# AleoNet/snarkVM

Hardware: NVIDIA H100
Metric: bls12_377_g1_msm_points_per_sec (higher is better)
Workload: dtype u32 limbs (Montgomery integer arithmetic, IMAD pipe)

## Files before the change

snarkvm_b200/csrc/api.cu:

```cuda
#include "../../include/snarkvm_b200.h"

#include <algorithm>
#include <atomic>
#include <condition_variable>
#include <cstdlib>
#include <cstring>
#include <deque>
#include <functional>
#include <map>
#include <memory>
#include <mutex>
#include <thread>
#include <vector>

#include <cuda_runtime.h>
#include <pthread.h>
#include <sched.h>
#include <cstdio>

#include "host_ec.hpp"
#include "msm.cuh"
#include "ntt.cuh"
#include "poly.cuh"

namespace b200 { void host_stream_copy(void* dst, const void* src, size_t n); }
using namespace b200;

namespace {

snarkvm_error_t make_error(int code) {
    snarkvm_error_t e;
    e.code = code;
    e.message = nullptr;
    if (code != 0) {
        const char* s = cudaGetErrorString((cudaError_t)code);
        if (s) { size_t n = strlen(s) + 1; e.message = (char*)malloc(n); if (e.message) memcpy(e.message, s, n); }
    }
    return e;
}

struct ThreadCtx {
    cudaStream_t stream[64] = {};
    bool have[64] = {};
    cudaStream_t copy_stream[64] = {};
    bool have_copy[64] = {};
    ~ThreadCtx() {}
};
thread_local ThreadCtx t_ctx;

int thread_stream(cudaStream_t* out) {
    int dev = 0;
    cudaError_t e = cudaGetDevice(&dev);
    if (e != cudaSuccess) return (int)e;
    dev &= 63;
    if (!t_ctx.have[dev]) {
        e = cudaStreamCreateWithFlags(&t_ctx.stream[dev], cudaStreamNonBlocking);
        if (e != cudaSuccess) return (int)e;
        t_ctx.have[dev] = true;
    }
    *out = t_ctx.stream[dev];
    return 0;
}

int thread_copy_stream(cudaStream_t* out) {
    int dev = 0;
    cudaError_t e = cudaGetDevice(&dev);
    if (e != cudaSuccess) return (int)e;
    dev &= 63;
    if (!t_ctx.have_copy[dev]) {
        e = cudaStreamCreateWithFlags(&t_ctx.copy_stream[dev], cudaStreamNonBlocking);
        if (e != cudaSuccess) return (int)e;
        t_ctx.have_copy[dev] = true;
    }
    *out = t_ctx.copy_stream[dev];
    return 0;
}

struct PrecomputedBases { uint32_t* table; size_t n; MsmPlan plan; int device; };
struct ResidentBases {
    void* d_ptr = nullptr;
    size_t npoints = 0, stride = 0;
    int device = 0;
    std::atomic<PrecomputedBases*> tables{nullptr};
    uint8_t head[104] = {}, tail[104] = {};
    ~ResidentBases() {
        int cur = 0;
        cudaGetDevice(&cur);
        if (cur != device) cudaSetDevice(device);
        if (d_ptr) cudaFree(d_ptr);
        if (PrecomputedBases* t = tables.load()) { cudaFree(t->table); delete t; }
        if (cur != device) cudaSetDevice(cur);
    }
};
std::mutex g_bases_mu;
std::map<const void*, std::shared_ptr<ResidentBases>> g_bases;

std::shared_ptr<ResidentBases> find_resident(const void* host, size_t npoints, size_t stride) {
    int dev = 0;
    if (cudaGetDevice(&dev) != cudaSuccess) return nullptr;
    std::shared_ptr<ResidentBases> r;
    {
        std::lock_guard<std::mutex> lock(g_bases_mu);
        auto it = g_bases.find(host);
        if (it == g_bases.end()) return nullptr;
        r = it->second;
    }
    if (r->device != dev || r->stride != stride || r->npoints < npoints) return nullptr;
    if (memcmp(r->head, host, 104) != 0) return nullptr;
    if (memcmp(r->tail, (const uint8_t*)host + (r->npoints - 1) * stride, 104) != 0) return nullptr;
    return r;
}

void write_infinity(void* out144) {
    host::Xyzz inf = host::xyzz_inf();
    host::xyzz_to_normalised_projective(inf, (uint64_t*)out144);
}

int msm_jobs_impl(void* out144s, const MsmPlan& plan, const MsmBases* bases, int nbases, const uint32_t* table, size_t table_n,
                  const MsmSegment* segs, int nsegs, int njobs, cudaStream_t stream) {
    const size_t sets = table ? 1 : (size_t)plan.nwin;
    const size_t npts = (size_t)njobs * sets;
    uint32_t* d_buf = nullptr;
    cudaError_t e = pool_alloc(&d_buf, npts * 192 + 256, stream);
    if (e != cudaSuccess) return (int)e;
    uint32_t* d_flags = d_buf + npts * 48;
    int rc = (int)cudaMemsetAsync(d_flags, 0, 256, stream);
    if (rc == 0) rc = msm_core(d_buf, d_flags, plan, bases, nbases, table, table_n, segs, nsegs, njobs, stream);
    static thread_local void* t_result_pinned = nullptr;
    constexpr size_t RESULT_PINNED_BYTES = (size_t)64 << 10;
    const size_t result_bytes = npts * 192 + 256;
    if (!t_result_pinned && result_bytes <= RESULT_PINNED_BYTES && cudaHostAlloc(&t_result_pinned, RESULT_PINNED_BYTES, cudaHostAllocDefault) != cudaSuccess) {
        cudaGetLastError(); t_result_pinned = nullptr;
    }
    std::vector<host::Xyzz> sums(npts + 2);
    void* land = (t_result_pinned && result_bytes <= RESULT_PINNED_BYTES) ? t_result_pinned : (void*)sums.data();
    if (rc == 0) rc = (int)cudaMemcpyAsync(land, d_buf, result_bytes, cudaMemcpyDeviceToHost, stream);
    cudaFreeAsync(d_buf, stream);
    if (rc == 0) rc = (int)cudaStreamSynchronize(stream);
    if (rc != 0) return rc;
    if (land != (void*)sums.data()) memcpy(sums.data(), land, result_bytes);
    uint32_t flags = 0;
    memcpy(&flags, sums.data() + npts, 4);
    if (flags & 1u) return (int)cudaErrorInvalidValue;
    auto finish = [&](int j) {
        host::Xyzz total = table ? sums[(size_t)j] : host::horner_windows(sums.data() + (size_t)j * sets, plan.nwin, plan.c);
        host::xyzz_to_normalised_projective(total, (uint64_t*)((uint8_t*)out144s + (size_t)j * 144));
    };
    if (njobs <= 2) { for (int j = 0; j < njobs; j++) finish(j); }
    else {
        const int nt = njobs < 8 ? njobs : 8;
        std::vector<std::thread> th;
        std::atomic<int> next{0};
        for (int t = 0; t < nt; t++) th.emplace_back([&] { for (int j; (j = next.fetch_add(1)) < njobs;) finish(j); });
        for (auto& t : th) t.join();
    }
    return 0;
}

int msm_device_impl(void* out144, const void* d_points, size_t npoints, const void* d_scalars, size_t stride, int mont,
                    cudaStream_t stream) {
    if (npoints == 0) { write_infinity(out144); return 0; }
    if (stride < 104 || (stride & 7)) return (int)cudaErrorInvalidValue;
    MsmPlan plan = msm_make_plan(npoints);
    MsmBases b{d_points, stride, npoints};
    MsmSegment sg{d_scalars, npoints, 0u, 0u, mont};
    return msm_jobs_impl(out144, plan, &b, 1, nullptr, 0, &sg, 1, 1, stream);
}

static bool device_local_cpus(cpu_set_t* out) {
    if (const char* e = getenv("SNARKVM_B200_COPY_NUMA")) { if (atoi(e) == 0) return false; }
    else { const char* lws = getenv("LOCAL_WORLD_SIZE"); if (!lws || atoi(lws) <= 1) return false; }
    int dev = 0;
    if (cudaGetDevice(&dev) != cudaSuccess) { cudaGetLastError(); return false; }
    char bus[64] = {};
    if (cudaDeviceGetPCIBusId(bus, (int)sizeof bus - 1, dev) != cudaSuccess) { cudaGetLastError(); return false; }
    for (char* c = bus; *c; c++) if (*c >= 'A' && *c <= 'Z') *c = (char)(*c - 'A' + 'a');
    char path[160];
    snprintf(path, sizeof path, "/sys/bus/pci/devices/%s/local_cpulist", bus);
    FILE* f = fopen(path, "r");
    if (!f) return false;
    char line[4096] = {};
    const bool got = fgets(line, sizeof line, f) != nullptr;
    fclose(f);
    if (!got) return false;
    cpu_set_t allowed, local;
    CPU_ZERO(&local);
    if (sched_getaffinity(0, sizeof allowed, &allowed) != 0) return false;
    for (const char* p = line; *p;) {
        while (*p == ',' || *p == ' ') p++;
        if (*p < '0' || *p > '9') break;
        char* end = nullptr;
        long a = strtol(p, &end, 10), b = a;
        if (*end == '-') b = strtol(end + 1, &end, 10);
        for (long c = a; c <= b && c < CPU_SETSIZE; c++) if (CPU_ISSET((int)c, &allowed)) CPU_SET((int)c, &local);
        p = end;
    }
    if (CPU_COUNT(&local) < 2 || CPU_COUNT(&local) == CPU_COUNT(&allowed)) return false;
    *out = local;
    return true;
}

class CopyPool {
public:
    bool numa_cpus(cpu_set_t* out) const { if (have_numa_) *out = numa_; return have_numa_; }
    static CopyPool& get() { static CopyPool* p = new CopyPool(); return *p; }
    void parallel_memcpy(void* dst, const void* src, size_t bytes) {
        const size_t piece = (size_t)2 << 20;
        if (bytes <= piece || nthreads_ == 0) { host_stream_copy(dst, src, bytes); return; }
        Batch batch;
        batch.dst = (uint8_t*)dst; batch.src = (const uint8_t*)src; batch.bytes = bytes; batch.piece = piece;
        batch.npieces = (bytes + piece - 1) / piece;
        run(batch);
    }
    void parallel_rows(void* dst, size_t dpitch, const void* src, size_t spitch, size_t width, size_t rows) {
        if (rows == 0 || width == 0) return;
        Batch batch;
        batch.dst = (uint8_t*)dst; batch.src = (const uint8_t*)src; batch.bytes = rows * width; batch.piece = width;
        batch.npieces = rows; batch.dpitch = dpitch; batch.spitch = spitch; batch.rows = true;
        if (nthreads_ == 0) { work(batch); return; }
        run(batch);
    }
private:
    struct Batch;
    void run(Batch& batch) {
        {
            std::lock_guard<std::mutex> lock(mu_);
            queue_.push_back(&batch);
        }
        cv_.notify_all();
        work(batch);
        std::unique_lock<std::mutex> lock(mu_);
        for (auto it = queue_.begin(); it != queue_.end(); ++it) if (*it == &batch) { queue_.erase(it); break; }
        done_cv_.wait(lock, [&] { return batch.active == 0; });
    }
    struct Batch {
        uint8_t* dst; const uint8_t* src; size_t bytes, piece, npieces;
        size_t dpitch = 0, spitch = 0;
        bool rows = false;
        std::atomic<size_t> next{0};
        int active = 0;
    };
    CopyPool() {
        int n = 12;
        if (const char* lws = getenv("LOCAL_WORLD_SIZE")) {
            const int procs = atoi(lws), cores = (int)std::thread::hardware_concurrency();
            if (procs > 1 && cores > 0) { int per = cores / procs - 1; if (per < 2) per = 2; if (per < n) n = per; }
        }
        if (const char* e = getenv("SNARKVM_B200_COPY_THREADS")) { int v = atoi(e); if (v >= 0 && v <= 64) n = v; }
        nthreads_ = n;
        have_numa_ = device_local_cpus(&numa_);
        for (int i = 0; i < n; i++) std::thread([this] { loop(); }).detach();
    }
    static void work(Batch& b) {
        for (;;) {
            size_t k = b.next.fetch_add(1);
            if (k >= b.npieces) return;
            if (b.rows) { host_stream_copy(b.dst + k * b.dpitch, b.src + k * b.spitch, b.piece); continue; }
            size_t off = k * b.piece, len = b.bytes - off < b.piece ? b.bytes - off : b.piece;
            host_stream_copy(b.dst + off, b.src + off, len);
        }
    }
    void loop() {
        if (have_numa_) pthread_setaffinity_np(pthread_self(), sizeof numa_, &numa_);
        std::unique_lock<std::mutex> lock(mu_);
        for (;;) {
            cv_.wait(lock, [&] { return !queue_.empty(); });
            Batch* b = queue_.front();
            if (b->next.load() >= b->npieces) { queue_.pop_front(); continue; }
            b->active++;
            lock.unlock();
            work(*b);
            lock.lock();
            if (--b->active == 0) done_cv_.notify_all();
        }
    }
    std::mutex mu_;
    std::condition_variable cv_, done_cv_;
    std::deque<Batch*> queue_;
    int nthreads_ = 0;
    cpu_set_t numa_;
    bool have_numa_ = false;
};

static bool host_is_pinned(const void* p) {
    cudaPointerAttributes attr;
    if (cudaPointerGetAttributes(&attr, p) != cudaSuccess) { cudaGetLastError(); return false; }
    return attr.type == cudaMemoryTypeHost || attr.type == cudaMemoryTypeManaged;
}

struct StageRing {
    static constexpr int SLOTS = 4;
    static constexpr size_t SLOT_BYTES = (size_t)32 << 20;
    void* buf[SLOTS] = {};
    cudaEvent_t ev[SLOTS] = {};
    bool used[SLOTS] = {};
    int next = 0;
    int init() {
        if (buf[0]) return 0;
// ... 164 lines not shown
    bool have = false;
    for (size_t i = 0; i < pcount && rc == 0; i++) {
        void* dst = have ? tmp : d_out;
        rc = (int)cudaMemsetAsync(dst, 0, bytes, stream);
        if (rc == 0 && plens[i]) rc = (int)cudaMemcpyAsync(dst, d_polys[i], plens[i] * 32, cudaMemcpyDeviceToDevice, stream);
        if (rc == 0) rc = ntt_device(dst, lg, NTT_FORWARD, NTT_STANDARD, scratch, stream);
        if (rc == 0 && have) rc = fr_pointwise_mul_device(d_out, tmp, n, stream);
        have = true;
    }
    for (size_t i = 0; i < ecount && rc == 0; i++) {
        if (have) rc = fr_pointwise_mul_device(d_out, d_evals[i], n, stream);
        else rc = (int)cudaMemcpyAsync(d_out, d_evals[i], bytes, cudaMemcpyDeviceToDevice, stream);
        have = true;
    }
    if (rc == 0) rc = ntt_device(d_out, lg, NTT_INVERSE, NTT_STANDARD, scratch, stream);
    cudaFreeAsync(tmp, stream);
    cudaFreeAsync(scratch, stream);
    return rc;
}

}

extern "C" {

const char* snarkvm_b200_version(void) { return "snarkvm_b200 0.1 (sm_90a)"; }
uint64_t snarkvm_b200_launch_count(void) { return launch_count(); }

snarkvm_error_t snarkvm_ntt(void* inout, uint32_t lg, snarkvm_ntt_order_t order, snarkvm_ntt_direction_t dir,
                            snarkvm_ntt_type_t type) {
    if (lg > NTT_MAX_LG || !inout || (int)order < 0 || (int)order > 3) return make_error((int)cudaErrorInvalidValue);
    cudaStream_t stream;
    int rc = thread_stream(&stream);
    if (rc) return make_error(rc);
    const size_t bytes = ((size_t)1 << lg) * 32;
    const bool pinned = host_is_pinned(inout);
    static const bool no_pipe = getenv("SNARKVM_B200_NTT_NO_PIPELINE") != nullptr;
    if (lg >= 20 && order == SNARKVM_NTT_NN && !no_pipe) {
        rc = ntt_host_pipelined(inout, lg, (int)dir, (int)type, stream, pinned);
        if (rc != -1) {
            int rs = (int)cudaStreamSynchronize(stream);
            return make_error(rc ? rc : rs);
        }
        rc = 0;
    }
    void *d = nullptr, *scratch = nullptr;
    rc = (int)pool_alloc(&d, bytes, stream);
    if (rc == 0) rc = (int)pool_alloc(&scratch, bytes, stream);
    if (rc == 0) rc = upload(d, inout, bytes, stream, pinned);
    if (rc == 0) rc = ntt_ordered(d, lg, (int)order, (int)dir, (int)type, scratch, stream);
    if (rc == 0) rc = (int)cudaStreamSynchronize(stream);
    if (rc == 0) rc = download(inout, d, bytes, stream, pinned);
    if (d) cudaFreeAsync(d, stream);
    if (scratch) cudaFreeAsync(scratch, stream);
    int rs = (int)cudaStreamSynchronize(stream);
    return make_error(rc ? rc : rs);
}

snarkvm_error_t snarkvm_polymul(void* out, size_t pcount, const void* polynomials, const void* plens_v, size_t ecount,
                                const void* evaluations, const void* elens_v, uint32_t lg) {
    if (pcount + ecount == 0) return make_error(0);
    if (lg > NTT_MAX_LG || !out) return make_error((int)cudaErrorInvalidValue);
    const void* const* polys = (const void* const*)polynomials;
    const void* const* evals = (const void* const*)evaluations;
    const size_t* plens = (const size_t*)plens_v;
    const size_t* elens = (const size_t*)elens_v;
    const size_t n = (size_t)1 << lg, bytes = n * 32;
    for (size_t i = 0; i < pcount; i++) if (plens[i] > n) return make_error((int)cudaErrorInvalidValue);
    for (size_t i = 0; i < ecount; i++) if (elens[i] != n) return make_error((int)cudaErrorInvalidValue);
    cudaStream_t stream;
    int rc = thread_stream(&stream);
    if (rc) return make_error(rc);
    std::vector<void*> dbuf(pcount + ecount, nullptr);
    std::vector<const void*> dp(pcount), de(ecount);
    void* d_out = nullptr;
    rc = (int)pool_alloc(&d_out, bytes, stream);
    for (size_t i = 0; i < pcount && rc == 0; i++) {
        size_t b = plens[i] ? plens[i] * 32 : 32;
        rc = (int)pool_alloc(&dbuf[i], b, stream);
        if (rc == 0 && plens[i]) rc = upload(dbuf[i], polys[i], plens[i] * 32, stream, host_is_pinned(polys[i]));
        dp[i] = dbuf[i];
    }
    for (size_t i = 0; i < ecount && rc == 0; i++) {
        rc = (int)pool_alloc(&dbuf[pcount + i], bytes, stream);
        if (rc == 0) rc = upload(dbuf[pcount + i], evals[i], bytes, stream, host_is_pinned(evals[i]));
        de[i] = dbuf[pcount + i];
    }
    if (rc == 0) rc = polymul_device_impl(d_out, pcount, dp.data(), plens, ecount, de.data(), elens, lg, stream);
    if (rc == 0) rc = (int)cudaStreamSynchronize(stream);
    if (rc == 0) rc = download(out, d_out, bytes, stream, host_is_pinned(out));
    for (void* p : dbuf) if (p) cudaFreeAsync(p, stream);
    if (d_out) cudaFreeAsync(d_out, stream);
    int rs = (int)cudaStreamSynchronize(stream);
    return make_error(rc ? rc : rs);
}

static std::vector<size_t> msm_ranges(size_t npoints) {
    std::vector<size_t> w;
    if (npoints >= ((size_t)1 << 23)) w = {1, 2, 4, 9};
    if (const char* e = getenv("SNARKVM_B200_MSM_CHUNKS")) {
        std::vector<size_t> v;
        for (const char* p = e; *p;) {
            char* end = nullptr;
            long x = strtol(p, &end, 10);
            if (end == p || x < 1 || x > 1024) { v.clear(); break; }
            v.push_back((size_t)x);
            p = *end == ':' ? end + 1 : end;
            if (*end && *end != ':') { v.clear(); break; }
        }
        if (v.size() == 1) v.assign(v[0] <= 64 ? v[0] : 64, 1);
        if (!v.empty()) w = v;
    }
    size_t total = 0;
    for (size_t x : w) total += x;
    std::vector<size_t> bounds{0};
    size_t acc = 0;
    for (size_t x : w) {
        acc += x;
        size_t b = (size_t)((unsigned __int128)npoints * acc / total);
        if (b > bounds.back()) bounds.push_back(b);
    }
    if (bounds.back() != npoints) bounds.push_back(npoints);
    return bounds;
}

snarkvm_error_t snarkvm_msm(void* out, const void* points, size_t npoints, const void* scalars, size_t ffi_affine_sz) {
    if (!out) return make_error((int)cudaErrorInvalidValue);
    if (npoints == 0) { write_infinity(out); return make_error(0); }
    if (!points || !scalars || ffi_affine_sz < 104 || (ffi_affine_sz & 7)) return make_error((int)cudaErrorInvalidValue);
    cudaStream_t stream;
    int rc = thread_stream(&stream);
    if (rc) return make_error(rc);
    void *d_points = nullptr, *d_scalars = nullptr;
    std::shared_ptr<ResidentBases> rb = find_resident(points, npoints, ffi_affine_sz);
    const bool resident = rb != nullptr;
    std::vector<size_t> bounds{0, npoints};
    if (!resident) bounds = msm_ranges(npoints);
    const int chunks = (int)bounds.size() - 1;
    const bool pin_s = host_is_pinned(scalars), pin_p = resident || host_is_pinned(points);
    if (!resident) rc = (int)pool_alloc(&d_points, npoints * ffi_affine_sz, stream);
    if (rc == 0) rc = (int)pool_alloc(&d_scalars, npoints * 32, stream);
    uint64_t result[18];
    if (chunks == 1) {
        if (rc == 0) rc = upload(d_scalars, scalars, npoints * 32, stream, pin_s);
        if (rc == 0 && !resident) rc = upload(d_points, points, npoints * ffi_affine_sz, stream, pin_p);
        if (rc == 0 && resident && rb->tables.load()) rc = snarkvm_b200_msm_precomputed_device(result, rb->tables.load(), d_scalars, npoints, stream);
        else if (rc == 0) rc = msm_device_impl(result, resident ? rb->d_ptr : d_points, npoints, d_scalars, ffi_affine_sz, 0, stream);
    } else {
        cudaStream_t copy = nullptr;
        if (rc == 0) rc = thread_copy_stream(&copy);
        std::vector<MsmPlan> plans;
        std::vector<size_t> sum_off{0};
        for (int k = 0; k < chunks; k++) {
            plans.push_back(msm_make_plan(bounds[k + 1] - bounds[k]));
            sum_off.push_back(sum_off.back() + (size_t)plans.back().nwin);
        }
        std::vector<cudaEvent_t> ev((size_t)chunks + 1, nullptr);
        for (auto& e : ev) if (rc == 0) rc = (int)cudaEventCreateWithFlags(&e, cudaEventDisableTiming);
        uint32_t* d_sums = nullptr;
        const size_t nsums = sum_off.back();
        if (rc == 0) rc = (int)pool_alloc(&d_sums, nsums * 192 + 256, stream);
        uint32_t* d_flags = d_sums ? d_sums + nsums * 48 : nullptr;
        if (rc == 0) rc = (int)cudaMemsetAsync(d_flags, 0, 256, stream);
        if (rc == 0) rc = (int)cudaEventRecord(ev[chunks], stream);
        if (rc == 0) rc = (int)cudaStreamWaitEvent(copy, ev[chunks], 0);
        for (int k = 0; k < chunks && rc == 0; k++) {
            const size_t i0 = bounds[k], cn = bounds[k + 1] - i0;
            rc = upload((uint8_t*)d_scalars + i0 * 32, (const uint8_t*)scalars + i0 * 32, cn * 32, copy, pin_s);
            if (rc == 0) rc = upload((uint8_t*)d_points + i0 * ffi_affine_sz, (const uint8_t*)points + i0 * ffi_affine_sz, cn * ffi_affine_sz, copy, pin_p);
            if (rc == 0) rc = (int)cudaEventRecord(ev[k], copy);
            if (rc == 0) rc = (int)cudaStreamWaitEvent(stream, ev[k], 0);
            if (rc == 0) rc = msm_window_sums_device(d_sums + sum_off[k] * 48, d_flags, plans[k], (const uint8_t*)d_points + i0 * ffi_affine_sz,
                                                     ffi_affine_sz, (const uint8_t*)d_scalars + i0 * 32, cn, stream);
        }
        std::vector<host::Xyzz> sums(nsums + 2);
        if (rc == 0) rc = (int)cudaMemcpyAsync(sums.data(), d_sums, nsums * 192 + 256, cudaMemcpyDeviceToHost, stream);
        if (d_sums) cudaFreeAsync(d_sums, stream);
        if (copy) { int rs = (int)cudaStreamSynchronize(copy); if (rc == 0) rc = rs; }
        if (rc == 0) rc = (int)cudaStreamSynchronize(stream);
        for (auto& e : ev) if (e) cudaEventDestroy(e);
        if (rc == 0) {
            uint32_t flags = 0;
            memcpy(&flags, sums.data() + nsums, 4);
            if (flags & 1u) rc = (int)cudaErrorInvalidValue;
        }
        if (rc == 0) {
            host::Xyzz total = host::xyzz_inf();
            for (int k = 0; k < chunks; k++) host::xyzz_add(total, host::horner_windows(sums.data() + sum_off[k], plans[k].nwin, plans[k].c));
            host::xyzz_to_normalised_projective(total, result);
        }
    }
    if (d_points) cudaFreeAsync(d_points, stream);
    if (d_scalars) cudaFreeAsync(d_scalars, stream);
    int rs = (int)cudaStreamSynchronize(stream);
    if (rc == 0 && rs == 0) memcpy(out, result, 144);
    return make_error(rc ? rc : rs);
}

int snarkvm_b200_ntt_device(void* d_inout, uint32_t lg, int order, int dir, int type, void* d_scratch, void* stream) {
    if (lg > NTT_MAX_LG) return (int)cudaErrorInvalidValue;
    return ntt_ordered(d_inout, lg, order, dir, type, d_scratch, (cudaStream_t)stream);
}

int snarkvm_b200_polymul_device(void* d_out, size_t pcount, const void* const* d_polys, const size_t* plens, size_t ecount,
                                const void* const* d_evals, const size_t* elens, uint32_t lg, void* stream) {
    if (lg > NTT_MAX_LG) return (int)cudaErrorInvalidValue;
    return polymul_device_impl(d_out, pcount, d_polys, plens, ecount, d_evals, elens, lg, (cudaStream_t)stream);
}

int snarkvm_b200_msm_plan(size_t npoints, int* c, int* nwin, uint32_t* cap) {
    MsmPlan p = msm_make_plan(npoints);
    if (c) *c = p.c;
    if (nwin) *nwin = p.nwin;
    if (cap) *cap = p.cap;
    return 0;
}

int snarkvm_b200_msm_plan_levels(size_t npoints) { return msm_make_plan(npoints).levels; }

int snarkvm_b200_msm_device(void* out144, const void* d_points, size_t npoints, const void* d_scalars, size_t stride,
                            void* stream) {
    if (!out144) return (int)cudaErrorInvalidValue;
    return msm_device_impl(out144, d_points, npoints, d_scalars, stride, 0, (cudaStream_t)stream);
}

static int msm_batch_impl(void* out144s, const void* d_points, size_t stride, const void* const* d_scalars, const size_t* nscalars,
                          size_t count, int mont, const void* d_points2, const void* const* d_scalars2, const size_t* nscalars2,
                          cudaStream_t stream) {
    if (count == 0) return 0;
    if (!out144s || !d_scalars || !nscalars || stride < 104 || (stride & 7)) return (int)cudaErrorInvalidValue;
    std::vector<MsmSegment> segs;
    std::vector<size_t> job_of(count, (size_t)-1);
    size_t max_n = 0, total_n = 0, max_n2 = 0;
    uint32_t njobs = 0;
    for (size_t i = 0; i < count; i++) {
        const size_t n2 = (d_scalars2 && nscalars2) ? nscalars2[i] : 0;
        if (nscalars[i] == 0 && n2 == 0) { write_infinity((uint8_t*)out144s + i * 144); continue; }
        job_of[i] = njobs;
        if (nscalars[i]) segs.push_back(MsmSegment{d_scalars[i], nscalars[i], 0u, njobs, mont});
        if (nscalars[i] > max_n) max_n = nscalars[i];
        if (n2 > max_n2) max_n2 = n2;
        total_n += nscalars[i] + n2;
        njobs++;
    }
    if (njobs == 0) return 0;
    if (max_n >= (1ull << 31)) return (int)cudaErrorInvalidValue;
    for (size_t i = 0; i < count; i++) {
        const size_t n2 = (d_scalars2 && nscalars2) ? nscalars2[i] : 0;
        if (n2) segs.push_back(MsmSegment{d_scalars2[i], n2, (uint32_t)max_n, (uint32_t)job_of[i], mont});
    }
    MsmBases bases[2] = {{d_points, stride, max_n}, {d_points2, stride, max_n2}};
    const int nbases = max_n2 ? 2 : 1;
    if (max_n2 && !d_points2) return (int)cudaErrorInvalidValue;
    size_t job_max = max_n + max_n2;
    MsmPlan plan = msm_make_plan_batch(job_max ? job_max : 1, total_n);
    std::vector<uint8_t> outs((size_t)njobs * 144);
    int rc = msm_jobs_impl(outs.data(), plan, bases, nbases, nullptr, 0, segs.data(), (int)segs.size(), (int)njobs, stream);
    if (rc != 0) return rc;
    for (size_t i = 0; i < count; i++) if (job_of[i] != (size_t)-1) memcpy((uint8_t*)out144s + i * 144, outs.data() + job_of[i] * 144, 144);
    return 0;
}

int snarkvm_b200_msm_batch_device(void* out144s, const void* d_points, size_t stride, const void* const* d_scalars, const size_t* nscalars,
                                  size_t count, void* stream) {
    return msm_batch_impl(out144s, d_points, stride, d_scalars, nscalars, count, 0, nullptr, nullptr, nullptr, (cudaStream_t)stream);
}

int snarkvm_b200_msm_window_sums_device(void* d_window_sums, const void* d_points, size_t npoints, const void* d_scalars,
                                        size_t stride, void* stream) {
    return snarkvm_b200_msm_window_sums_plan_device(d_window_sums, nullptr, npoints, d_points, npoints, d_scalars, stride, stream);
}

int snarkvm_b200_msm_window_sums_plan_device(void* d_window_sums, uint32_t* d_flags, size_t plan_npoints, const void* d_points,
                                             size_t npoints, const void* d_scalars, size_t stride, void* stream_v) {
    if (!d_window_sums || stride < 104 || (stride & 7) || plan_npoints == 0 || npoints > plan_npoints) return (int)cudaErrorInvalidValue;
    cudaStream_t stream = (cudaStream_t)stream_v;
    MsmPlan plan = msm_make_plan(plan_npoints);
    uint32_t* own_flags = nullptr;
    int rc = 0;
    if (!d_flags) { rc = (int)pool_alloc(&own_flags, 256, stream); if (rc) return rc; d_flags = own_flags; }
    rc = (int)cudaMemsetAsync(d_flags, 0, 4, stream);
    if (rc == 0 && npoints == 0) rc = (int)cudaMemsetAsync(d_window_sums, 0, (size_t)plan.nwin * 192, stream);
    else if (rc == 0) rc = msm_window_sums_device((uint32_t*)d_window_sums, d_flags, plan, d_points, stride, d_scalars, npoints, stream);
    if (own_flags) cudaFreeAsync(own_flags, stream);
    return rc;
}

int snarkvm_b200_msm_window_sums_host(void* d_window_sums, uint32_t* d_flags, size_t plan_npoints, const void* h_points, size_t npoints,
                                      const void* h_scalars, size_t stride, void* stream_v) {
    if (!d_window_sums || stride < 104 || (stride & 7) || plan_npoints == 0 || npoints > plan_npoints) return (int)cudaErrorInvalidValue;
    cudaStream_t stream = (cudaStream_t)stream_v;
    MsmPlan plan = msm_make_plan(plan_npoints);
    uint32_t* own_flags = nullptr;
    int rc = 0;
    if (!d_flags) { rc = (int)pool_alloc(&own_flags, 256, stream); if (rc) return rc; d_flags = own_flags; }
    rc = (int)cudaMemsetAsync(d_flags, 0, 4, stream);
    if (npoints == 0) {
        if (rc == 0) rc = (int)cudaMemsetAsync(d_window_sums, 0, (size_t)plan.nwin * 192, stream);
        if (own_flags) cudaFreeAsync(own_flags, stream);
        return rc;
    }
    if (!h_points || !h_scalars) { if (own_flags) cudaFreeAsync(own_flags, stream); return (int)cudaErrorInvalidValue; }
    std::vector<size_t> bounds = msm_ranges(npoints);
    const int chunks = (int)bounds.size() - 1;
    const bool pin_s = host_is_pinned(h_scalars), pin_p = host_is_pinned(h_points);
    cudaStream_t copy = nullptr;
    void *d_points = nullptr, *d_scalars = nullptr;
    uint32_t* d_parts = nullptr;
    std::vector<cudaEvent_t> ev((size_t)chunks + 1, nullptr);
    if (rc == 0) rc = thread_copy_stream(&copy);
    if (rc == 0) rc = (int)pool_alloc(&d_points, npoints * stride, stream);
    if (rc == 0) rc = (int)pool_alloc(&d_scalars, npoints * 32, stream);
    if (rc == 0 && chunks > 1) rc = (int)pool_alloc(&d_parts, (size_t)chunks * plan.nwin * 192, stream);
    for (auto& e : ev) if (rc == 0) rc = (int)cudaEventCreateWithFlags(&e, cudaEventDisableTiming);
    if (rc == 0) rc = (int)cudaEventRecord(ev[chunks], stream);
    if (rc == 0) rc = (int)cudaStreamWaitEvent(copy, ev[chunks], 0);
    for (int k = 0; k < chunks && rc == 0; k++) {
        const size_t i0 = bounds[k], cn = bounds[k + 1] - i0;
        rc = upload((uint8_t*)d_scalars + i0 * 32, (const uint8_t*)h_scalars + i0 * 32, cn * 32, copy, pin_s);
        if (rc == 0) rc = upload((uint8_t*)d_points + i0 * stride, (const uint8_t*)h_points + i0 * stride, cn * stride, copy, pin_p);
        if (rc == 0) rc = (int)cudaEventRecord(ev[k], copy);
        if (rc == 0) rc = (int)cudaStreamWaitEvent(stream, ev[k], 0);
        uint32_t* dst = chunks > 1 ? d_parts + (size_t)k * plan.nwin * 48 : (uint32_t*)d_window_sums;
        if (rc == 0) rc = msm_window_sums_device(dst, d_flags, plan, (const uint8_t*)d_points + i0 * stride, stride,
                                                 (const uint8_t*)d_scalars + i0 * 32, cn, stream);
    }
    if (rc == 0 && chunks > 1) rc = xyzz_sum_ranks_device((uint32_t*)d_window_sums, d_parts, chunks, plan.nwin, stream);
    if (rc != 0 && copy) cudaStreamSynchronize(copy);
    if (d_parts) cudaFreeAsync(d_parts, stream);
    if (d_points) cudaFreeAsync(d_points, stream);
    if (d_scalars) cudaFreeAsync(d_scalars, stream);
    if (own_flags) cudaFreeAsync(own_flags, stream);
    for (auto& e : ev) if (e) cudaEventDestroy(e);
    return rc;
}

int snarkvm_b200_xyzz_sum_ranks_device(void* d_out, const void* d_in, int nranks, int count, void* stream) {
    if (nranks < 1 || count < 1) return (int)cudaErrorInvalidValue;
    return xyzz_sum_ranks_device((uint32_t*)d_out, (const uint32_t*)d_in, nranks, count, (cudaStream_t)stream);
}

int snarkvm_b200_msm_finish(void* out144, const void* h_window_sums, int nwin, int c) {
    if (!out144 || !h_window_sums || nwin < 1 || c < 0) return (int)cudaErrorInvalidValue;
    std::vector<host::Xyzz> sums((size_t)nwin);
    memcpy(sums.data(), h_window_sums, (size_t)nwin * 192);
    host::Xyzz total = host::horner_windows(sums.data(), nwin, c);
    host::xyzz_to_normalised_projective(total, (uint64_t*)out144);
    return 0;
}

int snarkvm_b200_msm_scratch_stats(size_t* limit_bytes, size_t* in_use_bytes, size_t* peak_bytes) {
    return msm_scratch_stats(limit_bytes, in_use_bytes, peak_bytes);
}
int snarkvm_b200_msm_set_scratch_limit(size_t limit_bytes) { return msm_set_scratch_limit(limit_bytes); }

int snarkvm_b200_kzg_commit_device(void* out144, const void* d_powers, size_t stride, const void* d_coeffs_mont,
                                   size_t ncoeffs, void* stream_v) {
    if (!out144) return (int)cudaErrorInvalidValue;
    return msm_device_impl(out144, d_powers, ncoeffs, d_coeffs_mont, stride, 1, (cudaStream_t)stream_v);
}

int snarkvm_b200_msm_precompute_device(void** handle_out, const void* d_points, size_t npoints, size_t stride, void* stream_v) {
    if (!handle_out || !d_points || npoints == 0 || stride < 104 || (stride & 7)) return (int)cudaErrorInvalidValue;
    cudaStream_t stream = (cudaStream_t)stream_v;
    MsmPlan plan = msm_make_plan_precomputed(npoints);
    if (npoints * (size_t)plan.nwin >= (1ull << 31)) return (int)cudaErrorInvalidValue;
    int dev = 0;
    cudaError_t e = cudaGetDevice(&dev);
    if (e != cudaSuccess) return (int)e;
    uint32_t* table = nullptr;
    if ((e = cudaMalloc(&table, npoints * (size_t)plan.nwin * 128)) != cudaSuccess) return (int)e;
    int rc = msm_precompute_tables_device(table, plan, d_points, stride, npoints, stream);
    if (rc == 0) rc = (int)cudaStreamSynchronize(stream);
    if (rc != 0) { cudaFree(table); return rc; }
    *handle_out = new PrecomputedBases{table, npoints, plan, dev};
    return 0;
}

int snarkvm_b200_msm_precomputed_free(void* handle) {
    if (!handle) return (int)cudaErrorInvalidValue;
    PrecomputedBases* h = (PrecomputedBases*)handle;
    cudaError_t e = cudaFree(h->table);
    delete h;
    return (int)e;
}

int snarkvm_b200_msm_precomputed_info(const void* handle, size_t* npoints, int* c, int* nwin, size_t* table_bytes) {
    if (!handle) return (int)cudaErrorInvalidValue;
    const PrecomputedBases* h = (const PrecomputedBases*)handle;
    if (npoints) *npoints = h->n;
    if (c) *c = h->plan.c;
    if (nwin) *nwin = h->plan.nwin;
    if (table_bytes) *table_bytes = h->n * (size_t)h->plan.nwin * 128;
    return 0;
}

static int msm_precomputed_impl(void* out144, const void* handle, const void* d_scalars, size_t nscalars, int mont, cudaStream_t stream) {
    if (!out144 || !handle) return (int)cudaErrorInvalidValue;
    const PrecomputedBases* h = (const PrecomputedBases*)handle;
    if (nscalars > h->n) return (int)cudaErrorInvalidValue;
    if (nscalars == 0) { write_infinity(out144); return 0; }
    if (!d_scalars) return (int)cudaErrorInvalidValue;
    MsmSegment sg{d_scalars, nscalars, 0u, 0u, mont};
    return msm_jobs_impl(out144, h->plan, nullptr, 0, h->table, h->n, &sg, 1, 1, stream);
}
int snarkvm_b200_msm_precomputed_device(void* out144, const void* handle, const void* d_scalars, size_t nscalars, void* stream_v) {
    return msm_precomputed_impl(out144, handle, d_scalars, nscalars, 0, (cudaStream_t)stream_v);
}
int snarkvm_b200_kzg_commit_precomputed_device(void* out144, const void* handle, const void* d_coeffs_mont, size_t ncoeffs, void* stream_v) {
    return msm_precomputed_impl(out144, handle, d_coeffs_mont, ncoeffs, 1, (cudaStream_t)stream_v);
}
int snarkvm_b200_kzg_commit_batch_precomputed_device(void* out144s, const void* handle, const void* const* d_coeffs_mont, const size_t* ncoeffs,
                                                     size_t count, void* stream_v) {
    if (count == 0) return 0;
    if (!out144s || !handle || !d_coeffs_mont || !ncoeffs) return (int)cudaErrorInvalidValue;
    const PrecomputedBases* h = (const PrecomputedBases*)handle;
    std::vector<MsmSegment> segs;
    std::vector<size_t> job_of(count, (size_t)-1);
    uint32_t njobs = 0;
    for (size_t i = 0; i < count; i++) {
        if (ncoeffs[i] > h->n) return (int)cudaErrorInvalidValue;
        if (ncoeffs[i] == 0) { write_infinity((uint8_t*)out144s + i * 144); continue; }
        job_of[i] = njobs;
        segs.push_back(MsmSegment{d_coeffs_mont[i], ncoeffs[i], 0u, njobs++, 1});
    }
    if (njobs == 0) return 0;
    std::vector<uint8_t> outs((size_t)njobs * 144);
    int rc = msm_jobs_impl(outs.data(), h->plan, nullptr, 0, h->table, h->n, segs.data(), (int)segs.size(), (int)njobs, (cudaStream_t)stream_v);
    if (rc != 0) return rc;
    for (size_t i = 0; i < count; i++) if (job_of[i] != (size_t)-1) memcpy((uint8_t*)out144s + i * 144, outs.data() + job_of[i] * 144, 144);
    return 0;
}

int snarkvm_b200_kzg_commit_hiding_device(void* out144, const void* d_powers, size_t stride, const void* d_coeffs_mont, size_t ncoeffs,
                                          const void* d_gamma_powers, const void* d_blinding_mont, size_t nblinding, void* stream) {
    if (!out144) return (int)cudaErrorInvalidValue;
    const void* c1[1] = {d_coeffs_mont};
    const void* c2[1] = {d_blinding_mont};
    return msm_batch_impl(out144, d_powers, stride, c1, &ncoeffs, 1, 1, d_gamma_powers, c2, &nblinding, (cudaStream_t)stream);
}

int snarkvm_b200_kzg_commit_batch_device(void* out144s, const void* d_powers, size_t stride, const void* const* d_coeffs_mont,
                                         const size_t* ncoeffs, size_t count, void* stream) {
    return msm_batch_impl(out144s, d_powers, stride, d_coeffs_mont, ncoeffs, count, 1, nullptr, nullptr, nullptr, (cudaStream_t)stream);
}
int snarkvm_b200_kzg_commit_batch_hiding_device(void* out144s, const void* d_powers, size_t stride, const void* const* d_coeffs_mont,
                                                const size_t* ncoeffs, const void* d_gamma_powers, const void* const* d_blinding_mont,
                                                const size_t* nblinding, size_t count, void* stream) {
    return msm_batch_impl(out144s, d_powers, stride, d_coeffs_mont, ncoeffs, count, 1, d_gamma_powers, d_blinding_mont, nblinding, (cudaStream_t)stream);
}

int snarkvm_b200_sonic_commit_batch_device(void* out144s, size_t stride, const void* const* d_bases, const void* const* d_coeffs_mont,
                                           const size_t* ncoeffs, const void* const* d_gamma_bases, const void* const* d_blinding_mont,
                                           const size_t* nblinding, size_t count, void* stream_v) {
    cudaStream_t stream = (cudaStream_t)stream_v;
    if (count == 0) return 0;
    if (!out144s || !d_bases || !d_coeffs_mont || !ncoeffs || stride < 104 || (stride & 7)) return (int)cudaErrorInvalidValue;
    struct Use { const uint8_t* p; size_t n; const void* scal; uint32_t job; };
    std::vector<Use> uses;
    std::vector<size_t> job_of(count, (size_t)-1), job_n;
    uint32_t njobs = 0;
    size_t total_n = 0;
    for (size_t i = 0; i < count; i++) {
        const size_t n1 = ncoeffs[i], n2 = (d_blinding_mont && nblinding) ? nblinding[i] : 0;
        if (n1 == 0 && n2 == 0) { write_infinity((uint8_t*)out144s + i * 144); continue; }
        if ((n1 && (!d_bases[i] || !d_coeffs_mont[i])) || (n2 && (!d_gamma_bases || !d_gamma_bases[i] || !d_blinding_mont[i]))) return (int)cudaErrorInvalidValue;
        job_of[i] = njobs;
        if (n1) uses.push_back(Use{(const uint8_t*)d_bases[i], n1, d_coeffs_mont[i], njobs});
        if (n2) uses.push_back(Use{(const uint8_t*)d_gamma_bases[i], n2, d_blinding_mont[i], njobs});
        job_n.push_back(n1 + n2);
        total_n += n1 + n2;
        njobs++;
    }
    if (njobs == 0) return 0;
    std::vector<size_t> order(uses.size());
    for (size_t k = 0; k < order.size(); k++) order[k] = k;
    std::sort(order.begin(), order.end(), [&](size_t a, size_t b) { return uses[a].p < uses[b].p; });
    std::vector<MsmBases> arrays;
    std::vector<size_t> array_first;
    std::vector<uint32_t> base0(uses.size(), 0);
    size_t concat = 0;
    for (size_t k : order) {
        const Use& u = uses[k];
        bool joined = false;
        if (!arrays.empty()) {
            MsmBases& a = arrays.back();
            const uint8_t* a0 = (const uint8_t*)a.d_points;
            const size_t off = (size_t)(u.p - a0);
            if (off <= a.n * stride && off % stride == 0) {
                const size_t first = off / stride;
                if (first + u.n > a.n) { concat += first + u.n - a.n; a.n = first + u.n; }
                base0[k] = (uint32_t)(array_first.back() + first);
                joined = true;
            } else if (off < a.n * stride) return (int)cudaErrorInvalidValue;
        }
        if (!joined) {
            array_first.push_back(concat);
            arrays.push_back(MsmBases{u.p, stride, u.n});
            base0[k] = (uint32_t)concat;
            concat += u.n;
        }
        if (concat >= (1ull << 31)) return (int)cudaErrorInvalidValue;
    }
    std::vector<MsmSegment> segs;
    for (size_t k = 0; k < uses.size(); k++) segs.push_back(MsmSegment{uses[k].scal, uses[k].n, base0[k], uses[k].job, 1});
    size_t job_max = 1;
    for (size_t v : job_n) if (v > job_max) job_max = v;
    MsmPlan plan = msm_make_plan_batch(job_max, total_n);
    std::vector<uint8_t> outs((size_t)njobs * 144);
    int rc = msm_jobs_impl(outs.data(), plan, arrays.data(), (int)arrays.size(), nullptr, 0, segs.data(), (int)segs.size(), (int)njobs, stream);
    if (rc != 0) return rc;
    for (size_t i = 0; i < count; i++) if (job_of[i] != (size_t)-1) memcpy((uint8_t*)out144s + i * 144, outs.data() + job_of[i] * 144, 144);
    return 0;
}

static int msm_g2_impl(void* out288, const void* d_points, size_t npoints, const void* d_scalars, size_t stride, cudaStream_t stream) {
    if (!out288) return (int)cudaErrorInvalidValue;
    if (npoints == 0) { host::Xyzz2 inf = host::xyzz_inf_t<host::Fq2>(); host::xyzz_to_normalised_projective(inf, (uint64_t*)out288); return 0; }
    if (!d_points || !d_scalars || stride < 200 || (stride & 7)) return (int)cudaErrorInvalidValue;
    MsmPlan plan = msm_make_plan(npoints);
    const size_t nw = (size_t)plan.nwin;
    uint32_t* d_buf = nullptr;
    cudaError_t e = pool_alloc(&d_buf, nw * 384 + 256, stream);
    if (e != cudaSuccess) return (int)e;
    uint32_t* d_flags = d_buf + nw * 96;
    int rc = (int)cudaMemsetAsync(d_flags, 0, 256, stream);
    if (rc == 0) rc = msm_g2_window_sums_device(d_buf, d_flags, plan, d_points, stride, d_scalars, npoints, 0, stream);
    std::vector<host::Xyzz2> sums(nw + 1);
    if (rc == 0) rc = (int)cudaMemcpyAsync(sums.data(), d_buf, nw * 384 + 256, cudaMemcpyDeviceToHost, stream);
    cudaFreeAsync(d_buf, stream);
    if (rc == 0) rc = (int)cudaStreamSynchronize(stream);
    if (rc != 0) return rc;
    uint32_t flags = 0;
    memcpy(&flags, sums.data() + nw, 4);
    if (flags & 1u) return (int)cudaErrorInvalidValue;
    host::Xyzz2 total = host::horner_windows(sums.data(), plan.nwin, plan.c);
    host::xyzz_to_normalised_projective(total, (uint64_t*)out288);
    return 0;
}
int snarkvm_b200_msm_g2_device(void* out288, const void* d_points, size_t npoints, const void* d_scalars, size_t stride, void* stream) {
    return msm_g2_impl(out288, d_points, npoints, d_scalars, stride, (cudaStream_t)stream);
}
snarkvm_error_t snarkvm_b200_msm_g2(void* out, const void* points, size_t npoints, const void* scalars, size_t ffi_affine_sz) {
    if (!out) return make_error((int)cudaErrorInvalidValue);
    uint64_t result[36];
    if (npoints == 0) { int rc0 = msm_g2_impl(result, nullptr, 0, nullptr, 200, nullptr); if (rc0 == 0) memcpy(out, result, 288); return make_error(rc0); }
    if (!points || !scalars || ffi_affine_sz < 200 || (ffi_affine_sz & 7)) return make_error((int)cudaErrorInvalidValue);
    cudaStream_t stream;
    int rc = thread_stream(&stream);
    if (rc) return make_error(rc);
    void *d_points = nullptr, *d_scalars = nullptr;
    rc = (int)pool_alloc(&d_points, npoints * ffi_affine_sz, stream);
    if (rc == 0) rc = (int)pool_alloc(&d_scalars, npoints * 32, stream);
    if (rc == 0) rc = upload(d_scalars, scalars, npoints * 32, stream, host_is_pinned(scalars));
    if (rc == 0) rc = upload(d_points, points, npoints * ffi_affine_sz, stream, host_is_pinned(points));
    if (rc == 0) rc = msm_g2_impl(result, d_points, npoints, d_scalars, ffi_affine_sz, stream);
    if (d_points) cudaFreeAsync(d_points, stream);
    if (d_scalars) cudaFreeAsync(d_scalars, stream);
    int rs = (int)cudaStreamSynchronize(stream);
    if (rc == 0 && rs == 0) memcpy(out, result, 288);
    return make_error(rc ? rc : rs);
}
int snarkvm_b200_generate_bases_g2_device(void* d_points, size_t npoints, size_t stride, uint64_t seed, void* stream) {
    return msm_generate_bases_g2_device(d_points, npoints, stride, seed, (cudaStream_t)stream);
}

int snarkvm_b200_g1_ntt_device(void* d_out, size_t out_stride, const void* d_in, size_t in_stride, uint32_t lg, int direction, void* stream) {
    return g1_ntt_device(d_out, out_stride, d_in, in_stride, lg, direction, (cudaStream_t)stream);
}
int snarkvm_b200_fr_batch_inversion_and_mul_device(void* d_v, size_t n, const void* coeff_mont_host, void* stream) {
    return fr_batch_inversion_and_mul_device(d_v, n, coeff_mont_host, (cudaStream_t)stream);
}
int snarkvm_b200_poly_divide_by_vanishing_device(void* d_q, void* d_r, const void* d_p, size_t m, size_t n, void* stream) {
    return poly_divide_by_vanishing_device(d_q, d_r, d_p, m, n, (cudaStream_t)stream);
}
int snarkvm_b200_poly_divide_by_linear_device(void* d_q, const void* d_p, size_t m, const void* point_mont_host, void* stream) {
    return poly_divide_by_linear_device(d_q, d_p, m, point_mont_host, (cudaStream_t)stream);
}
int snarkvm_b200_sparse_matvec_device(void* d_out, const void* d_row_ptr, const void* d_cols, const void* d_vals, size_t nrows, const void* d_x,
                                      size_t nvars, void* stream) {
    return sparse_matvec_device(d_out, d_row_ptr, d_cols, d_vals, nrows, d_x, nvars, (cudaStream_t)stream);
}
int snarkvm_b200_fr_vec_op_device(void* d_out, const void* d_a, const void* d_b, size_t n, int op, void* stream) {
    return fr_vec_op_device(d_out, d_a, d_b, n, op, (cudaStream_t)stream);
}
int snarkvm_b200_fr_vec_scalar_op_device(void* d_out, const void* d_a, const void* scalar_mont_host, size_t n, int op, void* stream) {
    return fr_vec_scalar_op_device(d_out, d_a, scalar_mont_host, n, op, (cudaStream_t)stream);
}
int snarkvm_b200_domain_elements_device(void* d_out, uint32_t lg, void* stream) {
    return domain_elements_device(d_out, lg, (cudaStream_t)stream);
}
int snarkvm_b200_varuna_matrix_evals_device(void* d_row, void* d_col, void* d_row_col_val, const void* d_row_ptr, size_t nrows,
                                            const void* d_cols, const void* d_vals, size_t nnz, size_t nvars, size_t input_size,
                                            uint32_t lg_constraint, uint32_t lg_variable, uint32_t lg_non_zero, void* stream) {
    return varuna_matrix_evals_device(d_row, d_col, d_row_col_val, d_row_ptr, nrows, d_cols, d_vals, nnz, nvars, input_size, lg_constraint,
                                      lg_variable, lg_non_zero, (cudaStream_t)stream);
}
int snarkvm_b200_csr_transpose_device(void* d_t_row_ptr, void* d_t_cols, void* d_t_vals, const void* d_row_ptr, size_t nrows,
                                      const void* d_cols, const void* d_vals, size_t nnz, size_t nvars, size_t input_size,
                                      uint32_t lg_variable, void* stream) {
    return csr_transpose_device(d_t_row_ptr, d_t_cols, d_t_vals, d_row_ptr, nrows, d_cols, d_vals, nnz, nvars, input_size, lg_variable,
                                (cudaStream_t)stream);
}
int snarkvm_b200_poly_evaluate_device(void* out_mont_host, const void* d_coeffs, size_t m, const void* point_mont_host, void* stream) {
    return poly_evaluate_device(out_mont_host, d_coeffs, m, point_mont_host, (cudaStream_t)stream);
}

int snarkvm_b200_fr_from_mont_device(void* d_out, const void* d_in, size_t n, void* stream) {
    return fr_from_mont_device(d_out, d_in, n, (cudaStream_t)stream);
}
int snarkvm_b200_fr_to_mont_device(void* d_out, const void* d_in, size_t n, void* stream) {
    return fr_to_mont_device(d_out, d_in, n, (cudaStream_t)stream);
}

int snarkvm_b200_srs_decode_device(void* d_out, size_t stride, const void* d_in96, size_t npoints, uint32_t* d_invalid, void* stream) {
    if (!d_out || !d_in96 || !d_invalid) return (int)cudaErrorInvalidValue;
    return srs_decode_device(d_out, stride, d_in96, npoints, d_invalid, (cudaStream_t)stream);
}

int snarkvm_b200_register_bases(const void* host_points, size_t npoints, size_t stride) {
    if (!host_points || npoints == 0 || stride < 104 || (stride & 7)) return (int)cudaErrorInvalidValue;
    auto rb = std::make_shared<ResidentBases>();
    cudaError_t e = cudaGetDevice(&rb->device);
    if (e != cudaSuccess) return (int)e;
    if ((e = cudaMalloc(&rb->d_ptr, npoints * stride)) != cudaSuccess) return (int)e;
    if ((e = cudaMemcpy(rb->d_ptr, host_points, npoints * stride, cudaMemcpyHostToDevice)) != cudaSuccess) return (int)e;
    rb->npoints = npoints; rb->stride = stride;
    memcpy(rb->head, host_points, 104);
    memcpy(rb->tail, (const uint8_t*)host_points + (npoints - 1) * stride, 104);
    std::lock_guard<std::mutex> lock(g_bases_mu);
    g_bases[host_points] = rb;
    return 0;
}
int snarkvm_b200_unregister_bases(const void* host_points) {
    std::shared_ptr<ResidentBases> old;
    {
        std::lock_guard<std::mutex> lock(g_bases_mu);
        auto it = g_bases.find(host_points);
        if (it == g_bases.end()) return (int)cudaErrorInvalidValue;
        old = it->second;
        g_bases.erase(it);
    }
    return 0;
}
int snarkvm_b200_register_bases_precomputed(const void* host_points, size_t npoints, size_t stride) {
    int rc = snarkvm_b200_register_bases(host_points, npoints, stride);
    if (rc != 0) return rc;
    std::shared_ptr<ResidentBases> rb;
    {
        std::lock_guard<std::mutex> lock(g_bases_mu);
        auto it = g_bases.find(host_points);
        if (it == g_bases.end()) return (int)cudaErrorInvalidValue;
        rb = it->second;
    }
    cudaStream_t stream;
    if ((rc = thread_stream(&stream)) != 0) return rc;
    void* tables = nullptr;
    rc = snarkvm_b200_msm_precompute_device(&tables, rb->d_ptr, npoints, stride, stream);
    if (rc != 0) { snarkvm_b200_unregister_bases(host_points); return rc; }
    PrecomputedBases* expected = nullptr;
    if (!rb->tables.compare_exchange_strong(expected, (PrecomputedBases*)tables)) { snarkvm_b200_msm_precomputed_free(tables); }
    return 0;
}

int snarkvm_b200_selftest_host_copy(size_t max_bytes, uint64_t seed, uint32_t* mismatches) {
    if (!mismatches || max_bytes < 4096) return (int)cudaErrorInvalidValue;
    std::vector<uint8_t> src(max_bytes + 256), dst(max_bytes + 256), ref(max_bytes + 256);
    uint64_t x = seed | 1;
    auto rnd = [&x]() { x ^= x << 13; x ^= x >> 7; x ^= x << 17; return x; };
    for (size_t i = 0; i < src.size(); i++) src[i] = (uint8_t)rnd();
    uint32_t bad = 0;
    const size_t sizes[] = {0, 1, 31, 32, 33, 4095, 4096, 4097, 65537, ((size_t)2 << 20) - 1, ((size_t)2 << 20) + 5, max_bytes};
    for (size_t n : sizes) {
// ... 104 lines not shown
```

snarkvm_b200/csrc/host_ec.hpp:

```cpp
#pragma once
#include <cstdint>
#include <cstring>
#if defined(__x86_64__)
#include <x86intrin.h>
#endif

namespace b200 { namespace host {

typedef unsigned __int128 u128;

struct Fq {
    uint64_t l[6];
};
static const uint64_t Q_MOD[6] = {0x8508c00000000001ull, 0x170b5d4430000000ull, 0x1ef3622fba094800ull,
                                  0x1a22d9f300f5138full, 0xc63b05c06ca1493bull, 0x01ae3a4617c510eaull};
static const uint64_t Q_R1[6] = {0x02cdffffffffff68ull, 0x51409f837fffffb1ull, 0x9f7db3a98a7d3ff2ull,
                                 0x7b4e97b76e7c6305ull, 0x4cf495bf803c84e8ull, 0x008d6661e2fdf49aull};
static const uint64_t Q_INV = 9586122913090633727ull;

inline Fq fq_zero() { Fq r; memset(r.l, 0, 48); return r; }
inline Fq fq_one() { Fq r; memcpy(r.l, Q_R1, 48); return r; }
inline bool fq_is_zero(const Fq& a) { uint64_t t = 0; for (int i = 0; i < 6; i++) t |= a.l[i]; return t == 0; }
inline bool fq_eq(const Fq& a, const Fq& b) { return memcmp(a.l, b.l, 48) == 0; }
inline bool ge_mod(const uint64_t* t) {
    for (int i = 5; i >= 0; i--) { if (t[i] != Q_MOD[i]) return t[i] > Q_MOD[i]; }
    return true;
}
inline void sub_mod(uint64_t* t) {
    uint64_t br = 0;
    for (int i = 0; i < 6; i++) { u128 d = (u128)t[i] - Q_MOD[i] - br; t[i] = (uint64_t)d; br = (uint64_t)(d >> 64) & 1; }
}
inline Fq fq_add(const Fq& a, const Fq& b) {
#if defined(__x86_64__)
    unsigned long long s[6], d[6];
    unsigned char c = 0, br = 0;
    for (int i = 0; i < 6; i++) c = _addcarry_u64(c, a.l[i], b.l[i], &s[i]);
    for (int i = 0; i < 6; i++) br = _subborrow_u64(br, s[i], Q_MOD[i], &d[i]);
    Fq r;
    for (int i = 0; i < 6; i++) r.l[i] = br ? s[i] : d[i];
    return r;
#else
    Fq r; u128 c = 0;
    for (int i = 0; i < 6; i++) { c += (u128)a.l[i] + b.l[i]; r.l[i] = (uint64_t)c; c >>= 64; }
    if (ge_mod(r.l)) sub_mod(r.l);
    return r;
#endif
}
inline Fq fq_sub(const Fq& a, const Fq& b) {
#if defined(__x86_64__)
    unsigned long long d[6], e[6];
    unsigned char br = 0, c = 0;
    for (int i = 0; i < 6; i++) br = _subborrow_u64(br, a.l[i], b.l[i], &d[i]);
    for (int i = 0; i < 6; i++) c = _addcarry_u64(c, d[i], Q_MOD[i], &e[i]);
    Fq r;
    for (int i = 0; i < 6; i++) r.l[i] = br ? e[i] : d[i];
    return r;
#else
    Fq r; uint64_t br = 0;
    for (int i = 0; i < 6; i++) { u128 d = (u128)a.l[i] - b.l[i] - br; r.l[i] = (uint64_t)d; br = (uint64_t)(d >> 64) & 1; }
    if (br) { u128 c = 0; for (int i = 0; i < 6; i++) { c += (u128)r.l[i] + Q_MOD[i]; r.l[i] = (uint64_t)c; c >>= 64; } }
    return r;
#endif
}
inline Fq fq_dbl(const Fq& a) { return fq_add(a, a); }
inline void fq_mul_row(uint64_t (&t)[6], const uint64_t* a, uint64_t bi) {
    u128 p = (u128)a[0] * bi + t[0];
    uint64_t c1 = (uint64_t)(p >> 64);
    const uint64_t lo = (uint64_t)p, k = lo * Q_INV;
    p = (u128)k * Q_MOD[0] + lo;
    uint64_t c2 = (uint64_t)(p >> 64);
#pragma GCC unroll 8
    for (int j = 1; j < 6; j++) {
        p = (u128)a[j] * bi + t[j] + c1;
        c1 = (uint64_t)(p >> 64);
        p = (u128)k * Q_MOD[j] + (uint64_t)p + c2;
        t[j - 1] = (uint64_t)p;
        c2 = (uint64_t)(p >> 64);
    }
    t[5] = c1 + c2;
}
inline Fq fq_mul(const Fq& a, const Fq& b) {
    uint64_t t[6] = {0, 0, 0, 0, 0, 0};
#pragma GCC unroll 8
    for (int i = 0; i < 6; i++) fq_mul_row(t, a.l, b.l[i]);
    if (ge_mod(t)) sub_mod(t);
    Fq r; memcpy(r.l, t, 48); return r;
}
inline Fq fq_sqr(const Fq& a) { return fq_mul(a, a); }
inline Fq fq_inverse(const Fq& a) {
    uint64_t e[6]; memcpy(e, Q_MOD, 48); e[0] -= 2;
    Fq acc = fq_one(); bool started = false;
    for (int i = 5; i >= 0; i--)
        for (int b = 63; b >= 0; b--) {
            if (started) acc = fq_sqr(acc);
            if ((e[i] >> b) & 1) { acc = started ? fq_mul(acc, a) : a; started = true; }
        }
    return acc;
}

struct Fq2 {
    Fq c0, c1;
};
inline Fq fq_times5(const Fq& x) { Fq t = fq_dbl(fq_dbl(x)); return fq_add(t, x); }
inline Fq f_zero(const Fq*) { return fq_zero(); }
inline Fq f_one(const Fq*) { return fq_one(); }
inline bool f_is_zero(const Fq& a) { return fq_is_zero(a); }
inline Fq f_add(const Fq& a, const Fq& b) { return fq_add(a, b); }
inline Fq f_sub(const Fq& a, const Fq& b) { return fq_sub(a, b); }
inline Fq f_dbl(const Fq& a) { return fq_dbl(a); }
inline Fq f_mul(const Fq& a, const Fq& b) { return fq_mul(a, b); }
inline Fq f_sqr(const Fq& a) { return fq_sqr(a); }
inline Fq f_inverse(const Fq& a) { return fq_inverse(a); }
inline Fq2 f_zero(const Fq2*) { Fq2 r; r.c0 = fq_zero(); r.c1 = fq_zero(); return r; }
inline Fq2 f_one(const Fq2*) { Fq2 r; r.c0 = fq_one(); r.c1 = fq_zero(); return r; }
inline bool f_is_zero(const Fq2& a) { return fq_is_zero(a.c0) && fq_is_zero(a.c1); }
inline Fq2 f_add(const Fq2& a, const Fq2& b) { Fq2 r; r.c0 = fq_add(a.c0, b.c0); r.c1 = fq_add(a.c1, b.c1); return r; }
inline Fq2 f_sub(const Fq2& a, const Fq2& b) { Fq2 r; r.c0 = fq_sub(a.c0, b.c0); r.c1 = fq_sub(a.c1, b.c1); return r; }
inline Fq2 f_dbl(const Fq2& a) { return f_add(a, a); }
inline Fq2 f_mul(const Fq2& a, const Fq2& b) {
    Fq v0 = fq_mul(a.c0, b.c0), v1 = fq_mul(a.c1, b.c1);
    Fq2 r;
    r.c1 = fq_sub(fq_sub(fq_mul(fq_add(a.c0, a.c1), fq_add(b.c0, b.c1)), v0), v1);
    r.c0 = fq_sub(v0, fq_times5(v1));
    return r;
}
inline Fq2 f_sqr(const Fq2& a) { return f_mul(a, a); }
inline Fq2 f_inverse(const Fq2& a) {
    Fq n = fq_inverse(fq_add(fq_sqr(a.c0), fq_times5(fq_sqr(a.c1))));
    Fq2 r; r.c0 = fq_mul(a.c0, n); r.c1 = fq_sub(fq_zero(), fq_mul(a.c1, n));
    return r;
}

template <class F>
struct XyzzT {
    F X, Y, ZZ, ZZZ;
};
typedef XyzzT<Fq> Xyzz;
typedef XyzzT<Fq2> Xyzz2;
template <class F> inline XyzzT<F> xyzz_inf_t() { XyzzT<F> r; r.X = r.Y = r.ZZ = r.ZZZ = f_zero((const F*)nullptr); return r; }
inline Xyzz xyzz_inf() { return xyzz_inf_t<Fq>(); }
template <class F> inline bool xyzz_is_inf(const XyzzT<F>& p) { return f_is_zero(p.ZZ); }
template <class F> inline void xyzz_dbl(XyzzT<F>& p) {
    if (xyzz_is_inf(p)) return;
    F U = f_dbl(p.Y), V = f_sqr(U), W = f_mul(U, V), S = f_mul(p.X, V);
    F XX = f_sqr(p.X), M = f_add(f_dbl(XX), XX);
    F X3 = f_sub(f_sqr(M), f_dbl(S));
    F Y3 = f_sub(f_mul(M, f_sub(S, X3)), f_mul(W, p.Y));
    p.X = X3; p.Y = Y3; p.ZZ = f_mul(V, p.ZZ); p.ZZZ = f_mul(W, p.ZZZ);
}
template <class F> inline void xyzz_add(XyzzT<F>& p, const XyzzT<F>& o) {
    if (xyzz_is_inf(o)) return;
    if (xyzz_is_inf(p)) { p = o; return; }
    F U1 = f_mul(p.X, o.ZZ), U2 = f_mul(o.X, p.ZZ), S1 = f_mul(p.Y, o.ZZZ), S2 = f_mul(o.Y, p.ZZZ);
    F P = f_sub(U2, U1), R = f_sub(S2, S1);
    if (f_is_zero(P)) { if (f_is_zero(R)) xyzz_dbl(p); else p = xyzz_inf_t<F>(); return; }
    F PP = f_sqr(P), PPP = f_mul(P, PP), Q = f_mul(U1, PP);
    F X3 = f_sub(f_sub(f_sqr(R), PPP), f_dbl(Q));
    p.Y = f_sub(f_mul(R, f_sub(Q, X3)), f_mul(S1, PPP));
    p.X = X3;
    p.ZZ = f_mul(f_mul(p.ZZ, o.ZZ), PP);
    p.ZZZ = f_mul(f_mul(p.ZZZ, o.ZZZ), PPP);
}
template <class F> inline void xyzz_to_normalised_projective(const XyzzT<F>& p, uint64_t* out) {
    const size_t fb = sizeof(F);
    F one = f_one((const F*)nullptr);
    if (xyzz_is_inf(p)) { memset(out, 0, 3 * fb); memcpy((uint8_t*)out + fb, &one, fb); return; }
    F i = f_inverse(f_mul(p.ZZ, p.ZZZ));
    F x = f_mul(p.X, f_mul(i, p.ZZZ)), y = f_mul(p.Y, f_mul(i, p.ZZ));
    memcpy(out, &x, fb); memcpy((uint8_t*)out + fb, &y, fb); memcpy((uint8_t*)out + 2 * fb, &one, fb);
}
inline Xyzz xyzz_from_projective(const uint64_t in[18]) {
    Xyzz p; memcpy(p.X.l, in, 48); memcpy(p.Y.l, in + 6, 48);
    Fq Z; memcpy(Z.l, in + 12, 48);
    p.ZZ = fq_sqr(Z); p.ZZZ = fq_mul(p.ZZ, Z);
    if (fq_is_zero(Z)) p = xyzz_inf();
    return p;
}
template <class F> inline XyzzT<F> horner_windows(const XyzzT<F>* sums, int nwin, int c) {
    XyzzT<F> total = xyzz_inf_t<F>();
    for (int w = nwin - 1; w >= 0; w--) {
        for (int k = 0; k < c; k++) xyzz_dbl(total);
        xyzz_add(total, sums[w]);
    }
    return total;
}

}}
```

snarkvm_b200/csrc/msm.cu:

```cuda
#include "msm.cuh"

#include <atomic>
#include <condition_variable>
#include <memory>
#include <mutex>
#include <utility>
#include <vector>
#include <cstdio>
#include <cstdlib>
#include <cub/device/device_scan.cuh>

#define FF_CALL_MUL 1
#include "ec.cuh"
#include "cta_inverse.cuh"
#include "quad.cuh"
#define FIELD_TEST_ENTRY test_field_op_msm
#include "testops.cuh"

namespace b200 {

static std::atomic<uint64_t> g_launches{0};
uint64_t launch_count() { return g_launches.load(); }
void count_launch(int n) { g_launches.fetch_add((uint64_t)n); }

static std::atomic<bool> g_prof{false};
static std::mutex g_prof_mu;
static std::vector<std::pair<cudaEvent_t, cudaEvent_t>> g_prof_recs[PROF_KINDS];
void prof_enable(bool on) { g_prof.store(on); }
bool prof_enabled() { return g_prof.load(); }
ProfScope::ProfScope(int kind_, cudaStream_t stream_) : stream(stream_), kind(kind_) {
    if (!g_prof.load()) return;
    if (cudaEventCreate(&a) != cudaSuccess || cudaEventCreate(&b) != cudaSuccess) { a = b = nullptr; return; }
    cudaEventRecord(a, stream);
}
ProfScope::~ProfScope() {
    if (!a) return;
    cudaEventRecord(b, stream);
    std::lock_guard<std::mutex> lock(g_prof_mu);
    g_prof_recs[kind].emplace_back(a, b);
}
int prof_collect(int kind, double* total_ms, uint64_t* count) {
    if (kind < 0 || kind >= PROF_KINDS) return (int)cudaErrorInvalidValue;
    std::vector<std::pair<cudaEvent_t, cudaEvent_t>> recs;
    { std::lock_guard<std::mutex> lock(g_prof_mu); recs.swap(g_prof_recs[kind]); }
    double tot = 0; int rc = 0;
    for (auto& r : recs) {
        float ms = 0;
        cudaError_t e = cudaEventSynchronize(r.second);
        if (e == cudaSuccess) e = cudaEventElapsedTime(&ms, r.first, r.second);
        if (e != cudaSuccess) rc = (int)e; else tot += ms;
        cudaEventDestroy(r.first); cudaEventDestroy(r.second);
    }
    if (total_ms) *total_ms = tot;
    if (count) *count = recs.size();
    return rc;
}

#define CUDA_TRY(x)                                   \
    do {                                              \
        cudaError_t e_ = (x);                         \
        if (e_ != cudaSuccess) { rc = (int)e_; goto done; } \
    } while (0)

static int ceil_log2(size_t x) { int l = 0; size_t v = x > 1 ? x - 1 : 0; while (v) { l++; v >>= 1; } return l; }
static int plan_log2(size_t x) {
    int l = ceil_log2(x < 2 ? 2 : x);
    if (l > 1 && (double)x < 0.70710678118 * (double)((size_t)1 << l)) l--;
    return l;
}

MsmPlan msm_make_plan(size_t npoints) {
    MsmPlan p;
    int lg = plan_log2(npoints);
    int c = lg <= 8 ? 4 : lg <= 12 ? lg - 4 : lg <= 18 ? 11 : lg == 19 ? 13 : lg == 20 ? 15 : lg <= 22 ? 16 : 17;
    if (const char* e = getenv("SNARKVM_B200_MSM_C")) { int v = atoi(e); if (v >= 2 && v <= 24) c = v; }
    p.c = c;
    p.nwin = 253 / c + 1;
    p.nbuckets = 1u << (c - 1);
    size_t total = npoints * (size_t)p.nwin;
    size_t cap = total / 300000 + 1;
    if (cap < 16) cap = 16;
    if (const char* e = getenv("SNARKVM_B200_MSM_CAP")) { long v = atol(e); if (v >= 1) cap = (size_t)v; }
    p.cap = (uint32_t)cap;
    int levels = lg >= 23 ? 5 : lg >= 21 ? 4 : lg == 20 ? 3 : lg == 19 ? 2 : 0;
    while (levels > 0 && ((npoints >> (c - 1)) >> levels) < 2) levels--;
    if (const char* e = getenv("SNARKVM_B200_MSM_LEVELS")) { int v = atoi(e); if (v >= 0 && v <= 16) levels = v; }
    p.levels = levels;
    return p;
}

MsmPlan msm_make_plan_batch(size_t max_n, size_t total_n) {
    MsmPlan p = msm_make_plan(max_n);
    if (total_n > max_n) {
        int lgt = plan_log2(total_n);
        int levels = lgt >= 23 ? 5 : lgt >= 21 ? 4 : lgt == 20 ? 3 : lgt == 19 ? 2 : 0;
        while (levels > p.levels && ((max_n >> (p.c - 1)) >> levels) < 4) levels--;
        while (levels > 0 && ((max_n >> (p.c - 1)) >> levels) < 2) levels--;
        if (const char* e = getenv("SNARKVM_B200_MSM_LEVELS")) { int v = atoi(e); if (v >= 0 && v <= 16) levels = v; }
        if (levels > p.levels) p.levels = levels;
        size_t cap = total_n * (size_t)p.nwin / 300000 + 1;
        if (cap < 16) cap = 16;
        if (const char* e = getenv("SNARKVM_B200_MSM_CAP")) { long v = atol(e); if (v >= 1) cap = (size_t)v; }
        p.cap = (uint32_t)cap;
    }
    return p;
}

template <bool SCATTER, bool MONT>
__global__ void __launch_bounds__(256) k_digits(const uint32_t* __restrict__ scalars, size_t n, int c, int nwin,
                                                uint32_t nbuckets, uint32_t* __restrict__ counters ,
                                                uint32_t* __restrict__ sorted, size_t flat ,
                                                uint32_t slot_base, uint32_t index_base, uint32_t* __restrict__ flags) {
    size_t i = (size_t)blockIdx.x * blockDim.x + threadIdx.x;
    if (i >= n) return;
    uint32_t s[8];
    {
        const uint4* q = reinterpret_cast<const uint4*>(scalars + 8 * i);
        uint4 a = __ldg(q), b = __ldg(q + 1);
        s[0] = a.x; s[1] = a.y; s[2] = a.z; s[3] = a.w; s[4] = b.x; s[5] = b.y; s[6] = b.z; s[7] = b.w;
    }
    if (MONT) {
        Fr x;
#pragma unroll
        for (int k = 0; k < 8; k++) x.v[k] = s[k];
        x = x.from_mont();
#pragma unroll
        for (int k = 0; k < 8; k++) s[k] = x.v[k];
    }
    if (!SCATTER && (s[7] >> 29)) atomicOr(flags, 1u);
    const uint32_t half = 1u << (c - 1);
    uint32_t carry = 0;
    for (int w = 0; w < nwin; w++) {
        int bit = w * c;
        int wi = bit >> 5, sh = bit & 31;
        uint32_t lo = 0, hi = 0;
#pragma unroll
        for (int k = 0; k < 8; k++) { if (k == wi) lo = s[k]; if (k == wi + 1) hi = s[k]; }
        uint32_t raw = (__funnelshift_r(lo, hi, sh) & ((1u << c) - 1u)) + carry;
        uint32_t neg = raw > half ? 1u : 0u;
        uint32_t mag = neg ? (1u << c) - raw : raw;
        carry = neg;
        if (mag != 0u) {
            uint32_t slot = slot_base + (flat ? 0u : (uint32_t)w * nbuckets) + (mag - 1u);
            if (SCATTER) {
                uint32_t pos = atomicAdd(&counters[slot], 1u);
                sorted[pos] = (uint32_t)(flat ? (size_t)w * flat + i : (size_t)index_base + i) | (neg << 31);
            } else {
                atomicAdd(&counters[slot], 1u);
            }
        }
    }
}

__global__ void k_items_per_bucket(const uint32_t* __restrict__ hist, uint32_t* __restrict__ items, uint32_t total_buckets, uint32_t cap,
                                   uint32_t* __restrict__ hot , uint32_t hot_max,
                                   uint32_t keep) {
    uint32_t i = blockIdx.x * blockDim.x + threadIdx.x;
    if (i < total_buckets) {
        const uint32_t it = (hist[i] + cap - 1u) / cap;
        items[i] = it;
        if (hot != nullptr && it > keep) { const uint32_t pos = atomicAdd(hot, 1u); if (pos < hot_max) hot[1u + pos] = i; }
    } else if (i == total_buckets) items[i] = 0;
}

static constexpr int DENSE_WORDS = 24;
static constexpr int BASE_WORDS = 32;

struct DensePoint { Fq x, y; bool inf; };
FF_DEV DensePoint load_dense(const uint32_t* p) {
    DensePoint d; d.x = Fq::load_ldg(p); d.y = Fq::load_ldg(p + 12);
    d.inf = d.x.is_zero() && d.y.is_zero();
    return d;
}
FF_DEV void store_dense(uint32_t* p, const DensePoint& d) {
    if (d.inf) { Fq z = Fq::zero(); z.store(p); z.store(p + 12); }
    else { d.x.store(p); d.y.store(p + 12); }
}
static constexpr uint32_t REC_NONE = 0xffffffffu;
template <bool MONT, bool FLAT>
__global__ void __launch_bounds__(256) k_scatter_records(const uint32_t* __restrict__ scalars, size_t n, const uint8_t* __restrict__ points,
                                                         size_t stride, const uint32_t* __restrict__ table, size_t table_n, int c, uint32_t nbuckets,
                                                         uint32_t* __restrict__ cursors, uint32_t slot_base, int w_lo, int w_hi,
                                                         const uint32_t* __restrict__ pos_base_ptr, uint4* __restrict__ dense0) {
    __shared__ uint4 sh_rec[256 * 9];
    __shared__ uint32_t sh_pos[2][256];
    const uint32_t tid = threadIdx.x;
    const size_t i = (size_t)blockIdx.x * 256 + tid;
    const bool live = i < n;
    const uint32_t pos_base = __ldg(pos_base_ptr);
    uint32_t s[8];
#pragma unroll
    for (int k = 0; k < 8; k++) s[k] = 0u;
    auto stage = [&](Fq x, Fq y, bool inf) {
        Fq yn = y.neg();
        if (inf) { x = Fq::zero(); y = Fq::zero(); yn = Fq::zero(); }
        uint4* r = sh_rec + tid * 9;
#pragma unroll
        for (int k = 0; k < 3; k++) {
            r[k] = make_uint4(x.v[4 * k], x.v[4 * k + 1], x.v[4 * k + 2], x.v[4 * k + 3]);
            r[3 + k] = make_uint4(y.v[4 * k], y.v[4 * k + 1], y.v[4 * k + 2], y.v[4 * k + 3]);
            r[6 + k] = make_uint4(yn.v[4 * k], yn.v[4 * k + 1], yn.v[4 * k + 2], yn.v[4 * k + 3]);
        }
    };
    if (live) {
        const uint4* q = reinterpret_cast<const uint4*>(scalars + 8 * i);
        uint4 a = __ldg(q), b = __ldg(q + 1);
        s[0] = a.x; s[1] = a.y; s[2] = a.z; s[3] = a.w; s[4] = b.x; s[5] = b.y; s[6] = b.z; s[7] = b.w;
        if (MONT) {
            Fr x;
#pragma unroll
            for (int k = 0; k < 8; k++) x.v[k] = s[k];
            x = x.from_mont();
#pragma unroll
            for (int k = 0; k < 8; k++) s[k] = x.v[k];
        }
        if (!FLAT) {
            AffinePoint pt = load_affine(points, stride, i);
            stage(pt.x, pt.y, pt.inf);
        }
    }
    const uint32_t half = 1u << (c - 1);
    uint32_t carry = 0;
    for (int w = 0; w < w_hi; w++) {
        const int bit = w * c, wi = bit >> 5, sh = bit & 31;
        uint32_t lo = 0, hi = 0;
#pragma unroll
        for (int k = 0; k < 8; k++) { if (k == wi) lo = s[k]; if (k == wi + 1) hi = s[k]; }
        const uint32_t raw = (__funnelshift_r(lo, hi, sh) & ((1u << c) - 1u)) + carry;
        const uint32_t neg = raw > half ? 1u : 0u;
        const uint32_t mag = neg ? (1u << c) - raw : raw;
        carry = neg;
        if (w < w_lo) continue;
        if (FLAT) {
            if (w > w_lo) __syncthreads();
            if (live && mag != 0u) {
                const DensePoint d = load_dense(table + ((size_t)w * table_n + i) * BASE_WORDS);
                stage(d.x, d.y, d.inf);
            }
        }
        uint32_t pos = REC_NONE;
        if (live && mag != 0u) pos = (atomicAdd(&cursors[slot_base + (FLAT ? 0u : (uint32_t)w * nbuckets) + (mag - 1u)], 1u) - pos_base) | (neg << 31);
        uint32_t* my_pos = sh_pos[w & 1];
        my_pos[tid] = pos;
        __syncthreads();
        for (uint32_t k = tid; k < 256u * 6u; k += 256u) {
            const uint32_t r = k / 6u, part = k - 6u * r;
            const uint32_t pp = my_pos[r];
            if (pp == REC_NONE) continue;
            const uint32_t src = part < 3u ? part : ((pp >> 31) ? 3u : 0u) + part;
            dense0[(size_t)(pp & 0x7fffffffu) * 6u + part] = sh_rec[r * 9u + src];
        }
    }
}

FF_DEV AffinePoint load_record(const uint32_t* __restrict__ records, uint32_t idx) {
    const uint32_t* p = records + (size_t)idx * 32;
    AffinePoint a;
    a.x = Fq::load_ldg(p); a.y = Fq::load_ldg(p + 12);
    a.inf = a.x.is_zero() && a.y.is_zero();
    return a;
}
#ifndef MSM_ACC_THREADS
#define MSM_ACC_THREADS 128
#define MSM_ACC_MINBLOCKS 4
#endif
__global__ void __launch_bounds__(MSM_ACC_THREADS, MSM_ACC_MINBLOCKS) k_bucket_accumulate(const uint32_t* __restrict__ records ,
                                                            const uint32_t* __restrict__ sorted,
                                                            const uint32_t* __restrict__ bucket_start ,
                                                            const uint32_t* __restrict__ item_start ,
                                                            uint32_t total_buckets, uint32_t cap, uint32_t* __restrict__ partial) {
    uint32_t t = blockIdx.x * blockDim.x + threadIdx.x;
    uint32_t total_items = item_start[total_buckets];
    if (t >= total_items) return;
    uint32_t lo = 0, hi = total_buckets;
    while (hi - lo > 1) {
        uint32_t mid = (lo + hi) >> 1;
        if (item_start[mid] <= t) lo = mid; else hi = mid;
    }
    uint32_t wb = lo;
    uint32_t seg = t - item_start[wb];
    uint32_t b0 = bucket_start[wb], b1 = bucket_start[wb + 1];
    uint32_t s0 = b0 + seg * cap;
    uint32_t s1 = s0 + cap < b1 ? s0 + cap : b1;

    XYZZ acc = XYZZ::infinity();
    uint32_t e = sorted[s0];
    AffinePoint p = load_record(records, e & 0x7fffffffu);
    for (uint32_t k = s0; k < s1; k++) {
        uint32_t e_cur = e;
        AffinePoint p_cur = p;
        if (k + 1 < s1) { e = sorted[k + 1]; p = load_record(records, e & 0x7fffffffu); }
        acc.add_affine(p_cur, (e_cur >> 31) != 0u);
    }
    acc.store(partial + (size_t)t * XYZZ_WORDS);
}

template <bool GATHER>
FF_DEV DensePoint load_level_input(const uint32_t* __restrict__ dense_bases, const uint32_t* __restrict__ sorted,
                                   const uint32_t* __restrict__ dense_in, uint32_t idx) {
    DensePoint d;
    if (GATHER) {
        uint32_t e = sorted[idx];
        d = load_dense(dense_bases + (size_t)(e & 0x7fffffffu) * BASE_WORDS);
        if ((e >> 31) && !d.inf) d.y = d.y.neg();
    } else {
        d = load_dense(dense_in + (size_t)idx * DENSE_WORDS);
    }
    return d;
}
template <bool GATHER>
FF_DEV const uint32_t* level_input_ptr(const uint32_t* __restrict__ dense_bases, const uint32_t* __restrict__ sorted,
                                       const uint32_t* __restrict__ dense_in, uint32_t idx) {
    if (GATHER) return dense_bases + (size_t)(sorted[idx] & 0x7fffffffu) * BASE_WORDS;
    return dense_in + (size_t)idx * DENSE_WORDS;
}
__global__ void k_densify_bases(const uint8_t* __restrict__ points, size_t stride, size_t n, uint32_t* __restrict__ out) {
    size_t i = (size_t)blockIdx.x * blockDim.x + threadIdx.x;
    if (i >= n) return;
    AffinePoint a = load_affine(points, stride, i);
    DensePoint d; d.x = a.x; d.y = a.y; d.inf = a.inf;
    store_dense(out + i * BASE_WORDS, d);
}
__global__ void __launch_bounds__(CTA_INV_THREADS) k_precompute_tables(const uint8_t* __restrict__ points, size_t stride, size_t n, int c, int nwin,
                                                            uint32_t* __restrict__ table) {
    __shared__ uint4 sh_inv[CTA_INV_SMEM_BYTES / 16];
    const size_t i = (size_t)blockIdx.x * blockDim.x + threadIdx.x;
    const bool live = i < n;
    AffinePoint a;
    a.x = Fq::zero(); a.y = Fq::zero(); a.inf = true;
    if (live) a = load_affine(points, stride, i);
    DensePoint d; d.x = a.x; d.y = a.y; d.inf = a.inf;
    if (live) store_dense(table + i * BASE_WORDS, d);
    XYZZ q = XYZZ::from_affine(a);
    for (int w = 1; w < nwin; w++) {
        for (int k = 0; k < c; k++) q.dbl();
        const bool inf = q.is_inf();
        Fq z = inf ? Fq::one() : q.ZZ * q.ZZZ;
        Fq iz = cta_shared_inverse_by(z, reinterpret_cast<uint32_t*>(sh_inv), w & 3);
        __syncthreads();
        if (inf) { d.x = Fq::zero(); d.y = Fq::zero(); d.inf = true; }
        else { d.x = q.X * (iz * q.ZZZ); d.y = q.Y * (iz * q.ZZ); d.inf = false; }
        if (live) store_dense(table + ((size_t)w * n + i) * BASE_WORDS, d);
    }
}

static constexpr int PAIR_THREADS = CTA_INV_THREADS;
enum PairKind { PAIR_COPY1 = 0, PAIR_COPY2 = 1, PAIR_INF = 2, PAIR_ADD = 3, PAIR_DBL = 4 };
FF_DEV int classify_pair(const DensePoint& P, const DensePoint& Q, bool has2, Fq& d) {
    if (!has2 || Q.inf) return PAIR_COPY1;
    if (P.inf) return PAIR_COPY2;
    if (P.x == Q.x) {
        if (P.y == Q.y && !P.y.is_zero()) { d = P.y.dbl(); return PAIR_DBL; }
        return PAIR_INF;
    }
    d = Q.x - P.x;
    return PAIR_ADD;
}

template <bool GATHER>
__global__ void __launch_bounds__(PAIR_THREADS, 4) k_pair_level(const uint32_t* __restrict__ dense_bases,
                                                        const uint32_t* __restrict__ sorted, const uint32_t* __restrict__ dense_in,
                                                        const uint32_t* __restrict__ off_in, const uint32_t* __restrict__ off_out,
                                                        uint32_t total_buckets, uint32_t T, uint32_t* __restrict__ prefix,
                                                        uint32_t* __restrict__ dense_out) {
    __shared__ uint4 sh_inv4[PAIR_THREADS * 3];
    uint32_t* sh_inv = reinterpret_cast<uint32_t*>(sh_inv4);
    const uint32_t total = off_out[total_buckets];
    const uint64_t o0_64 = (uint64_t)(blockIdx.x * blockDim.x + threadIdx.x) * T;
    const uint32_t o0 = o0_64 < total ? (uint32_t)o0_64 : total;
    const uint32_t o1 = (o0_64 + T < total) ? o0 + T : total;
    uint32_t lo = 0, hi = total_buckets;
    if (o0 < o1) while (hi - lo > 1) { uint32_t mid = (lo + hi) >> 1; if (off_out[mid] <= o0) lo = mid; else hi = mid; }
    uint32_t b = lo;

    Fq run = Fq::one();
    for (uint32_t o = o0; o < o1; o++) {
        while (o >= off_out[b + 1]) b++;
        const uint32_t i = o - off_out[b], base_in = off_in[b], cnt = off_in[b + 1] - base_in;
        const bool has2 = 2 * i + 1 < cnt;
        if (has2) {
            const uint32_t* pp = level_input_ptr<GATHER>(dense_bases, sorted, dense_in, base_in + 2 * i);
            const uint32_t* qp = level_input_ptr<GATHER>(dense_bases, sorted, dense_in, base_in + 2 * i + 1);
            Fq x1 = Fq::load_ldg(pp), x2 = Fq::load_ldg(qp);
            if (x1 == x2 || x1.is_zero() || x2.is_zero()) {
                DensePoint P = load_level_input<GATHER>(dense_bases, sorted, dense_in, base_in + 2 * i);
                DensePoint Q = load_level_input<GATHER>(dense_bases, sorted, dense_in, base_in + 2 * i + 1);
                Fq d;
                int kind = classify_pair(P, Q, true, d);
                if (kind >= PAIR_ADD) run = run * d;
            } else {
                run = run * (x2 - x1);
            }
        }
        run.store(prefix + (size_t)o * 12);
    }
    Fq inv = cta_shared_inverse(run, sh_inv);
    for (uint32_t o = o1; o-- > o0;) {
        while (o < off_out[b]) b--;
        const uint32_t i = o - off_out[b], base_in = off_in[b], cnt = off_in[b + 1] - base_in;
        const bool has2 = 2 * i + 1 < cnt;
        DensePoint P = load_level_input<GATHER>(dense_bases, sorted, dense_in, base_in + 2 * i);
        DensePoint Q = P;
        if (has2) Q = load_level_input<GATHER>(dense_bases, sorted, dense_in, base_in + 2 * i + 1);
        Fq d;
        int kind = classify_pair(P, Q, has2, d);
        DensePoint R;
        if (kind == PAIR_COPY1) R = P;
        else if (kind == PAIR_COPY2) R = Q;
        else if (kind == PAIR_INF) { R.inf = true; R.x = Fq::zero(); R.y = Fq::zero(); }
        else {
            Fq inv_d = (o == o0) ? inv : inv * Fq::load(prefix + (size_t)(o - 1) * 12);
            inv = inv * d;
            Fq lambda;
            if (kind == PAIR_ADD) lambda = (Q.y - P.y) * inv_d;
            else { Fq xx = P.x.sqr(); lambda = (xx.dbl() + xx) * inv_d; }
            Fq x3 = lambda.sqr() - P.x - Q.x;
            R.y = lambda * (P.x - x3) - P.y;
            R.x = x3;
            R.inf = false;
        }
        store_dense(dense_out + (size_t)o * DENSE_WORDS, R);
    }
}


FF_DEV uint32_t smem_addr_u32(const void* p) { return (uint32_t)__cvta_generic_to_shared(p); }
FF_DEV void cp_async16(uint32_t dst, const void* src) {
    asm volatile("cp.async.cg.shared.global [%0], [%1], 16;" ::"r"(dst), "l"(src) : "memory");
}
FF_DEV void cp_async_commit() { asm volatile("cp.async.commit_group;" ::: "memory"); }
FF_DEV void cp_async_wait_1() { asm volatile("cp.async.wait_group 1;" ::: "memory"); }
FF_DEV void cp_async_wait_0() { asm volatile("cp.async.wait_group 0;" ::: "memory"); }
FF_DEV void cp_async_wait_3() { asm volatile("cp.async.wait_group 3;" ::: "memory"); }

static constexpr int RING_CHUNKS = 12;
static constexpr int RING_STAGE_U4 = RING_CHUNKS * 32;
static constexpr int PAIR2_SMEM = PAIR_THREADS * 48 + 4 * 2 * RING_STAGE_U4 * 16;

FF_DEV Fq ring_fq(const uint4* slot) {
    Fq r;
#pragma unroll
    for (int i = 0; i < 3; i++) { uint4 t = slot[i * 32]; r.v[4 * i] = t.x; r.v[4 * i + 1] = t.y; r.v[4 * i + 2] = t.z; r.v[4 * i + 3] = t.w; }
    return r;
}

static constexpr uint32_t PAIR_NONE = 0xffffffffu;
template <bool GATHER>
__global__ void __launch_bounds__(256) k_pair_desc(const uint32_t* __restrict__ sorted, const uint32_t* __restrict__ off_in,
                                                   const uint32_t* __restrict__ off_out, uint32_t total_buckets, uint2* __restrict__ desc,
                                                   const uint32_t* __restrict__ in_base_ptr ) {
    const uint32_t o = blockIdx.x * blockDim.x + threadIdx.x;
    if (o >= __ldg(off_out + total_buckets)) return;
    uint32_t lo = 0, hi = total_buckets;
    while (hi - lo > 1) { uint32_t mid = (lo + hi) >> 1; if (__ldg(off_out + mid) <= o) lo = mid; else hi = mid; }
    const uint32_t i = o - __ldg(off_out + lo), base_in = __ldg(off_in + lo), cnt = __ldg(off_in + lo + 1) - base_in;
    const uint32_t idx = base_in + 2u * i;
    const bool has2 = 2u * i + 1u < cnt;
    uint2 d;
    if (GATHER) { d.x = __ldg(sorted + idx); d.y = has2 ? __ldg(sorted + idx + 1) : PAIR_NONE; }
    else { d.x = idx - (in_base_ptr ? __ldg(in_base_ptr) : 0u); d.y = has2 ? 0u : PAIR_NONE; }
    desc[o] = d;
}

struct PairDesc {
    uint32_t p, q;
    bool valid;
    FF_DEV bool has2() const { return valid && q != PAIR_NONE; }
};
FF_DEV PairDesc pair_load_desc(int64_t j, uint32_t nv, const uint2* __restrict__ dlane) {
    PairDesc d; d.p = 0; d.q = PAIR_NONE; d.valid = false;
    if (j < 0 || j >= (int64_t)nv) return d;
    const uint2 v = __ldg(dlane + 32 * j);
    d.p = v.x; d.q = v.y; d.valid = true;
    return d;
}
template <bool GATHER>
FF_DEV const uint32_t* pair_src(const PairDesc& d, int which, const uint32_t* __restrict__ records) {
    if (GATHER) return records + (size_t)((which ? d.q : d.p) & 0x7fffffffu) * BASE_WORDS;
    return records + (size_t)(d.p + (uint32_t)which) * DENSE_WORDS;
}
template <bool GATHER, bool FULL>
FF_DEV void pair_issue(const PairDesc& d, uint4* ring, int st, int lane, const uint32_t* __restrict__ records, int chunks) {
    if (d.valid) {
        const uint32_t dst = smem_addr_u32(ring + (size_t)st * (size_t)(chunks * 32) + lane);
        const uint32_t* p = pair_src<GATHER>(d, 0, records);
#pragma unroll
        for (int k = 0; k < (FULL ? 6 : 3); k++) cp_async16(dst + (uint32_t)k * 512u, p + 4 * k);
        if (d.q != PAIR_NONE) {
            const uint32_t* q = pair_src<GATHER>(d, 1, records);
#pragma unroll
            for (int k = 0; k < (FULL ? 6 : 3); k++) cp_async16(dst + (uint32_t)((FULL ? 6 : 3) + k) * 512u, q + 4 * k);
        }
    }
    cp_async_commit();
}
template <bool GATHER>
FF_DEV int pair_classify_global(const PairDesc& d, const uint32_t* __restrict__ records, Fq& den) {
    DensePoint P = load_dense(pair_src<GATHER>(d, 0, records));
    DensePoint Q = load_dense(pair_src<GATHER>(d, 1, records));
    if (GATHER) { if ((d.p >> 31) && !P.inf) P.y = P.y.neg(); if ((d.q >> 31) && !Q.inf) Q.y = Q.y.neg(); }
    return classify_pair(P, Q, true, den);
}

template <bool GATHER, int MINB>
__global__ void __launch_bounds__(PAIR_THREADS, MINB) k_pair_level2(const uint32_t* __restrict__ records ,
                                                         const uint2* __restrict__ desc, const uint32_t* __restrict__ total_ptr,
                                                         uint32_t T, uint32_t* __restrict__ prefix, uint32_t* __restrict__ dense_out,
                                                         uint32_t* __restrict__ sm_slots) {
    extern __shared__ uint4 pair2_smem[];
    __shared__ uint32_t sh_slot;
    uint32_t* sh_inv = reinterpret_cast<uint32_t*>(pair2_smem);
    const int lane = threadIdx.x & 31, warp = threadIdx.x >> 5;
    uint4* ring = pair2_smem + PAIR_THREADS * 3 + (size_t)warp * 2 * RING_STAGE_U4;
    if (threadIdx.x == 0) {
        uint32_t smid;
        asm volatile("mov.u32 %0, %%smid;" : "=r"(smid));
        sh_slot = atomicAdd(sm_slots + (smid & 255u), 1u);
    }
    __syncthreads();
    const int inv_warp = (int)(sh_slot & 3u);
    const uint32_t total = __ldg(total_ptr);
    const uint64_t w0_64 = ((uint64_t)blockIdx.x * (PAIR_THREADS / 32) + (uint32_t)warp) * 32ull * T + (uint32_t)lane;
    uint32_t nv = 0;
    if (w0_64 < total) { const uint64_t left = (total - w0_64 + 31) / 32; nv = left < T ? (uint32_t)left : T; }
    const uint2* dlane = desc + w0_64;
    uint32_t* plane = prefix + w0_64 * 12;
    uint32_t* olane = dense_out + w0_64 * DENSE_WORDS;

    Fq run = Fq::one();
    {
        constexpr int PF = 3;
        PairDesc q0 = pair_load_desc(0, nv, dlane), q1 = pair_load_desc(1, nv, dlane), q2 = pair_load_desc(2, nv, dlane);
        pair_issue<GATHER, false>(q0, ring, 0, lane, records, 6);
        pair_issue<GATHER, false>(q1, ring, 1, lane, records, 6);
        pair_issue<GATHER, false>(q2, ring, 2, lane, records, 6);
        PairDesc ahead = pair_load_desc(PF, nv, dlane);
        for (uint32_t j = 0; j < T; j++) {
            pair_issue<GATHER, false>(ahead, ring, (int)((j + PF) & 3u), lane, records, 6);
            const PairDesc cur = q0;
            q0 = q1; q1 = q2; q2 = ahead;
            ahead = pair_load_desc((int64_t)j + PF + 1, nv, dlane);
            cp_async_wait_3();
            Fq d = Fq::one();
            if (cur.has2()) {
                const uint4* slot_p = ring + (size_t)(j & 3u) * (6 * 32) + lane;
                Fq x1 = ring_fq(slot_p), x2 = ring_fq(slot_p + 3 * 32);
                if (x1 == x2 || x1.is_zero() || x2.is_zero()) {
                    Fq den;
                    if (pair_classify_global<GATHER>(cur, records, den) >= PAIR_ADD) d = den;
                } else {
                    d = x2 - x1;
                }
            }
            run = run * d;
            if (cur.valid) run.store(plane + (size_t)j * (32 * 12));
        }
        cp_async_wait_0();
    }
    Fq inv = cta_shared_inverse_by(run, sh_inv, inv_warp);
    {
        PairDesc cur = pair_load_desc((int64_t)T - 1, nv, dlane);
        pair_issue<GATHER, true>(cur, ring, 0, lane, records, 12);
        PairDesc nxt = pair_load_desc((int64_t)T - 2, nv, dlane);
        for (uint32_t k = 0; k < T; k++) {
            const uint32_t j = T - 1 - k;
            pair_issue<GATHER, true>(nxt, ring, (int)((k + 1) & 1u), lane, records, 12);
            PairDesc nn = pair_load_desc((int64_t)j - 2, nv, dlane);
            Fq pf = Fq::one();
            if (cur.valid && j != 0) pf = Fq::load(plane + (size_t)(j - 1) * (32 * 12));
            cp_async_wait_1();
            const uint4* slot_p = ring + (size_t)(k & 1u) * RING_STAGE_U4 + lane;
            int kind = PAIR_COPY1;
            Fq d = Fq::one(), num = Fq::zero();
            const bool has2 = cur.has2();
            const bool negP = GATHER && (cur.p >> 31), negQ = GATHER && has2 && (cur.q >> 31);
            if (has2) {
                Fq x1 = ring_fq(slot_p), x2 = ring_fq(slot_p + 6 * 32);
                if (x1 == x2 || x1.is_zero() || x2.is_zero()) {
                    DensePoint P, Q;
                    P.x = x1; P.y = ring_fq(slot_p + 3 * 32); P.inf = P.x.is_zero() && P.y.is_zero();
                    Q.x = x2; Q.y = ring_fq(slot_p + 9 * 32); Q.inf = Q.x.is_zero() && Q.y.is_zero();
                    if (negP && !P.inf) P.y = P.y.neg();
                    if (negQ && !Q.inf) Q.y = Q.y.neg();
                    Fq den;
                    kind = classify_pair(P, Q, true, den);
                    if (kind >= PAIR_ADD) d = den;
                    if (kind == PAIR_ADD) num = Q.y - P.y;
                    else if (kind == PAIR_DBL) { Fq xx = P.x.sqr(); num = xx.dbl() + xx; }
                } else {
                    kind = PAIR_ADD;
                    d = x2 - x1;
                    Fq y1 = ring_fq(slot_p + 3 * 32), y2 = ring_fq(slot_p + 9 * 32);
                    if (negP == negQ) { num = y2 - y1; if (negP) num = num.neg(); }
                    else { num = y2 + y1; if (negQ) num = num.neg(); }
                }
            }
            Fq inv_next = inv * d;
            Fq inv_d = (j != 0) ? inv * pf : inv;
            inv = inv_next;
            Fq lambda = num * inv_d;
            Fq x3 = lambda.sqr();
            {
                Fq x1 = ring_fq(slot_p), x2 = has2 ? ring_fq(slot_p + 6 * 32) : x1;
                x3 = x3 - x1 - x2;
                Fq t = x1 - x3;
                Fq y3 = lambda * t;
                if (cur.valid) {
                    DensePoint R;
                    if (kind >= PAIR_ADD) {
                        Fq y1 = ring_fq(slot_p + 3 * 32);
                        R.x = x3; R.y = negP ? y3 + y1 : y3 - y1; R.inf = false;
                    } else if (kind == PAIR_INF) {
                        R.inf = true; R.x = Fq::zero(); R.y = Fq::zero();
                    } else {
                        const int c0 = (kind == PAIR_COPY2) ? 6 : 0;
                        R.x = ring_fq(slot_p + c0 * 32); R.y = ring_fq(slot_p + (c0 + 3) * 32);
                        R.inf = R.x.is_zero() && R.y.is_zero();
                        if (((kind == PAIR_COPY2) ? negQ : negP) && !R.inf) R.y = R.y.neg();
                    }
                    store_dense(olane + (size_t)j * (32 * DENSE_WORDS), R);
                }
            }
            cur = nxt; nxt = nn;
        }
        cp_async_wait_0();
    }
}

__global__ void k_halve_counts(const uint32_t* __restrict__ off_in, uint32_t* __restrict__ cnt_out, uint32_t total_buckets) {
    uint32_t i = blockIdx.x * blockDim.x + threadIdx.x;
    if (i < total_buckets) cnt_out[i] = (off_in[i + 1] - off_in[i] + 1u) >> 1;
    else if (i == total_buckets) cnt_out[i] = 0;
}
__global__ void k_items_from_offsets(const uint32_t* __restrict__ off, uint32_t* __restrict__ items, uint32_t total_buckets, uint32_t cap,
                                     uint32_t* __restrict__ hot, uint32_t hot_max, uint32_t keep) {
    uint32_t i = blockIdx.x * blockDim.x + threadIdx.x;
    if (i < total_buckets) {
        const uint32_t it = (off[i + 1] - off[i] + cap - 1u) / cap;
        items[i] = it;
        if (hot != nullptr && it > keep) { const uint32_t pos = atomicAdd(hot, 1u); if (pos < hot_max) hot[1u + pos] = i; }
    } else if (i == total_buckets) items[i] = 0;
}

__global__ void __launch_bounds__(MSM_ACC_THREADS, MSM_ACC_MINBLOCKS) k_bucket_accumulate_dense(
    const uint32_t* __restrict__ dense, const uint32_t* __restrict__ bucket_start, const uint32_t* __restrict__ item_start,
    uint32_t total_buckets, uint32_t cap, uint32_t* __restrict__ partial) {
    uint32_t t = blockIdx.x * blockDim.x + threadIdx.x;
    uint32_t total_items = item_start[total_buckets];
    if (t >= total_items) return;
    uint32_t lo = 0, hi = total_buckets;
    while (hi - lo > 1) { uint32_t mid = (lo + hi) >> 1; if (item_start[mid] <= t) lo = mid; else hi = mid; }
    uint32_t wb = lo, seg = t - item_start[wb];
    uint32_t b0 = bucket_start[wb], b1 = bucket_start[wb + 1];
    uint32_t s0 = b0 + seg * cap, s1 = s0 + cap < b1 ? s0 + cap : b1;
    XYZZ acc = XYZZ::infinity();
    DensePoint p = load_dense(dense + (size_t)s0 * DENSE_WORDS);
    for (uint32_t k = s0; k < s1; k++) {
        AffinePoint cur; cur.x = p.x; cur.y = p.y; cur.inf = p.inf;
        if (k + 1 < s1) p = load_dense(dense + (size_t)(k + 1) * DENSE_WORDS);
        acc.add_affine(cur, false);
    }
    acc.store(partial + (size_t)t * XYZZ_WORDS);
}

__global__ void k_group_counts(const uint32_t* __restrict__ start_in, uint32_t* __restrict__ cnt_out, uint32_t total_buckets) {
    uint32_t i = blockIdx.x * blockDim.x + threadIdx.x;
    if (i < total_buckets) cnt_out[i] = (start_in[i + 1] - start_in[i] + 31u) >> 5;
    else if (i == total_buckets) cnt_out[i] = 0;
}
__global__ void __launch_bounds__(128) k_partial_group_sum(const uint32_t* __restrict__ partial_in, const uint32_t* __restrict__ start_in,
                                                            const uint32_t* __restrict__ start_out, uint32_t total_buckets,
                                                            uint32_t* __restrict__ partial_out) {
    uint32_t t = blockIdx.x * blockDim.x + threadIdx.x;
    if (t >= start_out[total_buckets]) return;
    uint32_t lo = 0, hi = total_buckets;
    while (hi - lo > 1) { uint32_t mid = (lo + hi) >> 1; if (start_out[mid] <= t) lo = mid; else hi = mid; }
    uint32_t g = t - start_out[lo];
    uint32_t i0 = start_in[lo] + g * 32u, i1 = start_in[lo + 1];
    if (i0 + 32u < i1) i1 = i0 + 32u;
    XYZZ s = XYZZ::load(partial_in + (size_t)i0 * XYZZ_WORDS);
    for (uint32_t i = i0 + 1; i < i1; i++) s.add(XYZZ::load(partial_in + (size_t)i * XYZZ_WORDS));
    s.store(partial_out + (size_t)t * XYZZ_WORDS);
}

FF_DEV uint32_t fold_rounds_of(uint32_t cnt, uint32_t& final_cnt, uint32_t keep = 32u) {
    uint32_t r = 0;
    while (cnt > keep) { cnt = (cnt + 31u) >> 5; r++; }
    final_cnt = cnt;
    return r;
}

FF_DEV XYZZ bucket_sum(const uint32_t* __restrict__ partial, const uint32_t* __restrict__ item_start, uint32_t wb) {
    uint32_t i0 = item_start[wb], i1 = item_start[wb + 1];
    XYZZ s = XYZZ::infinity();
    for (uint32_t i = i0; i < i1; i++) {
        if (i == i0) s = XYZZ::load(partial + (size_t)i * XYZZ_WORDS);
        else s.add(XYZZ::load(partial + (size_t)i * XYZZ_WORDS));
    }
    return s;
}

template <bool PAIRS>
__global__ void __launch_bounds__(128) k_bucket_reduce(const uint32_t* __restrict__ partial, const uint32_t* __restrict__ item_start,
                                                        uint32_t nbuckets, uint32_t chunk, uint32_t chunks_per_window,
                                                        uint32_t nwin, uint32_t* __restrict__ out,
                                                        const uint32_t* __restrict__ partial_b = nullptr, int folds = 0) {
    uint32_t t = blockIdx.x * blockDim.x + threadIdx.x;
    if (t >= chunks_per_window * nwin) return;
    uint32_t w = t / chunks_per_window, j = t % chunks_per_window;
    uint32_t lo = j * chunk, hi = lo + chunk;
    XYZZ running = XYZZ::infinity(), acc = XYZZ::infinity();
    for (uint32_t b = hi; b-- > lo;) {
        XYZZ s;
        if (PAIRS && folds > 0) {
            const uint32_t wb = w * nbuckets + b, i0 = item_start[wb];
            uint32_t cnt = item_start[wb + 1] - i0;
            const uint32_t r = fold_rounds_of(cnt, cnt, 1u);
            s = cnt ? XYZZ::load(((r & 1u) ? partial_b : partial) + (size_t)i0 * XYZZ_WORDS) : XYZZ::infinity();
        } else
            s = bucket_sum(partial, item_start, w * nbuckets + b);
        running.add(s);
        acc.add(running);
    }
    if (PAIRS) {
        acc.store(out + (size_t)t * 2 * XYZZ_WORDS);
        running.store(out + ((size_t)t * 2 + 1) * XYZZ_WORDS);
        return;
    }
    if (lo != 0u) acc.add(running.mul_u32(lo));
    acc.store(out + (size_t)t * XYZZ_WORDS);
}

__global__ void __launch_bounds__(128) k_group_sum(const uint32_t* __restrict__ in, uint32_t per_row, uint32_t group,
                                                    uint32_t out_per_row, uint32_t rows, uint32_t* __restrict__ out) {
    uint32_t t = blockIdx.x * blockDim.x + threadIdx.x;
    if (t >= out_per_row * rows) return;
    uint32_t r = t / out_per_row, j = t % out_per_row;
    uint32_t i0 = j * group, i1 = i0 + group < per_row ? i0 + group : per_row;
    XYZZ s = XYZZ::infinity();
    for (uint32_t i = i0; i < i1; i++) s.add(XYZZ::load(in + ((size_t)r * per_row + i) * XYZZ_WORDS));
    s.store(out + (size_t)t * XYZZ_WORDS);
}

FF_DEV XYZZ shfl_xor_xyzz(const XYZZ& a, int m) {
    XYZZ r;
#pragma unroll
    for (int j = 0; j < 12; j++) {
        r.X.v[j] = __shfl_xor_sync(0xffffffffu, a.X.v[j], m); r.Y.v[j] = __shfl_xor_sync(0xffffffffu, a.Y.v[j], m);
        r.ZZ.v[j] = __shfl_xor_sync(0xffffffffu, a.ZZ.v[j], m); r.ZZZ.v[j] = __shfl_xor_sync(0xffffffffu, a.ZZZ.v[j], m);
    }
    return r;
}
FF_DEV XYZZ shfl_down_xyzz(const XYZZ& a, int d) {
    XYZZ r;
#pragma unroll
    for (int j = 0; j < 12; j++) {
        r.X.v[j] = __shfl_down_sync(0xffffffffu, a.X.v[j], d); r.Y.v[j] = __shfl_down_sync(0xffffffffu, a.Y.v[j], d);
        r.ZZ.v[j] = __shfl_down_sync(0xffffffffu, a.ZZ.v[j], d); r.ZZZ.v[j] = __shfl_down_sync(0xffffffffu, a.ZZZ.v[j], d);
    }
    return r;
}
FF_DEV XYZZ warp_sum_xyzz(XYZZ a) {
#pragma unroll 1
    for (int m = 16; m >= 1; m >>= 1) { XYZZ o = shfl_xor_xyzz(a, m); a.add(o); }
    return a;
}
FF_DEV XYZZ warp_suffix_scan_xyzz(XYZZ a, int lane) {
#pragma unroll 1
    for (int d = 1; d < 32; d <<= 1) { XYZZ o = shfl_down_xyzz(a, d); if (lane + d < 32) a.add(o); }
    return a;
}

static constexpr int ACC_G = 8;
__global__ void __launch_bounds__(128, 4) k_bucket_accumulate_g8(const uint32_t* __restrict__ records, const uint32_t* __restrict__ sorted,
                                                                 const uint32_t* __restrict__ bucket_start, const uint32_t* __restrict__ item_start,
                                                                 uint32_t total_buckets, uint32_t cap, uint32_t* __restrict__ partial) {
    const uint32_t t = blockIdx.x * blockDim.x + threadIdx.x, item = t / ACC_G, sub = t % ACC_G;
    const bool valid = item < item_start[total_buckets];
    XYZZ acc = XYZZ::infinity();
    if (valid) {
        uint32_t lo = 0, hi = total_buckets;
        while (hi - lo > 1) { uint32_t mid = (lo + hi) >> 1; if (item_start[mid] <= item) lo = mid; else hi = mid; }
        const uint32_t seg = item - item_start[lo];
        const uint32_t b0 = bucket_start[lo], b1 = bucket_start[lo + 1];
        const uint32_t s0 = b0 + seg * cap, s1 = s0 + cap < b1 ? s0 + cap : b1;
        uint32_t k = s0 + sub;
        if (k < s1) {
            uint32_t e = sorted[k];
            AffinePoint p = load_record(records, e & 0x7fffffffu);
            for (; k < s1; k += ACC_G) {
                const uint32_t e_cur = e;
                const AffinePoint p_cur = p;
                if (k + ACC_G < s1) { e = sorted[k + ACC_G]; p = load_record(records, e & 0x7fffffffu); }
                acc.add_affine(p_cur, (e_cur >> 31) != 0u);
            }
        }
    }
#pragma unroll 1
    for (int m = ACC_G / 2; m >= 1; m >>= 1) { XYZZ o = shfl_xor_xyzz(acc, m); acc.add(o); }
    if (valid && sub == 0) acc.store(partial + (size_t)item * XYZZ_WORDS);
}

__global__ void __launch_bounds__(128) k_bucket_reduce_warp(const uint32_t* __restrict__ partial, const uint32_t* __restrict__ item_start,
                                                            uint32_t nbuckets, uint32_t chunks, uint32_t nsets, uint32_t* __restrict__ out) {
    const uint32_t warp = (blockIdx.x * blockDim.x + threadIdx.x) >> 5, lane = threadIdx.x & 31u;
    if (warp >= nsets * chunks) return;
    const uint32_t set = warp / chunks, ch = warp % chunks, b = ch * 32u + lane;
    XYZZ s = XYZZ::infinity();
    if (b < nbuckets) s = bucket_sum(partial, item_start, set * nbuckets + b);
    const XYZZ run = warp_suffix_scan_xyzz(s, (int)lane);
    const XYZZ acc = warp_sum_xyzz(run);
    if (lane == 0) {
        acc.store(out + (size_t)warp * 2 * XYZZ_WORDS);
        run.store(out + ((size_t)warp * 2 + 1) * XYZZ_WORDS);
    }
}
__global__ void __launch_bounds__(32) k_window_combine_warp(const uint32_t* __restrict__ in, uint32_t chunks, uint32_t* __restrict__ out) {
    const uint32_t set = blockIdx.x, lane = threadIdx.x;
    XYZZ a = XYZZ::infinity(), r = XYZZ::infinity();
    if (lane < chunks) {
        a = XYZZ::load(in + ((size_t)set * chunks + lane) * 2 * XYZZ_WORDS);
        r = XYZZ::load(in + (((size_t)set * chunks + lane) * 2 + 1) * XYZZ_WORDS);
    }
    XYZZ total = warp_sum_xyzz(a);
    if (chunks > 1) {
        XYZZ suf = warp_suffix_scan_xyzz(r, (int)lane);
        if (lane == 0) suf = XYZZ::infinity();
        XYZZ w = warp_sum_xyzz(suf);
        for (int k = 0; k < 5; k++) w.dbl();
        total.add(w);
    }
    if (lane == 0) total.store(out + (size_t)set * XYZZ_WORDS);
}

FF_DEV XYZZ load_xyzz_plain(const uint32_t* p) {
    XYZZ r; const uint4* q = reinterpret_cast<const uint4*>(p);
    uint32_t w[XYZZ_WORDS];
#pragma unroll
    for (int i = 0; i < XYZZ_WORDS / 4; i++) { const uint4 t = q[i]; w[4 * i] = t.x; w[4 * i + 1] = t.y; w[4 * i + 2] = t.z; w[4 * i + 3] = t.w; }
#pragma unroll
    for (int j = 0; j < 12; j++) { r.X.v[j] = w[j]; r.Y.v[j] = w[12 + j]; r.ZZ.v[j] = w[24 + j]; r.ZZZ.v[j] = w[36 + j]; }
    return r;
}
FF_DEV void store_xyzz_plain(uint32_t* p, const XYZZ& a) {
    uint4* q = reinterpret_cast<uint4*>(p);
    uint32_t w[XYZZ_WORDS];
#pragma unroll
    for (int j = 0; j < 12; j++) { w[j] = a.X.v[j]; w[12 + j] = a.Y.v[j]; w[24 + j] = a.ZZ.v[j]; w[36 + j] = a.ZZZ.v[j]; }
#pragma unroll
    for (int i = 0; i < XYZZ_WORDS / 4; i++) q[i] = make_uint4(w[4 * i], w[4 * i + 1], w[4 * i + 2], w[4 * i + 3]);
}

__global__ void __launch_bounds__(128, 2) k_bucket_accumulate_q8(const uint32_t* __restrict__ records, const uint32_t* __restrict__ sorted,
                                                                 const uint32_t* __restrict__ bucket_start, const uint32_t* __restrict__ item_start,
                                                                 uint32_t total_buckets, uint32_t cap, uint32_t* __restrict__ partial) {
    const uint32_t item = (blockIdx.x * blockDim.x + threadIdx.x) >> 5;
    if (item >= item_start[total_buckets]) return;
    const Quad Q = Quad::here();
    uint32_t lo = 0, hi = total_buckets;
    while (hi - lo > 1) { uint32_t mid = (lo + hi) >> 1; if (item_start[mid] <= item) lo = mid; else hi = mid; }
    const uint32_t seg = item - item_start[lo];
    const uint32_t b0 = bucket_start[lo], b1 = bucket_start[lo + 1];
    const uint32_t s0 = b0 + seg * cap, s1 = s0 + cap < b1 ? s0 + cap : b1;
    XYZZ acc = XYZZ::infinity();
    {
        AffinePoint p; p.x = Fq::zero(); p.y = Fq::zero(); p.inf = true;
        uint32_t e = 0;
        uint32_t k = s0 + (uint32_t)Q.slot;
        if (k < s1) { e = sorted[k]; p = load_record(records, e & 0x7fffffffu); }
#pragma unroll 1
        for (uint32_t base = s0; base < s1; base += 8, k += 8) {
            __syncwarp();
            const uint32_t e_cur = e;
            const AffinePoint p_cur = p;
            p.inf = true;
            if (k + 8 < s1) { e = sorted[k + 8]; p = load_record(records, e & 0x7fffffffu); }
            acc = quad_add_affine(acc, p_cur, (e_cur >> 31) != 0u, Q);
        }
    }
    acc = slot_sum(acc, Q);
    if ((threadIdx.x & 31u) == 0u) acc.store(partial + (size_t)item * XYZZ_WORDS);
}

__global__ void __launch_bounds__(128) k_fold_hot_quad(const uint32_t* __restrict__ in, const uint32_t* __restrict__ item_start,
                                                       const uint32_t* __restrict__ hot, uint32_t hot_max, uint32_t round, uint32_t keep,
                                                       uint32_t* __restrict__ out) {
    uint32_t nhot = hot[0];
    if (nhot > hot_max) nhot = hot_max;
    const Quad Q = Quad::here();
    const uint32_t nwarps = (gridDim.x * blockDim.x) >> 5, w0 = (blockIdx.x * blockDim.x + threadIdx.x) >> 5;
    for (uint32_t h = w0 >> 5; h < nhot; h += nwarps >> 5) {
        const uint32_t b = hot[1u + h];
        const uint32_t i0 = item_start[b];
        uint32_t cnt = item_start[b + 1] - i0;
        bool live = true;
        for (uint32_t r = 0; r < round; r++) { if (cnt <= keep) live = false; cnt = (cnt + 31u) >> 5; }
        if (!live || cnt <= keep) continue;
        const uint32_t groups = (cnt + 31u) >> 5;
        for (uint32_t g = w0 & 31u; g < groups; g += 32u) {
            const uint32_t k = g << 5, end = k + 32u < cnt ? k + 32u : cnt;
            XYZZ s = XYZZ::infinity();
#pragma unroll 1
            for (uint32_t i = k; i < end; i += 8u) {
                __syncwarp();
                XYZZ v = XYZZ::infinity();
                if (i + (uint32_t)Q.slot < end) v = XYZZ::load(in + (size_t)(i0 + i + (uint32_t)Q.slot) * XYZZ_WORDS);
                s = quad_add(s, v, Q);
            }
            s = slot_sum(s, Q);
            if ((threadIdx.x & 31u) == 0u) s.store(out + (size_t)(i0 + g) * XYZZ_WORDS);
        }
    }
}

__global__ void __launch_bounds__(128) k_bucket_reduce_quad(const uint32_t* __restrict__ partial_a, const uint32_t* __restrict__ partial_b,
                                                            const uint32_t* __restrict__ item_start, int folds,
                                                            uint32_t nbuckets, uint32_t chunks, uint32_t nsets, uint32_t* __restrict__ out) {
    const uint32_t warp = (blockIdx.x * blockDim.x + threadIdx.x) >> 5;
    if (warp >= nsets * chunks) return;
    const Quad Q = Quad::here();
    const uint32_t set = warp / chunks, ch = warp % chunks, b = ch * 8u + (uint32_t)Q.slot;
    XYZZ s = XYZZ::infinity();
    {
        uint32_t i0 = 0, cnt = 0;
        const uint32_t* partial = partial_a;
        if (b < nbuckets) {
            const uint32_t wb = set * nbuckets + b;
            i0 = item_start[wb];
            cnt = item_start[wb + 1] - i0;
            if (folds) { if (fold_rounds_of(cnt, cnt) & 1u) partial = partial_b; }
        }
        const uint32_t trips = __reduce_max_sync(0xffffffffu, cnt);
#pragma unroll 1
        for (uint32_t i = 0; i < trips; i++) {
            __syncwarp();
            XYZZ t = XYZZ::infinity();
            if (i < cnt) t = XYZZ::load(partial + (size_t)(i0 + i) * XYZZ_WORDS);
            s = quad_add(s, t, Q);
        }
    }
    const XYZZ run = slot_suffix_scan(s, Q);
    const XYZZ acc = slot_sum(run, Q);
    if ((threadIdx.x & 31u) == 0u) {
        acc.store(out + (size_t)warp * 2 * XYZZ_WORDS);
        run.store(out + ((size_t)warp * 2 + 1) * XYZZ_WORDS);
    }
}

FF_DEV XYZZ combine_fold_quad(const XYZZ& a, const XYZZ& r, int lgw, const Quad& Q, XYZZ& run_out) {
    XYZZ A = slot_sum(a, Q);
    const XYZZ suf = slot_suffix_scan(r, Q);
    XYZZ W = slot_sum(Q.slot == 0 ? XYZZ::infinity() : suf, Q);
#pragma unroll 1
    for (int k = 0; k < lgw; k++) W = quad_dbl(W, Q);
    run_out = suf;
    return quad_add(A, W, Q);
}
__global__ void __launch_bounds__(128) k_combine_level_quad(const uint32_t* __restrict__ in, uint32_t m, uint32_t nsets, int lgw, uint32_t* __restrict__ out) {
    const uint32_t warp = (blockIdx.x * blockDim.x + threadIdx.x) >> 5, groups = (m + 7u) / 8u;
    if (warp >= nsets * groups) return;
    const Quad Q = Quad::here();
    const uint32_t set = warp / groups, g = warp % groups, j = g * 8u + (uint32_t)Q.slot;
    XYZZ a = XYZZ::infinity(), r = XYZZ::infinity();
    if (j < m) { a = load_xyzz_plain(in + ((size_t)set * m + j) * 2 * XYZZ_WORDS); r = load_xyzz_plain(in + (((size_t)set * m + j) * 2 + 1) * XYZZ_WORDS); }
    XYZZ run;
    const XYZZ A = combine_fold_quad(a, r, lgw, Q, run);
    if ((threadIdx.x & 31u) == 0u) {
        store_xyzz_plain(out + (size_t)warp * 2 * XYZZ_WORDS, A);
        store_xyzz_plain(out + ((size_t)warp * 2 + 1) * XYZZ_WORDS, run);
    }
}
__global__ void __launch_bounds__(128) k_combine_level_quadseq(const uint32_t* __restrict__ in, uint32_t m, uint32_t nsets, int lgw, uint32_t* __restrict__ out) {
    const uint32_t quad = (blockIdx.x * blockDim.x + threadIdx.x) >> 2, groups = (m + 7u) / 8u;
    if (quad >= nsets * groups) return;
    const Quad Q = Quad::here();
    const uint32_t set = quad / groups, g = quad % groups, first = g * 8u;
    const uint32_t cnt = m - first < 8u ? m - first : 8u;
    XYZZ A = XYZZ::infinity(), running = XYZZ::infinity(), W = XYZZ::infinity();
#pragma unroll 1
    for (uint32_t s = cnt; s-- > 0u;) {
        const size_t e = ((size_t)set * m + first + s) * 2;
        A = quad_add(A, load_xyzz_plain(in + e * XYZZ_WORDS), Q);
        running = quad_add(running, load_xyzz_plain(in + (e + 1) * XYZZ_WORDS), Q);
        if (s >= 1u) W = quad_add(W, running, Q);
    }
#pragma unroll 1
    for (int k = 0; k < lgw; k++) W = quad_dbl(W, Q);
    A = quad_add(A, W, Q);
    if (Q.q == 0) {
        store_xyzz_plain(out + (size_t)quad * 2 * XYZZ_WORDS, A);
        store_xyzz_plain(out + ((size_t)quad * 2 + 1) * XYZZ_WORDS, running);
    }
}
static constexpr int COMBINE_QUAD_MAX_WARPS = 8;
__global__ void __launch_bounds__(32 * COMBINE_QUAD_MAX_WARPS) k_window_combine_quad(const uint32_t* __restrict__ in, uint32_t m0, int lgw0, uint32_t* __restrict__ out) {
    __shared__ __align__(16) uint32_t sm[COMBINE_QUAD_MAX_WARPS][2][XYZZ_WORDS];
    const uint32_t set = blockIdx.x, warp = threadIdx.x >> 5;
    const Quad Q = Quad::here();
    const uint32_t* src = in + (size_t)set * m0 * 2 * XYZZ_WORDS;
    uint32_t m = m0;
    int lgw = lgw0;
    for (;;) {
        const uint32_t groups = (m + 7u) / 8u;
        XYZZ A, run;
        if (warp < groups) {
            const uint32_t j = warp * 8u + (uint32_t)Q.slot;
            XYZZ a = XYZZ::infinity(), r = XYZZ::infinity();
            if (j < m) { a = load_xyzz_plain(src + (size_t)j * 2 * XYZZ_WORDS); r = load_xyzz_plain(src + ((size_t)j * 2 + 1) * XYZZ_WORDS); }
            A = combine_fold_quad(a, r, lgw, Q, run);
            if (groups == 1u && (threadIdx.x & 31u) == 0u) A.store(out + (size_t)set * XYZZ_WORDS);
        }
        if (groups == 1u) break;
        __syncthreads();
        if (warp < groups && (threadIdx.x & 31u) == 0u) { store_xyzz_plain(&sm[warp][0][0], A); store_xyzz_plain(&sm[warp][1][0], run); }
        __syncthreads();
        src = &sm[0][0][0];
        m = groups; lgw += 3;
    }
}

__global__ void k_xyzz_sum_ranks(const uint32_t* __restrict__ in, int nranks, int count, uint32_t* __restrict__ out) {
    int i = blockIdx.x * blockDim.x + threadIdx.x;
    if (i >= count) return;
    XYZZ s = XYZZ::load(in + (size_t)i * XYZZ_WORDS);
    for (int r = 1; r < nranks; r++) s.add(XYZZ::load(in + ((size_t)r * count + i) * XYZZ_WORDS));
    s.store(out + (size_t)i * XYZZ_WORDS);
}

int xyzz_sum_ranks_device(uint32_t* d_out, const uint32_t* d_in, int nranks, int count, cudaStream_t stream) {
    k_xyzz_sum_ranks<<<(count + 31) / 32, 32, 0, stream>>>(d_in, nranks, count, d_out);
    count_launch();
    return (int)cudaGetLastError();
}

struct DeviceScratch {
    std::mutex mu;
    std::condition_variable cv;
    cudaMemPool_t pool = nullptr;
    size_t limit = 0, in_use = 0, peak = 0, total = 0;
    bool ready = false;
};
static DeviceScratch g_scratch[64];

static size_t default_scratch_bytes(size_t total) { return total / 20 * 11; }

static int scratch_init(DeviceScratch& ds, int dev) {
    if (ds.ready) return 0;
    size_t free_b = 0, total_b = 0;
    cudaError_t e = cudaMemGetInfo(&free_b, &total_b);
    if (e != cudaSuccess) return (int)e;
    size_t limit = default_scratch_bytes(total_b);
    if (const char* v = getenv("SNARKVM_B200_SCRATCH_LIMIT_GB")) { long g = atol(v); if (g >= 1) limit = (size_t)g << 30; }
    cudaMemPoolProps props = {};
    props.allocType = cudaMemAllocationTypePinned;
    props.handleTypes = cudaMemHandleTypeNone;
    props.location.type = cudaMemLocationTypeDevice;
    props.location.id = dev;
    if ((e = cudaMemPoolCreate(&ds.pool, &props)) != cudaSuccess) return (int)e;
    uint64_t thr = limit;
    cudaMemPoolSetAttribute(ds.pool, cudaMemPoolAttrReleaseThreshold, &thr);
    ds.limit = limit;
    ds.total = total_b;
    ds.ready = true;
    return 0;
}
static int scratch_group_budget(size_t* out) {
    int dev = 0;
    cudaError_t e = cudaGetDevice(&dev);
    if (e != cudaSuccess) return (int)e;
    DeviceScratch& ds = g_scratch[dev & 63];
    std::lock_guard<std::mutex> lock(ds.mu);
    int rc = scratch_init(ds, dev);
    if (rc) return rc;
    *out = default_scratch_bytes(ds.total);
    return 0;
}
int pool_alloc_raw(void** p, size_t bytes, cudaStream_t stream) {
    int dev = 0;
    cudaError_t e = cudaGetDevice(&dev);
    if (e != cudaSuccess) return (int)e;
    DeviceScratch& ds = g_scratch[dev & 63];
    {
        std::lock_guard<std::mutex> lock(ds.mu);
        int rc = scratch_init(ds, dev);
        if (rc) return rc;
    }
    return (int)cudaMallocFromPoolAsync(p, bytes ? bytes : 16, ds.pool, stream);
}
struct ScratchLease { DeviceScratch* ds; size_t bytes; };
static void CUDART_CB scratch_release_cb(void* p) {
    ScratchLease* l = (ScratchLease*)p;
    { std::lock_guard<std::mutex> lock(l->ds->mu); l->ds->in_use -= l->bytes; }
    l->ds->cv.notify_all();
    delete l;
}
static int scratch_acquire(void** out, size_t bytes, cudaStream_t stream, DeviceScratch** ds_out) {
    int dev = 0;
    cudaError_t e = cudaGetDevice(&dev);
    if (e != cudaSuccess) return (int)e;
    DeviceScratch& ds = g_scratch[dev & 63];
    {
        std::unique_lock<std::mutex> lock(ds.mu);
        int rc = scratch_init(ds, dev);
        if (rc) return rc;
        ds.cv.wait(lock, [&] { return ds.in_use == 0 || ds.in_use + bytes <= ds.limit; });
        ds.in_use += bytes;
        if (ds.in_use > ds.peak) ds.peak = ds.in_use;
    }
    e = cudaMallocFromPoolAsync(out, bytes, ds.pool, stream);
    if (e != cudaSuccess) {
        { std::lock_guard<std::mutex> lock(ds.mu); ds.in_use -= bytes; }
        ds.cv.notify_all();
        return (int)e;
    }
    *ds_out = &ds;
    return 0;
}
static void scratch_release(void* p, size_t bytes, cudaStream_t stream, DeviceScratch* ds) {
    cudaFreeAsync(p, stream);
    ScratchLease* l = new ScratchLease{ds, bytes};
    if (cudaLaunchHostFunc(stream, scratch_release_cb, l) != cudaSuccess) scratch_release_cb(l);
}
int msm_scratch_stats(size_t* limit, size_t* in_use, size_t* peak) {
    int dev = 0;
    cudaError_t e = cudaGetDevice(&dev);
    if (e != cudaSuccess) return (int)e;
    DeviceScratch& ds = g_scratch[dev & 63];
    std::lock_guard<std::mutex> lock(ds.mu);
    if (limit) *limit = ds.limit;
    if (in_use) *in_use = ds.in_use;
    if (peak) *peak = ds.peak;
    return 0;
}

int msm_set_scratch_limit(size_t bytes) {
    int dev = 0;
    cudaError_t e = cudaGetDevice(&dev);
    if (e != cudaSuccess) return (int)e;
    if (bytes == 0) return (int)cudaErrorInvalidValue;
    DeviceScratch& ds = g_scratch[dev & 63];
    {
        std::lock_guard<std::mutex> lock(ds.mu);
        int rc = scratch_init(ds, dev);
        if (rc) return rc;
        ds.limit = bytes;
        ds.peak = ds.in_use;
        uint64_t thr = bytes;
        cudaMemPoolSetAttribute(ds.pool, cudaMemPoolAttrReleaseThreshold, &thr);
    }
    ds.cv.notify_all();
    return 0;
}

struct Arena {
    uint8_t* base = nullptr;
    size_t off = 0;
    template <class T> T* take(size_t count) {
        T* p = base ? (T*)(base + off) : nullptr;
        off += (count * sizeof(T) + 255) & ~(size_t)255;
        return p;
    }
};

int msm_core(uint32_t* d_window_sums, uint32_t* d_flags, const MsmPlan& plan, const MsmBases* bases, int nbases,
             const uint32_t* table, size_t table_n, const MsmSegment* segs, int nsegs, int njobs, cudaStream_t stream) {
    int rc = 0;
    const bool flat = table != nullptr;
    const uint32_t sets_per_job = flat ? 1u : (uint32_t)plan.nwin;
    if (njobs < 1 || nsegs < 1 || (!flat && nbases < 1)) return (int)cudaErrorInvalidValue;
    const uint64_t nsets64 = (uint64_t)njobs * sets_per_job;
    const uint64_t TB64 = nsets64 * plan.nbuckets;
    if (TB64 >= (1ull << 31)) return (int)cudaErrorInvalidValue;
    const uint32_t nsets = (uint32_t)nsets64, TB = (uint32_t)TB64;
    size_t total_scalars = 0, total_bases = 0;
    std::vector<size_t> job_n((size_t)njobs, 0);
    for (int i = 0; i < nbases; i++) {
        if (bases[i].stride < 104 || (bases[i].stride & 7)) return (int)cudaErrorInvalidValue;
        total_bases += bases[i].n;
    }
    for (int i = 0; i < nsegs; i++) {
        if (segs[i].job >= (uint32_t)njobs) return (int)cudaErrorInvalidValue;
        if (flat ? (segs[i].base0 != 0 || segs[i].n > table_n) : ((size_t)segs[i].base0 + segs[i].n > total_bases)) return (int)cudaErrorInvalidValue;
        total_scalars += segs[i].n;
        job_n[segs[i].job] += segs[i].n;
    }
    size_t max_job_n = 0;
    for (size_t v : job_n) if (v > max_job_n) max_job_n = v;
    const size_t max_entries = total_scalars * (size_t)plan.nwin;
    if (total_scalars == 0 || total_bases >= (1ull << 31) || max_entries >= (1ull << 32)) return (int)cudaErrorInvalidValue;
    if (flat && table_n * (size_t)plan.nwin >= (1ull << 31)) return (int)cudaErrorInvalidValue;
    const int levels = plan.levels;
    const size_t set_cap = flat ? max_job_n * (size_t)plan.nwin : max_job_n;
    bool records = levels > 0;
    if (const char* e = getenv("SNARKVM_B200_MSM_RECORDS")) records = records && atoi(e) != 0;
    if (const char* e = getenv("SNARKVM_B200_MSM_PAIR_V1")) { if (atoi(e) != 0) records = false; }
    std::vector<const uint8_t*> seg_points((size_t)nsegs, nullptr);
    std::vector<size_t> seg_stride((size_t)nsegs, 0);
    if (records && !flat) {
        for (int i = 0; i < nsegs; i++) {
            size_t off = 0; bool found = segs[i].n == 0;
            for (int k = 0; k < nbases && !found; k++) {
                if (segs[i].base0 >= off && (size_t)segs[i].base0 + segs[i].n <= off + bases[k].n) {
                    seg_points[i] = (const uint8_t*)bases[k].d_points + ((size_t)segs[i].base0 - off) * bases[k].stride;
                    seg_stride[i] = bases[k].stride;
                    found = true;
                }
                off += bases[k].n;
            }
            if (!found) return (int)cudaErrorInvalidValue;
        }
    }

    size_t budget = 0;
    if ((rc = scratch_group_budget(&budget)) != 0) return rc;
    if (const char* e = getenv("SNARKVM_B200_MSM_SCRATCH_GB")) { long v = atol(e); if (v >= 1) budget = (size_t)v << 30; }
    if (const char* e = getenv("SNARKVM_B200_MSM_SCRATCH_MB")) { long v = atol(e); if (v >= 1) budget = (size_t)v << 20; }
    uint32_t gw = nsets;
    if (levels > 0) {
        size_t per_set = set_cap * (size_t)(records ? 180 : 104) + 1;
        size_t fit = budget / per_set;
        if (fit < 1) fit = 1;
        if (fit < gw) {
            const uint32_t ngroups = (uint32_t)((nsets + fit - 1) / fit);
            gw = (nsets + ngroups - 1) / ngroups;
        }
    }
    const uint32_t TBg = gw * plan.nbuckets;
    size_t entries_g = set_cap * (size_t)gw;
    if (entries_g > max_entries) entries_g = max_entries;
    if (records && entries_g >= 0x7fffffffull) return (int)cudaErrorInvalidValue;
    bool warp_reduce = plan.nbuckets <= 1024u;
    bool acc_g8 = levels == 0 && max_entries <= 100000;
    int quad_path = 1;
    if (const char* e = getenv("SNARKVM_B200_MSM_QUAD")) quad_path = atoi(e);
    bool acc_q8 = quad_path != 0 && warp_reduce && levels == 0 && (size_t)TB + max_entries / 32 <= 1100;
    if (const char* e = getenv("SNARKVM_B200_MSM_WARP_PATH")) { if (atoi(e) == 0) { warp_reduce = false; acc_g8 = false; acc_q8 = false; } }
    bool quad_tail_large = true;
    if (plan.nbuckets < 16384u) quad_tail_large = false;
    if (const char* e = getenv("SNARKVM_B200_MSM_QUAD_TAIL")) quad_tail_large = atoi(e) != 0;
    const bool quad_fold = quad_path != 0 && warp_reduce && levels == 0;
    const bool large_hot = quad_path != 0 && quad_tail_large && !warp_reduce;
    const uint32_t hot_keep = large_hot ? 1u : 32u;
    if (acc_q8) acc_g8 = false;
    uint32_t item_cap = plan.cap;
    if (acc_g8) {
        size_t per_lane = max_entries / 300000 + 1;
        if (per_lane < 4) per_lane = 4;
        if (per_lane > 16) per_lane = 16;
        item_cap = (uint32_t)per_lane * 8u;
        if (const char* e = getenv("SNARKVM_B200_MSM_CAP")) { long v = atol(e); if (v >= 1) item_cap = (uint32_t)v; }
    }
    if (acc_q8) {
        size_t cap16 = ((set_cap + 15) / 16 + 7) & ~(size_t)7;
        item_cap = (uint32_t)(cap16 < 32 ? 32 : cap16);
    } else if (quad_fold && !acc_g8 && max_entries <= 900000) {
        item_cap = max_entries <= 150000 ? 4 : 8;
        if (const char* e = getenv("SNARKVM_B200_MSM_CAP")) { long v = atol(e); if (v >= 1) item_cap = (uint32_t)v; }
    }
    const bool small_cap = quad_fold && !acc_g8 && !acc_q8 && item_cap != plan.cap;
    const size_t max_items = (size_t)TBg + entries_g / (item_cap < plan.cap ? item_cap : plan.cap) + 1;
    const size_t hot_max = max_items / 2 + 1;
    const size_t dense_cap_a = entries_g / 2 + TBg + 1, dense_cap_b = entries_g / 4 + 2 * (size_t)TBg + 1;

    size_t pair_waves = 0;
    if (const char* e = getenv("SNARKVM_B200_MSM_PAIR_WAVES")) { long v = atol(e); if (v >= 1) pair_waves = (size_t)v; }
    bool pair_v1 = false;
    if (const char* e = getenv("SNARKVM_B200_MSM_PAIR_V1")) pair_v1 = atoi(e) != 0;
    int pair_minb = 4;
    if (const char* e = getenv("SNARKVM_B200_MSM_PAIR_MINB")) { int v = atoi(e); if (v == 3 || v == 4) pair_minb = v; }
    int sm_count = 0;
    {
        static std::once_flag smem_once[64];
        int dev = 0; cudaGetDevice(&dev);
        std::call_once(smem_once[dev & 63], [] {
            cudaFuncSetAttribute(k_pair_level2<true, 4>, cudaFuncAttributeMaxDynamicSharedMemorySize, PAIR2_SMEM);
            cudaFuncSetAttribute(k_pair_level2<false, 4>, cudaFuncAttributeMaxDynamicSharedMemorySize, PAIR2_SMEM);
            cudaFuncSetAttribute(k_pair_level2<true, 3>, cudaFuncAttributeMaxDynamicSharedMemorySize, PAIR2_SMEM);
            cudaFuncSetAttribute(k_pair_level2<false, 3>, cudaFuncAttributeMaxDynamicSharedMemorySize, PAIR2_SMEM);
        });
        const cudaError_t e = cudaDeviceGetAttribute(&sm_count, cudaDevAttrMultiProcessorCount, dev);
        if (e != cudaSuccess) return (int)e;
    }
    const uint32_t chunk = plan.nbuckets < 16u ? plan.nbuckets : 16u;
    const uint32_t tree = 8;
    const uint32_t chunks_per_set = plan.nbuckets / chunk;

    size_t cub_bytes = 0;
    if (cub::DeviceScan::ExclusiveSum(nullptr, cub_bytes, (uint32_t*)nullptr, (uint32_t*)nullptr, (int)(TB + 1), stream) != cudaSuccess) return (int)cudaErrorUnknown;
    if (cub_bytes < 16) cub_bytes = 16;

    uint32_t *hist, *bucket_start, *cursors, *items, *item_start, *items2, *sorted, *partial, *partial2, *red_a, *red_b;
    uint32_t *off_a = nullptr, *off_b = nullptr, *dense_a = nullptr, *dense_b = nullptr, *prefix = nullptr, *dense_bases = nullptr, *sm_slots = nullptr;
    uint32_t *dense0 = nullptr, *cnt_tmp = nullptr, *hot_dev = nullptr;
    uint2* desc = nullptr;
    uint8_t* cub_tmp;
    Arena ar;
    auto layout = [&](Arena& a) {
        hist = a.take<uint32_t>((size_t)TB + 1);
        bucket_start = a.take<uint32_t>((size_t)TB + 1);
        cursors = a.take<uint32_t>((size_t)TB + 1);
        items = a.take<uint32_t>((size_t)TBg + 1);
        item_start = a.take<uint32_t>((size_t)TBg + 1);
        items2 = a.take<uint32_t>((size_t)TBg + 1);
        sorted = records ? nullptr : a.take<uint32_t>(max_entries);
        cnt_tmp = a.take<uint32_t>((size_t)TBg + 1);
        partial = a.take<uint32_t>(max_items * XYZZ_WORDS);
        partial2 = a.take<uint32_t>(((quad_fold || large_hot) ? max_items : (size_t)TBg + max_items / 32 + 2) * XYZZ_WORDS);
        hot_dev = a.take<uint32_t>(hot_max + 2);
        red_a = a.take<uint32_t>((size_t)gw * (2 * chunks_per_set > 2 * ((plan.nbuckets + 7u) / 8u) ? 2 * chunks_per_set : 2 * ((plan.nbuckets + 7u) / 8u)) * XYZZ_WORDS);
        red_b = a.take<uint32_t>((size_t)gw * (chunks_per_set / tree + 1 > 2 * ((plan.nbuckets + 63u) / 64u) + 2 ? chunks_per_set / tree + 1 : 2 * ((plan.nbuckets + 63u) / 64u) + 2) * XYZZ_WORDS);
        cub_tmp = a.take<uint8_t>(cub_bytes);
        if (!flat && !records) dense_bases = a.take<uint32_t>(total_bases * (size_t)BASE_WORDS);
        if (records) dense0 = a.take<uint32_t>(entries_g * (size_t)DENSE_WORDS);
        if (levels > 0) {
            off_a = a.take<uint32_t>((size_t)TBg + 1);
            off_b = a.take<uint32_t>((size_t)TBg + 1);
            dense_a = a.take<uint32_t>(dense_cap_a * DENSE_WORDS);
            if (levels > 1) dense_b = records && dense_cap_b <= entries_g ? dense0 : a.take<uint32_t>(dense_cap_b * DENSE_WORDS);
            prefix = a.take<uint32_t>(dense_cap_a * 12);
            desc = a.take<uint2>(dense_cap_a);
            sm_slots = a.take<uint32_t>(256);
        }
    };
    layout(ar);
    const size_t scratch_bytes = ar.off;
    void* block = nullptr;
    DeviceScratch* ds = nullptr;
    if ((rc = scratch_acquire(&block, scratch_bytes, stream, &ds)) != 0) return rc;
    ar.base = (uint8_t*)block; ar.off = 0;
    layout(ar);

    CUDA_TRY(cudaMemsetAsync(hist, 0, (size_t)(TB + 1) * 4, stream));
    if (sm_slots) CUDA_TRY(cudaMemsetAsync(sm_slots, 0, 256 * 4, stream));
    if (quad_fold) CUDA_TRY(cudaMemsetAsync(hot_dev, 0, 4, stream));
    {
        {
            ProfScope sort_scope(PROF_MSM_SORT, stream);
            for (int pass = 0; pass < (records ? 1 : 2); pass++) {
                for (int i = 0; i < nsegs; i++) {
                    const MsmSegment& sg = segs[i];
                    if (sg.n == 0) continue;
                    const unsigned grid = (unsigned)((sg.n + 255) / 256);
                    const uint32_t slot_base = sg.job * sets_per_job * plan.nbuckets;
                    const uint32_t* sc = (const uint32_t*)sg.d_scalars;
                    const size_t fl = flat ? table_n : 0;
                    if (pass == 0) {
                        if (sg.mont) k_digits<false, true><<<grid, 256, 0, stream>>>(sc, sg.n, plan.c, plan.nwin, plan.nbuckets, hist, nullptr, fl, slot_base, sg.base0, d_flags);
                        else k_digits<false, false><<<grid, 256, 0, stream>>>(sc, sg.n, plan.c, plan.nwin, plan.nbuckets, hist, nullptr, fl, slot_base, sg.base0, d_flags);
                    } else {
                        if (sg.mont) k_digits<true, true><<<grid, 256, 0, stream>>>(sc, sg.n, plan.c, plan.nwin, plan.nbuckets, cursors, sorted, fl, slot_base, sg.base0, d_flags);
                        else k_digits<true, false><<<grid, 256, 0, stream>>>(sc, sg.n, plan.c, plan.nwin, plan.nbuckets, cursors, sorted, fl, slot_base, sg.base0, d_flags);
                    }
                    count_launch();
                }
                if (pass == 0) {
                    CUDA_TRY(cub::DeviceScan::ExclusiveSum(cub_tmp, cub_bytes, hist, bucket_start, (int)(TB + 1), stream));
                    CUDA_TRY(cudaMemcpyAsync(cursors, bucket_start, (size_t)(TB + 1) * 4, cudaMemcpyDeviceToDevice, stream));
                    count_launch(2);
                }
            }
        }
        const uint32_t* gather_src = flat ? table : dense_bases;
        if (!flat && !records) {
            ProfScope acc_scope(PROF_MSM_ACCUMULATE, stream);
            size_t at = 0;
            for (int i = 0; i < nbases; i++) {
                if (bases[i].n == 0) continue;
                k_densify_bases<<<(unsigned)((bases[i].n + 255) / 256), 256, 0, stream>>>((const uint8_t*)bases[i].d_points, bases[i].stride, bases[i].n,
                                                                                        dense_bases + at * BASE_WORDS);
                count_launch();
                at += bases[i].n;
            }
        }
        for (uint32_t w0 = 0; w0 < nsets; w0 += gw) {
            const uint32_t wn = nsets - w0 < gw ? nsets - w0 : gw;
            const uint32_t tb = wn * plan.nbuckets;
            const uint32_t* bs = bucket_start + (size_t)w0 * plan.nbuckets;
            size_t entries = set_cap * (size_t)wn;
            if (entries > max_entries) entries = max_entries;
            if (large_hot) CUDA_TRY(cudaMemsetAsync(hot_dev, 0, 4, stream));
            size_t items_bound = 1;
            size_t items_launched = 1;
            const uint32_t* final_partial = nullptr;
            const uint32_t* final_start = nullptr;
            if (levels == 0) {
                const uint32_t cap = (acc_g8 || acc_q8 || small_cap) ? item_cap : plan.cap;
                k_items_per_bucket<<<(tb + 256) / 256, 256, 0, stream>>>(hist + (size_t)w0 * plan.nbuckets, items, tb, cap, (quad_fold || large_hot) ? hot_dev : nullptr, (uint32_t)hot_max, hot_keep);
                CUDA_TRY(cub::DeviceScan::ExclusiveSum(cub_tmp, cub_bytes, items, item_start, (int)(tb + 1), stream));
                count_launch(2);
                const size_t group_items = (size_t)tb + entries / cap + 1;
                items_bound = set_cap / cap + 1;
                items_launched = group_items;
                ProfScope acc_scope(PROF_MSM_ACCUMULATE, stream);
                if (acc_q8) {
                    k_bucket_accumulate_q8<<<(unsigned)((group_items * 32 + 127) / 128), 128, 0, stream>>>(gather_src, sorted, bs, item_start, tb, cap, partial);
                    items_bound = 1;
                } else if (acc_g8)
                    k_bucket_accumulate_g8<<<(unsigned)((group_items * ACC_G + 127) / 128), 128, 0, stream>>>(gather_src, sorted, bs, item_start, tb, cap, partial);
                else
                    k_bucket_accumulate<<<(unsigned)((group_items + MSM_ACC_THREADS - 1) / MSM_ACC_THREADS), MSM_ACC_THREADS, 0, stream>>>(
                        gather_src, sorted, bs, item_start, tb, cap, partial);
                count_launch();
            } else {
                if (records) {
                    ProfScope sort_scope(PROF_MSM_SORT, stream);
                    for (int i = 0; i < nsegs; i++) {
                        const MsmSegment& sg = segs[i];
                        if (sg.n == 0) continue;
                        const int64_t first = (int64_t)sg.job * sets_per_job;
                        int w_lo, w_hi;
                        if (flat) {
                            if (first < (int64_t)w0 || first >= (int64_t)w0 + wn) continue;
                            w_lo = 0; w_hi = plan.nwin;
                        } else {
                            const int64_t lo_w = (int64_t)w0 - first, hi_w = (int64_t)w0 + wn - first;
                            w_lo = lo_w < 0 ? 0 : (int)lo_w; w_hi = hi_w > plan.nwin ? plan.nwin : (int)hi_w;
                            if (w_lo >= w_hi) continue;
                        }
                        const unsigned grid = (unsigned)((sg.n + 255) / 256);
                        const uint32_t slot_base = sg.job * sets_per_job * plan.nbuckets;
                        const uint32_t* sc = (const uint32_t*)sg.d_scalars;
                        if (flat) {
                            if (sg.mont) k_scatter_records<true, true><<<grid, 256, 0, stream>>>(sc, sg.n, nullptr, 0, table, table_n, plan.c, plan.nbuckets, cursors, slot_base, w_lo, w_hi, bs, (uint4*)dense0);
                            else k_scatter_records<false, true><<<grid, 256, 0, stream>>>(sc, sg.n, nullptr, 0, table, table_n, plan.c, plan.nbuckets, cursors, slot_base, w_lo, w_hi, bs, (uint4*)dense0);
                        } else {
                            if (sg.mont) k_scatter_records<true, false><<<grid, 256, 0, stream>>>(sc, sg.n, seg_points[i], seg_stride[i], nullptr, 0, plan.c, plan.nbuckets, cursors, slot_base, w_lo, w_hi, bs, (uint4*)dense0);
                            else k_scatter_records<false, false><<<grid, 256, 0, stream>>>(sc, sg.n, seg_points[i], seg_stride[i], nullptr, 0, plan.c, plan.nbuckets, cursors, slot_base, w_lo, w_hi, bs, (uint4*)dense0);
                        }
                        count_launch();
                    }
                }
                ProfScope acc_scope(PROF_MSM_ACCUMULATE, stream);
                const uint32_t* off_in = bs;
                uint32_t* off_bufs[2] = {off_a, off_b};
                uint32_t* dense_bufs[2] = {dense_a, dense_b};
                const uint32_t* dense_in = records ? dense0 : nullptr;
                size_t bound = entries;
                for (int l = 0; l < levels; l++) {
                    uint32_t* off_out = off_bufs[l & 1];
                    uint32_t* dense_out = dense_bufs[l & 1];
                    k_halve_counts<<<(tb + 256) / 256, 256, 0, stream>>>(off_in, cnt_tmp, tb);
                    CUDA_TRY(cub::DeviceScan::ExclusiveSum(cub_tmp, cub_bytes, cnt_tmp, off_out, (int)(tb + 1), stream));
                    bound = bound / 2 + tb;
                    const size_t wave = (size_t)sm_count * (pair_v1 ? 4 : pair_minb) * 128;
                    size_t waves = (bound + 1024 * wave - 1) / (1024 * wave);
                    if (pair_waves) waves = pair_waves;
                    size_t T = (bound + waves * wave - 1) / (waves * wave);
                    const size_t nthreads = (bound + T - 1) / T;
                    const unsigned lgrid = (unsigned)((nthreads + 127) / 128);
                    if (pair_v1) {
                        if (l == 0 && !records)
                            k_pair_level<true><<<lgrid, 128, 0, stream>>>(gather_src, sorted, nullptr, off_in, off_out, tb, (uint32_t)T, prefix, dense_out);
                        else
                            k_pair_level<false><<<lgrid, 128, 0, stream>>>(nullptr, nullptr, dense_in, off_in, off_out, tb, (uint32_t)T, prefix, dense_out);
                    } else {
                        const unsigned dgrid = (unsigned)((bound + 255) / 256);
                        if (l == 0 && !records) {
                            k_pair_desc<true><<<dgrid, 256, 0, stream>>>(sorted, off_in, off_out, tb, desc, nullptr);
                            if (pair_minb == 3) k_pair_level2<true, 3><<<lgrid, 128, PAIR2_SMEM, stream>>>(gather_src, desc, off_out + tb, (uint32_t)T, prefix, dense_out, sm_slots);
                            else k_pair_level2<true, 4><<<lgrid, 128, PAIR2_SMEM, stream>>>(gather_src, desc, off_out + tb, (uint32_t)T, prefix, dense_out, sm_slots);
                        } else {
                            k_pair_desc<false><<<dgrid, 256, 0, stream>>>(nullptr, off_in, off_out, tb, desc, l == 0 ? bs : nullptr);
                            if (pair_minb == 3) k_pair_level2<false, 3><<<lgrid, 128, PAIR2_SMEM, stream>>>(dense_in, desc, off_out + tb, (uint32_t)T, prefix, dense_out, sm_slots);
                            else k_pair_level2<false, 4><<<lgrid, 128, PAIR2_SMEM, stream>>>(dense_in, desc, off_out + tb, (uint32_t)T, prefix, dense_out, sm_slots);
                        }
                        count_launch(1);
                    }
                    count_launch(3);
                    off_in = off_out;
                    dense_in = dense_out;
                }
                k_items_from_offsets<<<(tb + 256) / 256, 256, 0, stream>>>(off_in, items, tb, plan.cap, large_hot ? hot_dev : nullptr, (uint32_t)hot_max, hot_keep);
                CUDA_TRY(cub::DeviceScan::ExclusiveSum(cub_tmp, cub_bytes, items, item_start, (int)(tb + 1), stream));
                const size_t group_items = (size_t)tb + bound / plan.cap + 1;
                items_bound = ((set_cap >> levels) + 1) / plan.cap + 1;
                items_launched = group_items;
                k_bucket_accumulate_dense<<<(unsigned)((group_items + MSM_ACC_THREADS - 1) / MSM_ACC_THREADS), MSM_ACC_THREADS, 0, stream>>>(
                    dense_in, off_in, item_start, tb, plan.cap, partial);
                count_launch(3);
            }
            ProfScope red_scope(PROF_MSM_REDUCE, stream);
            int quad_rounds = 0;
            if (quad_fold) {
                size_t worst = acc_q8 ? 1 : items_bound;
                const uint32_t* p_in = partial; uint32_t* p_out = partial2;
                while (worst > 32) {
                    k_fold_hot_quad<<<(unsigned)sm_count * 8, 128, 0, stream>>>(p_in, item_start, hot_dev, (uint32_t)hot_max, (uint32_t)quad_rounds, 32u, p_out);
                    count_launch();
                    worst = (worst + 31) / 32;
                    quad_rounds++;
                    const uint32_t* t1 = p_in; p_in = p_out; p_out = (uint32_t*)t1;
                }
                final_partial = partial; final_start = item_start;
            } else if (large_hot) {
                size_t worst = items_bound;
                const uint32_t* p_in = partial; uint32_t* p_out = partial2;
                while (worst > 1) {
                    k_fold_hot_quad<<<(unsigned)sm_count * 8, 128, 0, stream>>>(p_in, item_start, hot_dev, (uint32_t)hot_max, (uint32_t)quad_rounds, 1u, p_out);
                    count_launch();
                    worst = (worst + 31) / 32;
                    quad_rounds++;
                    const uint32_t* t1 = p_in; p_in = p_out; p_out = (uint32_t*)t1;
                }
                final_partial = partial; final_start = item_start;
            } else {
                size_t worst = items_bound;
                size_t total_bound = items_launched;
                uint32_t* p_in = partial; uint32_t* p_out = partial2;
                uint32_t* st_in = item_start; uint32_t* st_out = items2;
                while (worst > 1) {
                    k_group_counts<<<(tb + 256) / 256, 256, 0, stream>>>(st_in, cnt_tmp, tb);
                    CUDA_TRY(cub::DeviceScan::ExclusiveSum(cub_tmp, cub_bytes, cnt_tmp, st_out, (int)(tb + 1), stream));
                    const size_t out_bound = (size_t)tb + total_bound / 32 + 1;
                    total_bound = out_bound;
                    k_partial_group_sum<<<(unsigned)((out_bound + 127) / 128), 128, 0, stream>>>(p_in, st_in, st_out, tb, p_out);
                    count_launch(3);
                    worst = (worst + 31) / 32;
                    uint32_t* t1 = p_in; p_in = p_out; p_out = t1;
                    uint32_t* t2 = st_in; st_in = st_out; st_out = t2;
                }
                final_partial = p_in; final_start = st_in;
            }
            uint32_t* group_sums = d_window_sums + (size_t)w0 * XYZZ_WORDS;
            if (warp_reduce && quad_path != 0) {
                const uint32_t qchunks = (plan.nbuckets + 7u) / 8u;
                k_bucket_reduce_quad<<<(wn * qchunks * 32u + 127u) / 128u, 128, 0, stream>>>(final_partial, quad_fold ? partial2 : final_partial, final_start,
                                                                                              quad_rounds, plan.nbuckets, qchunks, wn, red_a);
                const uint32_t* ent = red_a;
                uint32_t m = qchunks;
                int lgw = 3;
                if (m > 64u) {
                    const uint32_t groups = (m + 7u) / 8u;
                    k_combine_level_quad<<<(wn * groups * 32u + 127u) / 128u, 128, 0, stream>>>(ent, m, wn, lgw, red_b);
                    count_launch();
                    ent = red_b; m = groups; lgw += 3;
                }
                k_window_combine_quad<<<wn, 32u * ((m + 7u) / 8u), 0, stream>>>(ent, m, lgw, group_sums);
                count_launch(2);
                continue;
            }
            if (warp_reduce) {
                const uint32_t wchunks = (plan.nbuckets + 31u) / 32u;
                k_bucket_reduce_warp<<<(wn * wchunks * 32u + 127u) / 128u, 128, 0, stream>>>(final_partial, final_start, plan.nbuckets, wchunks, wn, red_a);
                k_window_combine_warp<<<wn, 32, 0, stream>>>(red_a, wchunks, group_sums);
                count_launch(2);
                continue;
            }
            const uint32_t nthreads = chunks_per_set * wn;
            if (quad_path != 0 && quad_tail_large) {
                k_bucket_reduce<true><<<(nthreads + 127) / 128, 128, 0, stream>>>(final_partial, final_start, plan.nbuckets, chunk, chunks_per_set, wn, red_a,
                                                                                    partial2, large_hot ? quad_rounds : 0);
                count_launch(1);
                const uint32_t* ent = red_a;
                uint32_t* other = red_b;
                uint32_t m = chunks_per_set;
                int lgw = 0;
                while ((1u << lgw) < chunk) lgw++;
                while (m > 64u) {
                    const uint32_t groups = (m + 7u) / 8u;
                    if ((size_t)wn * groups >= 2048)
                        k_combine_level_quadseq<<<(unsigned)(((size_t)wn * groups * 4 + 127) / 128), 128, 0, stream>>>(ent, m, wn, lgw, other);
                    else
                        k_combine_level_quad<<<(wn * groups * 32u + 127u) / 128u, 128, 0, stream>>>(ent, m, wn, lgw, other);
                    count_launch();
                    uint32_t* done = other; other = (uint32_t*)ent; ent = done;
                    m = groups; lgw += 3;
                }
                k_window_combine_quad<<<wn, 32u * ((m + 7u) / 8u), 0, stream>>>(ent, m, lgw, group_sums);
                count_launch();
                continue;
            }
            k_bucket_reduce<false><<<(nthreads + 127) / 128, 128, 0, stream>>>(final_partial, final_start, plan.nbuckets, chunk, chunks_per_set, wn, red_a);
            count_launch(1);
            uint32_t per_row = chunks_per_set;
            const uint32_t* src = red_a;
            uint32_t* bufs[2] = {red_b, red_a};
            int which = 0;
            while (per_row > 1) {
                uint32_t out_per_row = (per_row + tree - 1) / tree;
                uint32_t* target = out_per_row == 1 ? group_sums : bufs[which];
                uint32_t nt = out_per_row * wn;
                k_group_sum<<<(nt + 127) / 128, 128, 0, stream>>>(src, per_row, tree, out_per_row, wn, target);
                count_launch();
                src = target; which ^= 1; per_row = out_per_row;
            }
            if (chunks_per_set == 1)
                CUDA_TRY(cudaMemcpyAsync(group_sums, red_a, (size_t)wn * XYZZ_WORDS * 4, cudaMemcpyDeviceToDevice, stream));
        }
        CUDA_TRY(cudaGetLastError());
    }
done:
    scratch_release(block, scratch_bytes, stream, ds);
    return rc;
}

size_t msm_scan_bytes(size_t count) {
    size_t bytes = 0;
    cub::DeviceScan::ExclusiveSum(nullptr, bytes, (uint32_t*)nullptr, (uint32_t*)nullptr, (int)count);
    return bytes < 16 ? 16 : bytes;
}
int msm_exclusive_scan(void* tmp, size_t tmp_bytes, const uint32_t* in, uint32_t* out, size_t count, cudaStream_t stream) {
    count_launch(2);
    return (int)cub::DeviceScan::ExclusiveSum(tmp, tmp_bytes, in, out, (int)count, stream);
}
int msm_sort_indices(const MsmPlan& plan, const void* d_scalars, size_t n, int mont, uint32_t* hist, uint32_t* bucket_start, uint32_t* cursors,
                     uint32_t* sorted, void* cub_tmp, size_t cub_bytes, uint32_t* d_flags, cudaStream_t stream) {
    const uint32_t TB = (uint32_t)plan.nwin * plan.nbuckets;
    int rc = (int)cudaMemsetAsync(hist, 0, (size_t)(TB + 1) * 4, stream);
    if (rc) return rc;
    const unsigned grid = (unsigned)((n + 255) / 256);
    const uint32_t* sc = (const uint32_t*)d_scalars;
    if (mont) k_digits<false, true><<<grid, 256, 0, stream>>>(sc, n, plan.c, plan.nwin, plan.nbuckets, hist, nullptr, 0, 0u, 0u, d_flags);
    else k_digits<false, false><<<grid, 256, 0, stream>>>(sc, n, plan.c, plan.nwin, plan.nbuckets, hist, nullptr, 0, 0u, 0u, d_flags);
    if ((rc = msm_exclusive_scan(cub_tmp, cub_bytes, hist, bucket_start, (size_t)TB + 1, stream)) != 0) return rc;
    if ((rc = (int)cudaMemcpyAsync(cursors, bucket_start, (size_t)(TB + 1) * 4, cudaMemcpyDeviceToDevice, stream)) != 0) return rc;
    if (mont) k_digits<true, true><<<grid, 256, 0, stream>>>(sc, n, plan.c, plan.nwin, plan.nbuckets, cursors, sorted, 0, 0u, 0u, d_flags);
    else k_digits<true, false><<<grid, 256, 0, stream>>>(sc, n, plan.c, plan.nwin, plan.nbuckets, cursors, sorted, 0, 0u, 0u, d_flags);
    count_launch(3);
    return (int)cudaGetLastError();
}
int msm_items_per_bucket(const uint32_t* hist, uint32_t* items, uint32_t total_buckets, uint32_t cap, cudaStream_t stream) {
    k_items_per_bucket<<<(total_buckets + 256) / 256, 256, 0, stream>>>(hist, items, total_buckets, cap, nullptr, 0u, 32u);
    count_launch();
    return (int)cudaGetLastError();
}
int msm_group_counts(const uint32_t* start_in, uint32_t* cnt_out, uint32_t total_buckets, cudaStream_t stream) {
    k_group_counts<<<(total_buckets + 256) / 256, 256, 0, stream>>>(start_in, cnt_out, total_buckets);
    count_launch();
    return (int)cudaGetLastError();
}

int msm_window_sums_device(uint32_t* d_window_sums, uint32_t* d_flags, const MsmPlan& plan, const void* d_points, size_t stride,
                           const void* d_scalars, size_t npoints, cudaStream_t stream) {
    MsmBases b{d_points, stride, npoints};
    MsmSegment sg{d_scalars, npoints, 0u, 0u, 0};
    return msm_core(d_window_sums, d_flags, plan, &b, 1, nullptr, 0, &sg, 1, 1, stream);
}

MsmPlan msm_make_plan_precomputed(size_t npoints) {
    MsmPlan p;
    int lg = ceil_log2(npoints < 2 ? 2 : npoints);
    int c = lg >= 22 ? 20 : lg >= 20 ? 17 : lg >= 8 ? lg - 2 : 6;
    if (const char* e = getenv("SNARKVM_B200_MSM_PRE_C")) { int v = atoi(e); if (v >= 2 && v <= 24) c = v; }
    p.c = c;
    p.nwin = 253 / c + 1;
    p.nbuckets = 1u << (c - 1);
    size_t total = npoints * (size_t)p.nwin;
    size_t cap = total / 300000 + 1;
    if (cap < 16) cap = 16;
    p.cap = (uint32_t)cap;
    int levels = lg >= 24 ? 5 : lg >= 22 ? 4 : lg >= 20 ? 3 : 1;
    if (const char* e = getenv("SNARKVM_B200_MSM_PRE_LEVELS")) { int v = atoi(e); if (v >= 1 && v <= 16) levels = v; }
    p.levels = levels;
    return p;
}

int msm_precompute_tables_device(uint32_t* d_table, const MsmPlan& plan, const void* d_points, size_t stride, size_t npoints,
                                 cudaStream_t stream) {
    if (stride < 104 || (stride & 7) || npoints == 0) return (int)cudaErrorInvalidValue;
    k_precompute_tables<<<(unsigned)((npoints + 127) / 128), 128, 0, stream>>>((const uint8_t*)d_points, stride, npoints, plan.c, plan.nwin, d_table);
    count_launch();
    return (int)cudaGetLastError();
}

int msm_precomputed_sum_device(uint32_t* d_sum, uint32_t* d_flags, const MsmPlan& plan, const uint32_t* d_table, size_t table_n, const void* d_scalars,
                               size_t nscalars, int mont, cudaStream_t stream) {
    MsmSegment sg{d_scalars, nscalars, 0u, 0u, mont};
    return msm_core(d_sum, d_flags, plan, nullptr, 0, d_table, table_n, &sg, 1, 1, stream);
}

FF_DEV uint64_t splitmix64(uint64_t x) {
    x += 0x9E3779B97F4A7C15ull;
    x = (x ^ (x >> 30)) * 0xBF58476D1CE4E5B9ull;
    x = (x ^ (x >> 27)) * 0x94D049BB133111EBull;
    return x ^ (x >> 31);
}
__constant__ uint32_t G1_GEN_X[12] = {0xec301b95u, 0x1042a645u, 0xc1060f28u, 0x5a990780u, 0xa9007a5bu, 0x684a8ab3u,
                                      0x257ba63fu, 0x1c35a184u, 0xfea8e32eu, 0xb2b2abd2u, 0x23fb2017u, 0x017df3a2u};
__constant__ uint32_t G1_GEN_Y[12] = {0xe2801ab9u, 0xbc5a1ae8u, 0xcbfe13b0u, 0xd4f3c861u, 0x4e949f13u, 0xecdd5ffcu,
                                      0x7503667du, 0x8f87199bu, 0x7dc4fe1cu, 0x0f0b1b83u, 0x053eaabeu, 0x004bcc7eu};

__global__ void __launch_bounds__(128) k_generate_bases(uint8_t* points, size_t n, size_t stride, uint64_t seed) {
    size_t i = (size_t)blockIdx.x * blockDim.x + threadIdx.x;
    if (i >= n) return;
    uint64_t k = splitmix64(seed ^ splitmix64((uint64_t)i));
    if (k == 0) k = 1;
    AffinePoint g;
#pragma unroll
    for (int j = 0; j < 12; j++) { g.x.v[j] = G1_GEN_X[j]; g.y.v[j] = G1_GEN_Y[j]; }
    g.inf = false;
    XYZZ acc = XYZZ::infinity();
    bool started = false;
    for (int b = 63; b >= 0; b--) {
        if (started) acc.dbl();
        if ((k >> b) & 1ull) { acc.add_affine(g, false); started = true; }
    }
    store_affine(points, stride, i, acc.to_affine());
}

__global__ void __launch_bounds__(128) k_srs_decode(const uint8_t* __restrict__ in, size_t n, uint8_t* __restrict__ out, size_t stride,
                                                     uint32_t* __restrict__ invalid) {
    size_t i = (size_t)blockIdx.x * blockDim.x + threadIdx.x;
    if (i >= n) return;
    const uint32_t* w = reinterpret_cast<const uint32_t*>(in + i * 96);
    Fq x, y;
#pragma unroll
    for (int k = 0; k < 12; k++) { x.v[k] = __ldg(w + k); y.v[k] = __ldg(w + 12 + k); }
    const uint32_t flags = y.v[11] >> 30;
    y.v[11] &= 0x3fffffffu;
    AffinePoint a;
    bool bad = false;
    if (flags & 1u) {
        a.x = Fq::zero(); a.y = Fq::one(); a.inf = true;
        bad = (flags & 2u) != 0u;
    } else {
        Fq tx = x, ty = y;
        tx.final_sub(); ty.final_sub();
        bad = (tx != x) || (ty != y);
        a.x = x.to_mont(); a.y = y.to_mont(); a.inf = false;
        Fq lhs = a.y.sqr(), rhs = a.x.sqr() * a.x + Fq::one();
        bad = bad || (lhs != rhs);
    }
    if (bad) atomicAdd(invalid, 1u);
    store_affine(out, stride, i, a);
}
int srs_decode_device(void* d_out, size_t stride, const void* d_in, size_t npoints, uint32_t* d_invalid, cudaStream_t stream) {
    if (stride < 104 || (stride & 7) || ((uintptr_t)d_in & 3)) return (int)cudaErrorInvalidValue;
    cudaError_t e = cudaMemsetAsync(d_invalid, 0, 4, stream);
    if (e != cudaSuccess) return (int)e;
    if (npoints == 0) return 0;
    k_srs_decode<<<(unsigned)((npoints + 127) / 128), 128, 0, stream>>>((const uint8_t*)d_in, npoints, (uint8_t*)d_out, stride, d_invalid);
    count_launch();
    return (int)cudaGetLastError();
}

__global__ void __launch_bounds__(128) k_selftest_coop(uint32_t nwarps, uint64_t seed, uint32_t* __restrict__ mismatches) {
    const uint32_t w = (blockIdx.x * blockDim.x + threadIdx.x) >> 5;
    const int lane = threadIdx.x & 31;
    if (w >= nwarps) return;
    Fq a, b;
#pragma unroll
    for (int k = 0; k < 12; k += 2) {
        uint64_t ra = splitmix64(seed + 0x100ull * w + (uint64_t)k), rb = splitmix64(~seed + 0x100ull * w + (uint64_t)k);
        a.v[k] = (uint32_t)ra; a.v[k + 1] = (uint32_t)(ra >> 32); b.v[k] = (uint32_t)rb; b.v[k + 1] = (uint32_t)(rb >> 32);
    }
    a.v[11] &= 0x00ffffffu; b.v[11] &= 0x00ffffffu;
    if (w == 0) a = Fq::zero();
    if (w == 1) a = Fq::one();
    if (w == 2) a = Fq::zero() - Fq::one();
    if (w == 3) { a = Fq::zero() - Fq::one(); b = a; }
    if (w == 4) {
#pragma unroll
        for (int k = 0; k < 12; k++) a.v[k] = k < 11 ? 0xffffffffu : 0u;
        b = Fq::one();
    }
    const uint32_t p = coop_mod_limb<FqParams>(lane);
    uint32_t al = 0u, bl = 0u;
#pragma unroll
    for (int k = 0; k < 12; k++) { if (lane == k) { al = a.v[k]; bl = b.v[k]; } }
    const uint32_t prod = coop_mul<FqParams>(al, bl, p, lane);
    const Fq want = a * b;
    uint32_t wl = 0u;
#pragma unroll
    for (int k = 0; k < 12; k++) if (lane == k) wl = want.v[k];
    bool bad = prod != wl;
    const Fq inv = coop_inverse<FqParams>(a);
    const Fq one = inv * a;
    if (a.is_zero()) bad = bad || !inv.is_zero();
    else bad = bad || (one != Fq::one()) || (inv != a.inverse());
    {
        const uint32_t t = blockIdx.x * blockDim.x + threadIdx.x;
        Fq x, y;
        Fr u, v;
#pragma unroll
        for (int k = 0; k < 12; k += 2) {
            uint64_t rx = splitmix64(seed * 3 + 0x1000ull * t + (uint64_t)k), ry = splitmix64(~seed * 5 + 0x1000ull * t + (uint64_t)k);
            x.v[k] = (uint32_t)rx; x.v[k + 1] = (uint32_t)(rx >> 32); y.v[k] = (uint32_t)ry; y.v[k + 1] = (uint32_t)(ry >> 32);
        }
        x.v[11] &= 0x00ffffffu; y.v[11] &= 0x00ffffffu;
        if ((t & 7u) == 1u) { for (int k = 0; k < 6; k++) { y.v[k] = x.v[k + 6]; y.v[k + 6] = x.v[k]; } y.v[11] &= 0x00ffffffu; y.v[5] = x.v[11]; }
        if ((t & 7u) == 2u) { for (int k = 0; k < 6; k++) x.v[k + 6] = x.v[k]; x.v[11] &= 0x00ffffffu; }
        if (t == 8u) x = Fq::zero();
        if (t == 9u) y = Fq::one();
        if (t == 10u) { x = Fq::zero() - Fq::one(); y = x; }
        if (t == 11u) { x = Fq::zero() - Fq::one(); }
#pragma unroll
        for (int k = 0; k < 8; k++) { u.v[k] = x.v[k] ^ y.v[11 - k]; v.v[k] = y.v[k] + x.v[11 - k]; }
        u.v[7] &= 0x0fffffffu; v.v[7] &= 0x0fffffffu;
        if ((t & 7u) == 3u) { for (int k = 0; k < 4; k++) v.v[k + 4] = v.v[k]; v.v[7] &= 0x0fffffffu; }
        if (t == 12u) { u = Fr::zero() - Fr::one(); v = u; }
        bool bad2 = Fq::mul_karatsuba(x, y) != Fq::mul_inline(x, y) || Fq::mul_karatsuba(x, x) != Fq::sqr_inline(x);
        bad2 = bad2 || Fr::mul_karatsuba(u, v) != Fr::mul_inline(u, v) || Fr::mul_karatsuba(v, v) != Fr::sqr_inline(v);
        bad = bad || bad2;
    }
    if (__any_sync(0xffffffffu, bad) && lane == 0) atomicAdd(mismatches, 1u);
}
int selftest_coop_device(uint32_t nwarps, uint64_t seed, uint32_t* d_mismatches, cudaStream_t stream) {
    cudaError_t e = cudaMemsetAsync(d_mismatches, 0, 4, stream);
    if (e != cudaSuccess) return (int)e;
// ... 121 lines not shown
```

snarkvm_b200/csrc/msm.cuh:

```cuda
#pragma once
#include <cstddef>
#include <cstdint>
#include <cuda_runtime.h>

namespace b200 {

struct MsmPlan {
    int c;
    int nwin;
    uint32_t nbuckets;
    uint32_t cap;
    int levels;
};

MsmPlan msm_make_plan(size_t npoints);
MsmPlan msm_make_plan_batch(size_t max_n, size_t total_n);

struct MsmBases {
    const void* d_points;
    size_t stride, n;
};
struct MsmSegment {
    const void* d_scalars;
    size_t n;
    uint32_t base0;
    uint32_t job;
    int mont;
};
int msm_core(uint32_t* d_window_sums, uint32_t* d_flags, const MsmPlan& plan, const MsmBases* bases, int nbases,
             const uint32_t* table, size_t table_n, const MsmSegment* segs, int nsegs, int njobs, cudaStream_t stream);

int msm_window_sums_device(uint32_t* d_window_sums, uint32_t* d_flags, const MsmPlan& plan, const void* d_points, size_t stride,
                           const void* d_scalars, size_t npoints, cudaStream_t stream);

MsmPlan msm_make_plan_precomputed(size_t npoints);
int msm_precompute_tables_device(uint32_t* d_table, const MsmPlan& plan, const void* d_points, size_t stride, size_t npoints, cudaStream_t stream);
int msm_precomputed_sum_device(uint32_t* d_sum, uint32_t* d_flags, const MsmPlan& plan, const uint32_t* d_table, size_t table_n, const void* d_scalars,
                               size_t nscalars, int mont, cudaStream_t stream);

size_t msm_scan_bytes(size_t count);
int msm_exclusive_scan(void* tmp, size_t tmp_bytes, const uint32_t* in, uint32_t* out, size_t count, cudaStream_t stream);
int msm_sort_indices(const MsmPlan& plan, const void* d_scalars, size_t n, int mont, uint32_t* hist, uint32_t* bucket_start, uint32_t* cursors,
                     uint32_t* sorted, void* cub_tmp, size_t cub_bytes, uint32_t* d_flags, cudaStream_t stream);
int msm_items_per_bucket(const uint32_t* hist, uint32_t* items, uint32_t total_buckets, uint32_t cap, cudaStream_t stream);
int msm_group_counts(const uint32_t* start_in, uint32_t* cnt_out, uint32_t total_buckets, cudaStream_t stream);

int msm_g2_window_sums_device(uint32_t* d_window_sums, uint32_t* d_flags, const MsmPlan& plan, const void* d_points, size_t stride,
                              const void* d_scalars, size_t npoints, int mont, cudaStream_t stream);
int msm_generate_bases_g2_device(void* d_points, size_t npoints, size_t stride, uint64_t seed, cudaStream_t stream);

int msm_generate_bases_device(void* d_points, size_t npoints, size_t stride, uint64_t seed, cudaStream_t stream);
int msm_generator_mul_device(void* d_points, size_t npoints, size_t stride, const void* d_scalars, cudaStream_t stream);

int srs_decode_device(void* d_out, size_t stride, const void* d_in, size_t npoints, uint32_t* d_invalid, cudaStream_t stream);

int selftest_coop_device(uint32_t nwarps, uint64_t seed, uint32_t* d_mismatches, cudaStream_t stream);
int test_field_op_msm(int field, int op, void* d_out, const void* d_a, const void* d_b, size_t n, cudaStream_t stream);
int test_field_op_ntt(int field, int op, void* d_out, const void* d_a, const void* d_b, size_t n, cudaStream_t stream);
int test_curve_op_device(int group, int op, void* d_out, const void* d_a, const void* d_b, const uint32_t* d_k, size_t n, cudaStream_t stream);

int xyzz_sum_ranks_device(uint32_t* d_out, const uint32_t* d_in, int nranks, int count, cudaStream_t stream);

int pool_alloc_raw(void** p, size_t bytes, cudaStream_t stream);
template <class T> inline cudaError_t pool_alloc(T** p, size_t bytes, cudaStream_t stream) { return (cudaError_t)pool_alloc_raw((void**)p, bytes, stream); }
int msm_scratch_stats(size_t* limit, size_t* in_use, size_t* peak);
int msm_set_scratch_limit(size_t bytes);

uint64_t launch_count();
void count_launch(int n = 1);

enum ProfKind { PROF_MSM_SORT = 0, PROF_MSM_ACCUMULATE = 1, PROF_MSM_REDUCE = 2, PROF_NTT_PASS = 3, PROF_KINDS = 4 };
void prof_enable(bool on);
bool prof_enabled();
struct ProfScope {
    cudaEvent_t a = nullptr, b = nullptr;
    cudaStream_t stream;
    int kind;
    ProfScope(int kind, cudaStream_t stream);
    ~ProfScope();
};
int prof_collect(int kind, double* total_ms, uint64_t* count);

}
```

Measured before the change: 127.0 million.

## Add mixed-width MSM windows with a wider top window split into bucket sets

Adds support for a non-uniform window plan where the last window is wider than the others, represented as extra bucket sets with digit offsets. For large inputs (log2 n ≥ 24) with no env overrides, the default plan uses 13 windows of 18 bits plus a 20-bit top window. This aims to reduce the number of windows and the bucket-reduction and Horner work. The combine and reduce kernels add offset multiples of running sums, and the host Horner step folds in the extra top sets. Pair-level kernels now derive their per-lane count from the device-side total instead of a host bound.

```diff
diff --git a/snarkvm_b200/csrc/api.cu b/snarkvm_b200/csrc/api.cu
--- a/snarkvm_b200/csrc/api.cu
+++ b/snarkvm_b200/csrc/api.cu
@@ -118,7 +118,7 @@
 
 int msm_jobs_impl(void* out144s, const MsmPlan& plan, const MsmBases* bases, int nbases, const uint32_t* table, size_t table_n,
                   const MsmSegment* segs, int nsegs, int njobs, cudaStream_t stream) {
-    const size_t sets = table ? 1 : (size_t)plan.nwin;
+    const size_t sets = table ? 1 : (size_t)plan.nsets;
     const size_t npts = (size_t)njobs * sets;
     uint32_t* d_buf = nullptr;
     cudaError_t e = pool_alloc(&d_buf, npts * 192 + 256, stream);
@@ -143,7 +143,7 @@
     memcpy(&flags, sums.data() + npts, 4);
     if (flags & 1u) return (int)cudaErrorInvalidValue;
     auto finish = [&](int j) {
-        host::Xyzz total = table ? sums[(size_t)j] : host::horner_windows(sums.data() + (size_t)j * sets, plan.nwin, plan.c);
+        host::Xyzz total = table ? sums[(size_t)j] : host::horner_windows(sums.data() + (size_t)j * sets, plan.nwin, plan.c, plan.top_sets());
         host::xyzz_to_normalised_projective(total, (uint64_t*)((uint8_t*)out144s + (size_t)j * 144));
     };
     if (njobs <= 2) { for (int j = 0; j < njobs; j++) finish(j); }
@@ -614,7 +614,7 @@
         std::vector<size_t> sum_off{0};
         for (int k = 0; k < chunks; k++) {
             plans.push_back(msm_make_plan(bounds[k + 1] - bounds[k]));
-            sum_off.push_back(sum_off.back() + (size_t)plans.back().nwin);
+            sum_off.push_back(sum_off.back() + (size_t)plans.back().nsets);
         }
         std::vector<cudaEvent_t> ev((size_t)chunks + 1, nullptr);
         for (auto& e : ev) if (rc == 0) rc = (int)cudaEventCreateWithFlags(&e, cudaEventDisableTiming);
@@ -647,7 +647,7 @@
         }
         if (rc == 0) {
             host::Xyzz total = host::xyzz_inf();
-            for (int k = 0; k < chunks; k++) host::xyzz_add(total, host::horner_windows(sums.data() + sum_off[k], plans[k].nwin, plans[k].c));
+            for (int k = 0; k < chunks; k++) host::xyzz_add(total, host::horner_windows(sums.data() + sum_off[k], plans[k].nwin, plans[k].c, plans[k].top_sets()));
             host::xyzz_to_normalised_projective(total, result);
         }
     }
@@ -670,14 +670,14 @@
 }
 
 int snarkvm_b200_msm_plan(size_t npoints, int* c, int* nwin, uint32_t* cap) {
-    MsmPlan p = msm_make_plan(npoints);
+    MsmPlan p = msm_make_plan(npoints, false);
     if (c) *c = p.c;
     if (nwin) *nwin = p.nwin;
     if (cap) *cap = p.cap;
     return 0;
 }
 
-int snarkvm_b200_msm_plan_levels(size_t npoints) { return msm_make_plan(npoints).levels; }
+int snarkvm_b200_msm_plan_levels(size_t npoints) { return msm_make_plan(npoints, false).levels; }
 
 int snarkvm_b200_msm_device(void* out144, const void* d_points, size_t npoints, const void* d_scalars, size_t stride,
                             void* stream) {
@@ -736,7 +736,7 @@
                                              size_t npoints, const void* d_scalars, size_t stride, void* stream_v) {
     if (!d_window_sums || stride < 104 || (stride & 7) || plan_npoints == 0 || npoints > plan_npoints) return (int)cudaErrorInvalidValue;
     cudaStream_t stream = (cudaStream_t)stream_v;
-    MsmPlan plan = msm_make_plan(plan_npoints);
+    MsmPlan plan = msm_make_plan(plan_npoints, false);
     uint32_t* own_flags = nullptr;
     int rc = 0;
     if (!d_flags) { rc = (int)pool_alloc(&own_flags, 256, stream); if (rc) return rc; d_flags = own_flags; }
@@ -751,7 +751,7 @@
                                       const void* h_scalars, size_t stride, void* stream_v) {
     if (!d_window_sums || stride < 104 || (stride & 7) || plan_npoints == 0 || npoints > plan_npoints) return (int)cudaErrorInvalidValue;
     cudaStream_t stream = (cudaStream_t)stream_v;
-    MsmPlan plan = msm_make_plan(plan_npoints);
+    MsmPlan plan = msm_make_plan(plan_npoints, false);
     uint32_t* own_flags = nullptr;
     int rc = 0;
     if (!d_flags) { rc = (int)pool_alloc(&own_flags, 256, stream); if (rc) return rc; d_flags = own_flags; }
@@ -979,7 +979,7 @@
     if (!out288) return (int)cudaErrorInvalidValue;
     if (npoints == 0) { host::Xyzz2 inf = host::xyzz_inf_t<host::Fq2>(); host::xyzz_to_normalised_projective(inf, (uint64_t*)out288); return 0; }
     if (!d_points || !d_scalars || stride < 200 || (stride & 7)) return (int)cudaErrorInvalidValue;
-    MsmPlan plan = msm_make_plan(npoints);
+    MsmPlan plan = msm_make_plan(npoints, false);
     const size_t nw = (size_t)plan.nwin;
     uint32_t* d_buf = nullptr;
     cudaError_t e = pool_alloc(&d_buf, nw * 384 + 256, stream);
diff --git a/snarkvm_b200/csrc/host_ec.hpp b/snarkvm_b200/csrc/host_ec.hpp
--- a/snarkvm_b200/csrc/host_ec.hpp
+++ b/snarkvm_b200/csrc/host_ec.hpp
@@ -176,11 +176,12 @@
     if (fq_is_zero(Z)) p = xyzz_inf();
     return p;
 }
-template <class F> inline XyzzT<F> horner_windows(const XyzzT<F>* sums, int nwin, int c) {
+template <class F> inline XyzzT<F> horner_windows(const XyzzT<F>* sums, int nwin, int c, int top_sets = 1) {
     XyzzT<F> total = xyzz_inf_t<F>();
     for (int w = nwin - 1; w >= 0; w--) {
         for (int k = 0; k < c; k++) xyzz_dbl(total);
         xyzz_add(total, sums[w]);
+        if (w == nwin - 1) for (int s = 1; s < top_sets; s++) xyzz_add(total, sums[w + s]);
     }
     return total;
 }
diff --git a/snarkvm_b200/csrc/msm.cu b/snarkvm_b200/csrc/msm.cu
--- a/snarkvm_b200/csrc/msm.cu
+++ b/snarkvm_b200/csrc/msm.cu
@@ -8,6 +8,7 @@
 #include <vector>
 #include <cstdio>
 #include <cstdlib>
+#include <cstring>
 #include <cub/device/device_scan.cuh>
 
 #define FF_CALL_MUL 1
@@ -69,14 +70,47 @@
     return l;
 }
 
-MsmPlan msm_make_plan(size_t npoints) {
+static bool parse_window_widths(const char* s, MsmPlan& p) {
+    std::vector<int> w;
+    while (*s) {
+        char* end = nullptr;
+        long v = strtol(s, &end, 10);
+        if (end == s || v < 2 || v > 24) return false;
+        long k = 1;
+        s = end;
+        if (*s == '*') { k = strtol(s + 1, &end, 10); if (end == s + 1 || k < 1 || k > 128) return false; s = end; }
+        for (long i = 0; i < k && w.size() <= 128; i++) w.push_back((int)v);
+        if (*s == ',') s++;
+        else if (*s) return false;
+    }
+    if (w.size() < 2 || w.size() > 128) return false;
+    for (size_t i = 1; i + 1 < w.size(); i++) if (w[i] != w[0]) return false;
+    const int c = w[0], nwin = (int)w.size(), c_top = w.back();
+    if ((nwin - 1) * c >= 253 || (nwin - 1) * c + c_top < 254) return false;
+    const int top_sets = c_top > c ? 1 << (c_top - c) : 1;
+    if (top_sets > 64) return false;
+    p.c = c; p.nwin = nwin; p.c_top = c_top; p.nsets = nwin - 1 + top_sets;
+    p.nbuckets = 1u << (c - 1);
+    return true;
+}
+
+MsmPlan msm_make_plan(size_t npoints, bool mixed) {
     MsmPlan p;
     int lg = plan_log2(npoints);
     int c = lg <= 8 ? 4 : lg <= 12 ? lg - 4 : lg <= 18 ? 11 : lg == 19 ? 13 : lg == 20 ? 15 : lg <= 22 ? 16 : 17;
-    if (const char* e = getenv("SNARKVM_B200_MSM_C")) { int v = atoi(e); if (v >= 2 && v <= 24) c = v; }
+    const char* ec = getenv("SNARKVM_B200_MSM_C");
+    if (ec) { int v = atoi(ec); if (v >= 2 && v <= 24) c = v; }
     p.c = c;
     p.nwin = 253 / c + 1;
     p.nbuckets = 1u << (c - 1);
+    p.c_top = c;
+    p.nsets = p.nwin;
+    if (mixed) {
+        const char* ew = getenv("SNARKVM_B200_MSM_WINDOWS");
+        if (ew && *ew && strcmp(ew, "0") != 0) parse_window_widths(ew, p);
+        else if (!ew && !ec && lg >= 24) parse_window_widths("18*13,20", p);
+        c = p.c;
+    }
     size_t total = npoints * (size_t)p.nwin;
     size_t cap = total / 300000 + 1;
     if (cap < 16) cap = 16;
@@ -107,7 +141,7 @@
 }
 
 template <bool SCATTER, bool MONT>
-__global__ void __launch_bounds__(256) k_digits(const uint32_t* __restrict__ scalars, size_t n, int c, int nwin,
+__global__ void __launch_bounds__(256) k_digits(const uint32_t* __restrict__ scalars, size_t n, int c_low, int c_top, int nwin,
                                                 uint32_t nbuckets, uint32_t* __restrict__ counters ,
                                                 uint32_t* __restrict__ sorted, size_t flat ,
                                                 uint32_t slot_base, uint32_t index_base, uint32_t* __restrict__ flags) {
@@ -128,14 +162,15 @@
         for (int k = 0; k < 8; k++) s[k] = x.v[k];
     }
     if (!SCATTER && (s[7] >> 29)) atomicOr(flags, 1u);
-    const uint32_t half = 1u << (c - 1);
     uint32_t carry = 0;
     for (int w = 0; w < nwin; w++) {
-        int bit = w * c;
+        const int c = w == nwin - 1 ? c_top : c_low;
+        int bit = w * c_low;
         int wi = bit >> 5, sh = bit & 31;
         uint32_t lo = 0, hi = 0;
 #pragma unroll
         for (int k = 0; k < 8; k++) { if (k == wi) lo = s[k]; if (k == wi + 1) hi = s[k]; }
+        const uint32_t half = 1u << (c - 1);
         uint32_t raw = (__funnelshift_r(lo, hi, sh) & ((1u << c) - 1u)) + carry;
         uint32_t neg = raw > half ? 1u : 0u;
         uint32_t mag = neg ? (1u << c) - raw : raw;
@@ -179,7 +214,8 @@
 static constexpr uint32_t REC_NONE = 0xffffffffu;
 template <bool MONT, bool FLAT>
 __global__ void __launch_bounds__(256) k_scatter_records(const uint32_t* __restrict__ scalars, size_t n, const uint8_t* __restrict__ points,
-                                                         size_t stride, const uint32_t* __restrict__ table, size_t table_n, int c, uint32_t nbuckets,
+                                                         size_t stride, const uint32_t* __restrict__ table, size_t table_n, int c_low, int c_top,
+                                                         int nwin, uint32_t nbuckets,
                                                          uint32_t* __restrict__ cursors, uint32_t slot_base, int w_lo, int w_hi,
                                                          const uint32_t* __restrict__ pos_base_ptr, uint4* __restrict__ dense0) {
     __shared__ uint4 sh_rec[256 * 9];
@@ -219,13 +255,14 @@
             stage(pt.x, pt.y, pt.inf);
         }
     }
-    const uint32_t half = 1u << (c - 1);
     uint32_t carry = 0;
     for (int w = 0; w < w_hi; w++) {
-        const int bit = w * c, wi = bit >> 5, sh = bit & 31;
+        const int c = w == nwin - 1 ? c_top : c_low;
+        const int bit = w * c_low, wi = bit >> 5, sh = bit & 31;
         uint32_t lo = 0, hi = 0;
 #pragma unroll
         for (int k = 0; k < 8; k++) { if (k == wi) lo = s[k]; if (k == wi + 1) hi = s[k]; }
+        const uint32_t half = 1u << (c - 1);
         const uint32_t raw = (__funnelshift_r(lo, hi, sh) & ((1u << c) - 1u)) + carry;
         const uint32_t neg = raw > half ? 1u : 0u;
         const uint32_t mag = neg ? (1u << c) - raw : raw;
@@ -505,8 +542,9 @@
 template <bool GATHER, int MINB>
 __global__ void __launch_bounds__(PAIR_THREADS, MINB) k_pair_level2(const uint32_t* __restrict__ records ,
                                                          const uint2* __restrict__ desc, const uint32_t* __restrict__ total_ptr,
-                                                         uint32_t T, uint32_t* __restrict__ prefix, uint32_t* __restrict__ dense_out,
+                                                         uint32_t T_bound, uint32_t* __restrict__ prefix, uint32_t* __restrict__ dense_out,
                                                          uint32_t* __restrict__ sm_slots) {
+    (void)T_bound;
     extern __shared__ uint4 pair2_smem[];
     __shared__ uint32_t sh_slot;
     uint32_t* sh_inv = reinterpret_cast<uint32_t*>(pair2_smem);
@@ -520,6 +558,8 @@
     __syncthreads();
     const int inv_warp = (int)(sh_slot & 3u);
     const uint32_t total = __ldg(total_ptr);
+    const uint64_t lanes = (uint64_t)gridDim.x * PAIR_THREADS;
+    const uint32_t T = total > lanes ? (uint32_t)((total + lanes - 1) / lanes) : 1u;
     const uint64_t w0_64 = ((uint64_t)blockIdx.x * (PAIR_THREADS / 32) + (uint32_t)warp) * 32ull * T + (uint32_t)lane;
     uint32_t nv = 0;
     if (w0_64 < total) { const uint64_t left = (total - w0_64 + 31) / 32; nv = left < T ? (uint32_t)left : T; }
@@ -700,11 +740,24 @@
     return s;
 }
 
+struct SetOffsets {
+    uint32_t set0, per_job, top_first, nbuckets;
+    FF_DEV uint32_t of(uint32_t set) const {
+        const uint32_t s = (set0 + set) % per_job;
+        return s > top_first ? (s - top_first) * nbuckets : 0u;
+    }
+};
+static SetOffsets set_offsets(const MsmPlan& plan, bool flat, uint32_t set0) {
+    if (flat) return SetOffsets{0u, 1u, 0u, 0u};
+    return SetOffsets{set0, (uint32_t)plan.nsets, (uint32_t)plan.nwin - 1u, plan.nbuckets};
+}
+
 template <bool PAIRS>
 __global__ void __launch_bounds__(128) k_bucket_reduce(const uint32_t* __restrict__ partial, const uint32_t* __restrict__ item_start,
                                                         uint32_t nbuckets, uint32_t chunk, uint32_t chunks_per_window,
                                                         uint32_t nwin, uint32_t* __restrict__ out,
-                                                        const uint32_t* __restrict__ partial_b = nullptr, int folds = 0) {
+                                                        const uint32_t* __restrict__ partial_b = nullptr, int folds = 0,
+                                                        SetOffsets so = SetOffsets{0u, 1u, 0u, 0u}) {
     uint32_t t = blockIdx.x * blockDim.x + threadIdx.x;
     if (t >= chunks_per_window * nwin) return;
     uint32_t w = t / chunks_per_window, j = t % chunks_per_window;
@@ -727,7 +780,8 @@
         running.store(out + ((size_t)t * 2 + 1) * XYZZ_WORDS);
         return;
     }
-    if (lo != 0u) acc.add(running.mul_u32(lo));
+    const uint32_t lo_off = lo + so.of(w);
+    if (lo_off != 0u) acc.add(running.mul_u32(lo_off));
     acc.store(out + (size_t)t * XYZZ_WORDS);
 }
 
@@ -815,7 +869,8 @@
         run.store(out + ((size_t)warp * 2 + 1) * XYZZ_WORDS);
     }
 }
-__global__ void __launch_bounds__(32) k_window_combine_warp(const uint32_t* __restrict__ in, uint32_t chunks, uint32_t* __restrict__ out) {
+__global__ void __launch_bounds__(32) k_window_combine_warp(const uint32_t* __restrict__ in, uint32_t chunks, uint32_t* __restrict__ out,
+                                                            SetOffsets so) {
     const uint32_t set = blockIdx.x, lane = threadIdx.x;
     XYZZ a = XYZZ::infinity(), r = XYZZ::infinity();
     if (lane < chunks) {
@@ -830,6 +885,8 @@
         for (int k = 0; k < 5; k++) w.dbl();
         total.add(w);
     }
+    const uint32_t off = so.of(set);
+    if (off != 0u) { const XYZZ run = warp_sum_xyzz(r); total.add(run.mul_u32(off)); }
     if (lane == 0) total.store(out + (size_t)set * XYZZ_WORDS);
 }
 
@@ -992,8 +1049,18 @@
         store_xyzz_plain(out + ((size_t)quad * 2 + 1) * XYZZ_WORDS, running);
     }
 }
+FF_DEV XYZZ quad_mul_u32(const XYZZ& a, uint32_t k, const Quad& Q) {
+    XYZZ r = XYZZ::infinity();
+#pragma unroll 1
+    for (int b = 31 - __clz(k); b >= 0; b--) {
+        r = quad_dbl(r, Q);
+        if ((k >> b) & 1u) r = quad_add(r, a, Q);
+    }
+    return r;
+}
 static constexpr int COMBINE_QUAD_MAX_WARPS = 8;
-__global__ void __launch_bounds__(32 * COMBINE_QUAD_MAX_WARPS) k_window_combine_quad(const uint32_t* __restrict__ in, uint32_t m0, int lgw0, uint32_t* __restrict__ out) {
+__global__ void __launch_bounds__(32 * COMBINE_QUAD_MAX_WARPS) k_window_combine_quad(const uint32_t* __restrict__ in, uint32_t m0, int lgw0, uint32_t* __restrict__ out,
+                                                                                      SetOffsets so) {
     __shared__ __align__(16) uint32_t sm[COMBINE_QUAD_MAX_WARPS][2][XYZZ_WORDS];
     const uint32_t set = blockIdx.x, warp = threadIdx.x >> 5;
     const Quad Q = Quad::here();
@@ -1008,7 +1075,11 @@
             XYZZ a = XYZZ::infinity(), r = XYZZ::infinity();
             if (j < m) { a = load_xyzz_plain(src + (size_t)j * 2 * XYZZ_WORDS); r = load_xyzz_plain(src + ((size_t)j * 2 + 1) * XYZZ_WORDS); }
             A = combine_fold_quad(a, r, lgw, Q, run);
-            if (groups == 1u && (threadIdx.x & 31u) == 0u) A.store(out + (size_t)set * XYZZ_WORDS);
+            if (groups == 1u) {
+                const uint32_t off = so.of(set);
+                if (off != 0u && Q.slot == 0) A = quad_add(A, quad_mul_u32(run, off, Q), Q);
+                if ((threadIdx.x & 31u) == 0u) A.store(out + (size_t)set * XYZZ_WORDS);
+            }
         }
         if (groups == 1u) break;
         __syncthreads();
@@ -1166,8 +1237,10 @@
              const uint32_t* table, size_t table_n, const MsmSegment* segs, int nsegs, int njobs, cudaStream_t stream) {
     int rc = 0;
     const bool flat = table != nullptr;
-    const uint32_t sets_per_job = flat ? 1u : (uint32_t)plan.nwin;
+    const uint32_t sets_per_job = flat ? 1u : (uint32_t)plan.nsets;
+    const uint32_t wins_per_job = flat ? 1u : (uint32_t)plan.nwin;
     if (njobs < 1 || nsegs < 1 || (!flat && nbases < 1)) return (int)cudaErrorInvalidValue;
+    if (plan.nsets < plan.nwin || plan.nwin < 1 || (flat && plan.nsets != plan.nwin)) return (int)cudaErrorInvalidValue;
     const uint64_t nsets64 = (uint64_t)njobs * sets_per_job;
     const uint64_t TB64 = nsets64 * plan.nbuckets;
     if (TB64 >= (1ull << 31)) return (int)cudaErrorInvalidValue;
@@ -1215,18 +1288,25 @@
     if ((rc = scratch_group_budget(&budget)) != 0) return rc;
     if (const char* e = getenv("SNARKVM_B200_MSM_SCRATCH_GB")) { long v = atol(e); if (v >= 1) budget = (size_t)v << 30; }
     if (const char* e = getenv("SNARKVM_B200_MSM_SCRATCH_MB")) { long v = atol(e); if (v >= 1) budget = (size_t)v << 20; }
-    uint32_t gw = nsets;
+    const uint32_t nwins = (uint32_t)njobs * wins_per_job;
+    uint32_t gu = nwins;
     if (levels > 0) {
-        size_t per_set = set_cap * (size_t)(records ? 180 : 104) + 1;
-        size_t fit = budget / per_set;
+        size_t per_win = set_cap * (size_t)(records ? 180 : 104) + 1;
+        size_t fit = budget / per_win;
         if (fit < 1) fit = 1;
-        if (fit < gw) {
-            const uint32_t ngroups = (uint32_t)((nsets + fit - 1) / fit);
-            gw = (nsets + ngroups - 1) / ngroups;
-        }
+        if (fit < gu) {
+            const uint32_t ngroups = (uint32_t)((nwins + fit - 1) / fit);
+            gu = (nwins + ngroups - 1) / ngroups;
+        }
+    }
+    auto set_of = [&](uint32_t u) { return (u / wins_per_job) * sets_per_job + u % wins_per_job; };
+    uint32_t gw = 0;
+    for (uint32_t u0 = 0; u0 < nwins; u0 += gu) {
+        const uint32_t s = set_of(u0 + (nwins - u0 < gu ? nwins - u0 : gu)) - set_of(u0);
+        if (s > gw) gw = s;
     }
     const uint32_t TBg = gw * plan.nbuckets;
-    size_t entries_g = set_cap * (size_t)gw;
+    size_t entries_g = set_cap * (size_t)gu;
     if (entries_g > max_entries) entries_g = max_entries;
     if (records && entries_g >= 0x7fffffffull) return (int)cudaErrorInvalidValue;
     bool warp_reduce = plan.nbuckets <= 1024u;
@@ -1345,11 +1425,11 @@
                     const uint32_t* sc = (const uint32_t*)sg.d_scalars;
                     const size_t fl = flat ? table_n : 0;
                     if (pass == 0) {
-                        if (sg.mont) k_digits<false, true><<<grid, 256, 0, stream>>>(sc, sg.n, plan.c, plan.nwin, plan.nbuckets, hist, nullptr, fl, slot_base, sg.base0, d_flags);
-                        else k_digits<false, false><<<grid, 256, 0, stream>>>(sc, sg.n, plan.c, plan.nwin, plan.nbuckets, hist, nullptr, fl, slot_base, sg.base0, d_flags);
+                        if (sg.mont) k_digits<false, true><<<grid, 256, 0, stream>>>(sc, sg.n, plan.c, plan.c_top, plan.nwin, plan.nbuckets, hist, nullptr, fl, slot_base, sg.base0, d_flags);
+                        else k_digits<false, false><<<grid, 256, 0, stream>>>(sc, sg.n, plan.c, plan.c_top, plan.nwin, plan.nbuckets, hist, nullptr, fl, slot_base, sg.base0, d_flags);
                     } else {
-                        if (sg.mont) k_digits<true, true><<<grid, 256, 0, stream>>>(sc, sg.n, plan.c, plan.nwin, plan.nbuckets, cursors, sorted, fl, slot_base, sg.base0, d_flags);
-                        else k_digits<true, false><<<grid, 256, 0, stream>>>(sc, sg.n, plan.c, plan.nwin, plan.nbuckets, cursors, sorted, fl, slot_base, sg.base0, d_flags);
+                        if (sg.mont) k_digits<true, true><<<grid, 256, 0, stream>>>(sc, sg.n, plan.c, plan.c_top, plan.nwin, plan.nbuckets, cursors, sorted, fl, slot_base, sg.base0, d_flags);
+                        else k_digits<true, false><<<grid, 256, 0, stream>>>(sc, sg.n, plan.c, plan.c_top, plan.nwin, plan.nbuckets, cursors, sorted, fl, slot_base, sg.base0, d_flags);
                     }
                     count_launch();
                 }
@@ -1372,11 +1452,13 @@
                 at += bases[i].n;
             }
         }
-        for (uint32_t w0 = 0; w0 < nsets; w0 += gw) {
-            const uint32_t wn = nsets - w0 < gw ? nsets - w0 : gw;
+        for (uint32_t u0 = 0; u0 < nwins; u0 += gu) {
+            const uint32_t un = nwins - u0 < gu ? nwins - u0 : gu;
+            const uint32_t w0 = set_of(u0), wn = set_of(u0 + un) - w0;
             const uint32_t tb = wn * plan.nbuckets;
             const uint32_t* bs = bucket_start + (size_t)w0 * plan.nbuckets;
-            size_t entries = set_cap * (size_t)wn;
+            const SetOffsets so = set_offsets(plan, flat, w0);
+            size_t entries = set_cap * (size_t)un;
             if (entries > max_entries) entries = max_entries;
             if (large_hot) CUDA_TRY(cudaMemsetAsync(hot_dev, 0, 4, stream));
             size_t items_bound = 1;
@@ -1407,25 +1489,26 @@
                     for (int i = 0; i < nsegs; i++) {
                         const MsmSegment& sg = segs[i];
                         if (sg.n == 0) continue;
-                        const int64_t first = (int64_t)sg.job * sets_per_job;
+                        const int64_t first = (int64_t)sg.job * wins_per_job;
                         int w_lo, w_hi;
                         if (flat) {
-                            if (first < (int64_t)w0 || first >= (int64_t)w0 + wn) continue;
+                            if (first < (int64_t)u0 || first >= (int64_t)u0 + un) continue;
                             w_lo = 0; w_hi = plan.nwin;
                         } else {
-                            const int64_t lo_w = (int64_t)w0 - first, hi_w = (int64_t)w0 + wn - first;
+                            const int64_t lo_w = (int64_t)u0 - first, hi_w = (int64_t)u0 + un - first;
                             w_lo = lo_w < 0 ? 0 : (int)lo_w; w_hi = hi_w > plan.nwin ? plan.nwin : (int)hi_w;
                             if (w_lo >= w_hi) continue;
                         }
                         const unsigned grid = (unsigned)((sg.n + 255) / 256);
                         const uint32_t slot_base = sg.job * sets_per_job * plan.nbuckets;
                         const uint32_t* sc = (const uint32_t*)sg.d_scalars;
+                        const int ct = plan.c_top, nw = plan.nwin;
                         if (flat) {
-                            if (sg.mont) k_scatter_records<true, true><<<grid, 256, 0, stream>>>(sc, sg.n, nullptr, 0, table, table_n, plan.c, plan.nbuckets, cursors, slot_base, w_lo, w_hi, bs, (uint4*)dense0);
-                            else k_scatter_records<false, true><<<grid, 256, 0, stream>>>(sc, sg.n, nullptr, 0, table, table_n, plan.c, plan.nbuckets, cursors, slot_base, w_lo, w_hi, bs, (uint4*)dense0);
+                            if (sg.mont) k_scatter_records<true, true><<<grid, 256, 0, stream>>>(sc, sg.n, nullptr, 0, table, table_n, plan.c, ct, nw, plan.nbuckets, cursors, slot_base, w_lo, w_hi, bs, (uint4*)dense0);
+                            else k_scatter_records<false, true><<<grid, 256, 0, stream>>>(sc, sg.n, nullptr, 0, table, table_n, plan.c, ct, nw, plan.nbuckets, cursors, slot_base, w_lo, w_hi, bs, (uint4*)dense0);
                         } else {
-                            if (sg.mont) k_scatter_records<true, false><<<grid, 256, 0, stream>>>(sc, sg.n, seg_points[i], seg_stride[i], nullptr, 0, plan.c, plan.nbuckets, cursors, slot_base, w_lo, w_hi, bs, (uint4*)dense0);
-                            else k_scatter_records<false, false><<<grid, 256, 0, stream>>>(sc, sg.n, seg_points[i], seg_stride[i], nullptr, 0, plan.c, plan.nbuckets, cursors, slot_base, w_lo, w_hi, bs, (uint4*)dense0);
+                            if (sg.mont) k_scatter_records<true, false><<<grid, 256, 0, stream>>>(sc, sg.n, seg_points[i], seg_stride[i], nullptr, 0, plan.c, ct, nw, plan.nbuckets, cursors, slot_base, w_lo, w_hi, bs, (uint4*)dense0);
+                            else k_scatter_records<false, false><<<grid, 256, 0, stream>>>(sc, sg.n, seg_points[i], seg_stride[i], nullptr, 0, plan.c, ct, nw, plan.nbuckets, cursors, slot_base, w_lo, w_hi, bs, (uint4*)dense0);
                         }
                         count_launch();
                     }
@@ -1535,14 +1618,14 @@
                     count_launch();
                     ent = red_b; m = groups; lgw += 3;
                 }
-                k_window_combine_quad<<<wn, 32u * ((m + 7u) / 8u), 0, stream>>>(ent, m, lgw, group_sums);
+                k_window_combine_quad<<<wn, 32u * ((m + 7u) / 8u), 0, stream>>>(ent, m, lgw, group_sums, so);
                 count_launch(2);
                 continue;
             }
             if (warp_reduce) {
                 const uint32_t wchunks = (plan.nbuckets + 31u) / 32u;
                 k_bucket_reduce_warp<<<(wn * wchunks * 32u + 127u) / 128u, 128, 0, stream>>>(final_partial, final_start, plan.nbuckets, wchunks, wn, red_a);
-                k_window_combine_warp<<<wn, 32, 0, stream>>>(red_a, wchunks, group_sums);
+                k_window_combine_warp<<<wn, 32, 0, stream>>>(red_a, wchunks, group_sums, so);
                 count_launch(2);
                 continue;
             }
@@ -1566,11 +1649,12 @@
                     uint32_t* done = other; other = (uint32_t*)ent; ent = done;
                     m = groups; lgw += 3;
                 }
-                k_window_combine_quad<<<wn, 32u * ((m + 7u) / 8u), 0, stream>>>(ent, m, lgw, group_sums);
+                k_window_combine_quad<<<wn, 32u * ((m + 7u) / 8u), 0, stream>>>(ent, m, lgw, group_sums, so);
                 count_launch();
                 continue;
             }
-            k_bucket_reduce<false><<<(nthreads + 127) / 128, 128, 0, stream>>>(final_partial, final_start, plan.nbuckets, chunk, chunks_per_set, wn, red_a);
+            k_bucket_reduce<false><<<(nthreads + 127) / 128, 128, 0, stream>>>(final_partial, final_start, plan.nbuckets, chunk, chunks_per_set, wn, red_a,
+                                                                                 nullptr, 0, so);
             count_launch(1);
             uint32_t per_row = chunks_per_set;
             const uint32_t* src = red_a;
@@ -1605,17 +1689,18 @@
 }
 int msm_sort_indices(const MsmPlan& plan, const void* d_scalars, size_t n, int mont, uint32_t* hist, uint32_t* bucket_start, uint32_t* cursors,
                      uint32_t* sorted, void* cub_tmp, size_t cub_bytes, uint32_t* d_flags, cudaStream_t stream) {
+    if (plan.nsets != plan.nwin || plan.c_top != plan.c) return (int)cudaErrorInvalidValue;
     const uint32_t TB = (uint32_t)plan.nwin * plan.nbuckets;
     int rc = (int)cudaMemsetAsync(hist, 0, (size_t)(TB + 1) * 4, stream);
     if (rc) return rc;
     const unsigned grid = (unsigned)((n + 255) / 256);
     const uint32_t* sc = (const uint32_t*)d_scalars;
-    if (mont) k_digits<false, true><<<grid, 256, 0, stream>>>(sc, n, plan.c, plan.nwin, plan.nbuckets, hist, nullptr, 0, 0u, 0u, d_flags);
-    else k_digits<false, false><<<grid, 256, 0, stream>>>(sc, n, plan.c, plan.nwin, plan.nbuckets, hist, nullptr, 0, 0u, 0u, d_flags);
+    if (mont) k_digits<false, true><<<grid, 256, 0, stream>>>(sc, n, plan.c, plan.c_top, plan.nwin, plan.nbuckets, hist, nullptr, 0, 0u, 0u, d_flags);
+    else k_digits<false, false><<<grid, 256, 0, stream>>>(sc, n, plan.c, plan.c_top, plan.nwin, plan.nbuckets, hist, nullptr, 0, 0u, 0u, d_flags);
     if ((rc = msm_exclusive_scan(cub_tmp, cub_bytes, hist, bucket_start, (size_t)TB + 1, stream)) != 0) return rc;
     if ((rc = (int)cudaMemcpyAsync(cursors, bucket_start, (size_t)(TB + 1) * 4, cudaMemcpyDeviceToDevice, stream)) != 0) return rc;
-    if (mont) k_digits<true, true><<<grid, 256, 0, stream>>>(sc, n, plan.c, plan.nwin, plan.nbuckets, cursors, sorted, 0, 0u, 0u, d_flags);
-    else k_digits<true, false><<<grid, 256, 0, stream>>>(sc, n, plan.c, plan.nwin, plan.nbuckets, cursors, sorted, 0, 0u, 0u, d_flags);
+    if (mont) k_digits<true, true><<<grid, 256, 0, stream>>>(sc, n, plan.c, plan.c_top, plan.nwin, plan.nbuckets, cursors, sorted, 0, 0u, 0u, d_flags);
+    else k_digits<true, false><<<grid, 256, 0, stream>>>(sc, n, plan.c, plan.c_top, plan.nwin, plan.nbuckets, cursors, sorted, 0, 0u, 0u, d_flags);
     count_launch(3);
     return (int)cudaGetLastError();
 }
@@ -1645,6 +1730,8 @@
     p.c = c;
     p.nwin = 253 / c + 1;
     p.nbuckets = 1u << (c - 1);
+    p.c_top = c;
+    p.nsets = p.nwin;
     size_t total = npoints * (size_t)p.nwin;
     size_t cap = total / 300000 + 1;
     if (cap < 16) cap = 16;
diff --git a/snarkvm_b200/csrc/msm.cuh b/snarkvm_b200/csrc/msm.cuh
--- a/snarkvm_b200/csrc/msm.cuh
+++ b/snarkvm_b200/csrc/msm.cuh
@@ -11,9 +11,18 @@
     uint32_t nbuckets;
     uint32_t cap;
     int levels;
+    int c_top;
+    int nsets;
+
+    int top_sets() const { return nsets - nwin + 1; }
+    int window_bit(int w) const { return w * c; }
+    int window_bits(int w) const { return w == nwin - 1 ? c_top : c; }
+    uint32_t window_buckets(int w) const { return 1u << (window_bits(w) - 1); }
+    int window_first_set(int w) const { return w; }
+    uint32_t set_digit_offset(int s) const { return s >= nwin ? (uint32_t)(s - nwin + 1) * nbuckets : 0u; }
 };
 
-MsmPlan msm_make_plan(size_t npoints);
+MsmPlan msm_make_plan(size_t npoints, bool mixed = true);
 MsmPlan msm_make_plan_batch(size_t max_n, size_t total_n);
 
 struct MsmBases {
```

Result: faster. 131.6 million (median of 6 runs) (+3.7%).
